# zhongzisha/multi_frame_super_resolution

Measured on AMD Instinct MI355X. Metric: Mpix/s end-to-end (N-frame burst -> x2 SR), higher is better.
Workload: dtype f32

## Files before the change

include/mfsr.h:

```cpp
#ifndef MFSR_H
#define MFSR_H

#include <stddef.h>
#include <stdint.h>

#ifdef __cplusplus
extern "C" {
#endif

#define MFSR_VERSION 100
#define MFSR_MAX_FUSE_GROUP 4

typedef void* mfsr_stream_t;

typedef struct { float x, y; } mfsr_float2;
typedef struct { float x, y, z; } mfsr_float3;
typedef struct { float x, y, z, w; } mfsr_float4;

typedef struct {
    const void* ptr;
    int32_t pitch;
    int32_t width;
    int32_t height;
} mfsr_tex2d;

enum {
    MFSR_OK = 0,
    MFSR_E_INVALID = -1,
    MFSR_E_UNSUPPORTED = -2,
    MFSR_E_NODEVICE = -3,
    MFSR_E_WORKSPACE = -4
};

enum { MFSR_RED = 0, MFSR_GREEN = 1, MFSR_BLUE = 2, MFSR_CYAN = 3, MFSR_MAGENTA = 4, MFSR_YELLOW = 5, MFSR_WHITE = 6 };

const char* mfsr_error_string(int code);
int mfsr_version(void);
int mfsr_device_count(void);

int mfsr_set_cfa_pattern(const int32_t pattern[4]);
int mfsr_get_cfa_pattern(int32_t pattern[4]);

int mfsr_deBayersSubSample3(const uint16_t* dataIn, mfsr_float3* imgOut, float maxVal, int dimX, int dimY, int strideOut,
                            mfsr_stream_t stream);
int mfsr_deBayerGreenKernel(int width, int height, const float* imgIn, int strideIn, mfsr_float3* outImage,
                            int strideOut, mfsr_float3 blackPoint, mfsr_float3 scale, mfsr_stream_t stream);
int mfsr_deBayerRedBlueKernel(int width, int height, const float* imgIn, int strideIn, mfsr_float3* outImage,
                              int strideOut, mfsr_float3 blackPoint, mfsr_float3 scale, mfsr_stream_t stream);
int mfsr_accumulateImages(const uint16_t* dataIn, mfsr_float3* imgOut, mfsr_float3* totalWeights,
                          const mfsr_float4* certaintyMask, const mfsr_float3* kernelParam, const mfsr_float2* shifts,
                          mfsr_float3 whiteLevel, mfsr_float3 blackLevel, int dimX, int dimY, int strideOut,
                          int strideMask, int strideShift, mfsr_stream_t stream);
int mfsr_accumulateImagesSuperRes(const uint16_t* dataIn, mfsr_float3* imgOut, mfsr_float3* totalWeights,
                                  const mfsr_float4* certaintyMask, mfsr_tex2d kernelParam, mfsr_tex2d shifts,
                                  mfsr_float3 whiteLevel, mfsr_float3 blackLevel, int dimX, int dimY, int strideOut,
                                  int strideMask, mfsr_stream_t stream);
int mfsr_accumulateSuperResFull(const uint16_t* dataIn, mfsr_float3* imgOut, mfsr_float3* totalWeights,
                                const mfsr_float4* certaintyMask, mfsr_tex2d kernelParam, mfsr_tex2d shifts,
                                mfsr_float3 whiteLevel, mfsr_float3 blackLevel, int dimX, int dimY, int scale,
                                int strideOut, int strideMask, mfsr_stream_t stream);

int mfsr_accumulateSuperResFull2(const uint16_t* dataIn0, const uint16_t* dataIn1, mfsr_float3* imgOut,
                                 mfsr_float3* totalWeights, const mfsr_float4* certaintyMask0,
                                 const mfsr_float4* certaintyMask1, mfsr_tex2d kernelParam, mfsr_tex2d shifts0,
                                 mfsr_tex2d shifts1, mfsr_float3 whiteLevel, mfsr_float3 blackLevel, int dimX, int dimY,
                                 int scale, int strideOut, int strideMask, mfsr_stream_t stream);

int mfsr_accumulateSuperResFullN(int nFrames, const uint16_t* const* dataIn, mfsr_float3* imgOut, mfsr_float3* totalWeights,
                                 const mfsr_float4* const* certaintyMask, mfsr_tex2d kernelParam, const mfsr_tex2d* shifts,
                                 mfsr_float3 whiteLevel, mfsr_float3 blackLevel, int dimX, int dimY, int scale,
                                 int strideOut, int strideMask, int accumulatorsUndefined, mfsr_stream_t stream);

int mfsr_accumulateSuperResFullRows(int nFrames, const uint16_t* const* dataIn, mfsr_float3* imgOut, mfsr_float3* totalWeights,
                                    const mfsr_float4* const* certaintyMask, mfsr_tex2d kernelParam, const mfsr_tex2d* shifts,
                                    mfsr_float3 whiteLevel, mfsr_float3 blackLevel, int dimX, int dimY, int scale,
                                    int strideOut, int strideMask, int accumulatorsUndefined, int rowBegin, int rowEnd,
                                    mfsr_stream_t stream);

int mfsr_accumulateSuperResFullWindow(int nFrames, const uint16_t* const* dataIn, mfsr_float3* imgOut, mfsr_float3* totalWeights,
                                      const mfsr_float4* const* certaintyMask, mfsr_tex2d kernelParam, const mfsr_tex2d* shifts,
                                      mfsr_float3 whiteLevel, mfsr_float3 blackLevel, int dimX, int dimY, int scale,
                                      int strideOut, int strideMask, int accumulatorsUndefined, int x0, int y0, int w, int h,
                                      mfsr_stream_t stream);

int mfsr_squaredSum(const float* inTiles, float* outValues, int maxShift, int tileSize, int tileCount,
                    mfsr_stream_t stream);
int mfsr_boxFilterWithBorderX(const float* inTiles, float* outTiles, int maxShift, int tileSize, int tileCount,
                              mfsr_stream_t stream);
int mfsr_boxFilterWithBorderY(const float* inTiles, float* outTiles, int maxShift, int tileSize, int tileCount,
                              mfsr_stream_t stream);
int mfsr_normalizedCC(const float* ccImage, const float* squaredTemplate, const float* boxFilteredImage,
                      float* shiftImage, int maxShift, int tileSize, int tileCount, mfsr_stream_t stream);
int mfsr_convertToTilesOverlapBorder(const float* inImg, float* outTiles, int imgWidth, int imgHeight, int imgPitch,
                                     int maxShift, int tileSize, int tileCountX, int tileCountY, mfsr_float2 baseShift,
                                     float baseRotation, mfsr_stream_t stream);
int mfsr_convertToTilesOverlapPreShift(const float* inImg, float* outTiles, const mfsr_float2* preShift,
                                       int preShiftPitch, int imgWidth, int imgHeight, int imgPitch, int maxShift,
                                       int tileSize, int tileCountX, int tileCountY, mfsr_float2 baseShift,
                                       float baseRotation, mfsr_stream_t stream);
int mfsr_GammasRGB(mfsr_float3* inOutImg, int imgWidth, int imgHeight, int imgPitch, mfsr_stream_t stream);
int mfsr_ApplyWeighting(mfsr_float3* inOutImg, const mfsr_float3* finalImg, const mfsr_float3* weight, int imgWidth,
                        int imgHeight, int imgPitch, float threshold, mfsr_stream_t stream);
int mfsr_conjugateComplexMulKernel(const mfsr_float2* aIn, mfsr_float2* bInOut, int maxElem,
                                   mfsr_stream_t stream);
int mfsr_findMinimum(const float* shiftImage, mfsr_float2* coordinates, int coordinatesPitch, int maxShift,
                     int tileCount, int tileCountX, float threshold, mfsr_stream_t stream);
int mfsr_UpSampleShifts(const mfsr_float2* inShift, mfsr_float2* outShift, int inPitch, int outPitch, int oldLevel,
                        int newLevel, int oldCountX, int oldCountY, int newCountX, int newCountY, int oldTileSize,
                        int newTileSize, mfsr_stream_t stream);
int mfsr_ComputeStructureTensor(const float* imgDx, const float* imgDy, mfsr_float3* outImg, int imgWidth,
                                int imgHeight, int imgDxDyPitch, int imgOutPitch, mfsr_stream_t stream);
int mfsr_ComputeKernelParam(mfsr_float3* kernelImg, int imgWidth, int imgHeight, int imgOutPitch, float Dth, float Dtr,
                            float kDetail, float kDenoise, float kStretch, float kShrink,
                            mfsr_stream_t stream);
int mfsr_fourierFilter(mfsr_float2* img, size_t stride, int width, int height, float lp, float hp, float lps,
                       float hps, int clearAxis, mfsr_stream_t stream);
int mfsr_fftshift(mfsr_float2* fft, int width, int height, mfsr_stream_t stream);

int mfsr_copyShiftMatrix(float* matrices, int tileCount, int imageCount, int shiftCount,
                         mfsr_stream_t stream);
int mfsr_setPointers(float** shiftMatrixArray, float** shiftMatrixSafeArray, float** matrixSquareArray,
                     float** matrixInvertedArray, float** solvedMatrixArray, mfsr_float2** shiftOneToOneArray,
                     mfsr_float2** shiftMeasuredArray, mfsr_float2** shiftOptimArray, float* shiftMatrices,
                     float* shiftSafeMatrices, float* matricesSquared, float* matricesInverted, float* solvedMatrices,
                     mfsr_float2* shiftsOneToOne, mfsr_float2* shiftsMeasured, mfsr_float2* shiftsOptim, int tileCount,
                     int imageCount, int shiftCount, mfsr_stream_t stream);
int mfsr_checkForOutliers(mfsr_float2* measuredShifts, const float* optimShiftsT, float* shiftMatrix, int* status,
                          int* inversionInfo, int tileCount, int imageCount, int shiftCount,
                          mfsr_stream_t stream);
int mfsr_transposeShifts(mfsr_float2* measuredShifts, const float* measuredShiftsT, const float* shiftsOneToOneT,
                         mfsr_float2* shiftsOneToOne, int tileCount, int imageCount, int shiftCount,
                         mfsr_stream_t stream);
int mfsr_getOptimalShifts(mfsr_float2* optimalShifts, const mfsr_float2* bestShifts, int imageCount, int tileCountX,
                          int tileCountY, int optimalShiftsPitch, int referenceImage, int imageToTrack,
                          mfsr_stream_t stream);
int mfsr_concatenateShifts(const mfsr_float2* const* shiftIn, int* shiftInPitch, mfsr_float2* shiftOut, int shiftCount,
// ... 189 lines not shown
                           int outPitch, uint16_t* out16, int width, int height, float threshold, int applyGamma, float maxOut,
                           int colOffset, int rowOffset, int fullWidth, int fullHeight, mfsr_stream_t stream);

typedef struct {
    int32_t width, height;
    int32_t frames;
    int32_t reference;
    int32_t scale;
    int32_t mono;
    int32_t cfa[4];
    float black[3], white[3];
    float maxVal;
    int32_t levels;
    int32_t levelFactor[4];
    int32_t tileSize[4];
    int32_t maxShift[4];
    float minimumThreshold;
    float sigmaTracking;
    int32_t lkIterations;
    int32_t lkHalfWindow;
    float lkMinDet;
    float alpha, beta, thresholdM;
    float sigmaTensor;
    float Dth, Dtr, kDetail, kDenoise, kStretch, kShrink;
    float weightThreshold;
    int32_t applyGamma;
    int32_t fused;
    int32_t pairFrames;
    int32_t asyncFuse;
    int32_t preAlign;
    float preAlignMaxAngle;
    int32_t uploadRing;
    int32_t maskErode;
    int32_t rawPacking;
} mfsr_config;

typedef struct mfsr_burst mfsr_burst;

int mfsr_config_default(mfsr_config* cfg, int width, int height, int frames, int scale, int mono);
size_t mfsr_burst_workspace_bytes(const mfsr_config* cfg);
size_t mfsr_burst_accumulator_bytes(const mfsr_config* cfg);
int mfsr_burst_create(mfsr_burst** out, const mfsr_config* cfg, void* workspace, size_t workspaceBytes);
void mfsr_burst_destroy(mfsr_burst* b);

int mfsr_window_check(const mfsr_config* cfg, int x0, int y0, int w, int h);
int mfsr_burst_set_window(mfsr_burst* b, int x0, int y0, int w, int h);
int mfsr_burst_get_window(const mfsr_burst* b, int* x0, int* y0, int* w, int* h);
int mfsr_burst_set_reference(mfsr_burst* b, const uint16_t* rawRef, mfsr_stream_t stream);
int mfsr_burst_set_reference_rows(mfsr_burst* b, const uint16_t* rawRef, int hrRow0, int hrRow1, mfsr_stream_t stream);
int mfsr_burst_add_frame(mfsr_burst* b, const uint16_t* raw, int isReference, mfsr_float3* imgOut,
                         mfsr_float3* totalWeights, mfsr_stream_t stream);
int mfsr_burst_begin(mfsr_burst* b, mfsr_float3* imgOut, mfsr_float3* totalWeights, mfsr_stream_t stream);
int mfsr_burst_flush(mfsr_burst* b, mfsr_stream_t stream);
int mfsr_burst_finish(mfsr_burst* b, const mfsr_float3* imgOut, const mfsr_float3* totalWeights, mfsr_float3* outImg,
                      uint16_t* out16, mfsr_stream_t stream);
int mfsr_burst_finish_rows(mfsr_burst* b, const mfsr_float3* imgOut, const mfsr_float3* totalWeights,
                           mfsr_float3* outImg, uint16_t* out16, int row0, int rows, mfsr_stream_t stream);
int mfsr_burst_set_reference_host(mfsr_burst* b, const uint16_t* hostRaw, mfsr_stream_t stream);
int mfsr_burst_add_frame_host(mfsr_burst* b, const uint16_t* hostRaw, int isReference, mfsr_float3* imgOut,
                              mfsr_float3* totalWeights, mfsr_stream_t stream);
int mfsr_burst_prefetch_host(mfsr_burst* b, const uint16_t* const* hostRaws, int nFrames, mfsr_stream_t stream);
int mfsr_burst_finish_host(mfsr_burst* b, const mfsr_float3* imgOut, const mfsr_float3* totalWeights, uint16_t* out16Dev,
                           uint16_t* out16Host, mfsr_stream_t stream);
int mfsr_burst_host_sync(mfsr_burst* b);
int mfsr_burst_set_host_row_bytes(mfsr_burst* b, int rowBytes);
int mfsr_burst_field_dims(const mfsr_burst* b, int* flowW, int* flowH, int* maskW, int* maskH);
int mfsr_burst_align_frame(mfsr_burst* b, const uint16_t* raw, int isReference, mfsr_float2* flowOut, int flowPitch,
                           mfsr_float4* maskOut, int maskPitch, mfsr_stream_t stream);
int mfsr_burst_align_frames(mfsr_burst* b, int nFrames, const uint16_t* const* raws, const int* isReference,
                            mfsr_float2* const* flowOut, int flowPitch, mfsr_float4* const* maskOut, int maskPitch,
                            mfsr_stream_t stream);
int mfsr_burst_group_size(const mfsr_config* cfg);
int mfsr_burst_fuse_rows(mfsr_burst* b, int nFrames, const uint16_t* const* raws, const mfsr_float2* const* flows, int flowPitch,
                         const mfsr_float4* const* masks, int maskPitch, mfsr_float3* imgOut, mfsr_float3* totalWeights,
                         int accumulatorsUndefined, int rowBegin, int rowEnd, mfsr_stream_t stream);

typedef struct {
    int32_t rowBegin, rowEnd;
    int32_t flowRow0, flowRows;
    int32_t maskRow0, maskRows;
    int32_t rawRow0, rawRows;
    float maxFlowY;
    int32_t reserved[3];
} mfsr_stripe_plan;
int mfsr_dist_stripe_plan(const mfsr_config* cfg, int worldSize, int rank, int rawHalo, mfsr_stripe_plan* out);
int mfsr_checkFlowBound(const mfsr_float2* flow, int pitch, int width, int rows, float bound, int* flag, mfsr_stream_t stream);
int mfsr_maxAbsFlowY(const mfsr_float2* flow, int pitch, int width, int rows, int* maxBits, mfsr_stream_t stream);
int mfsr_exactDivisionOk(float d);

typedef struct mfsr_stream mfsr_stream;
size_t mfsr_stream_workspace_bytes(const mfsr_config* cfg, int radius);
int mfsr_stream_create(mfsr_stream** out, const mfsr_config* cfg, int radius, int framesInHostMemory, void* workspace,
                       size_t workspaceBytes);
void mfsr_stream_destroy(mfsr_stream* s);
int mfsr_stream_push(mfsr_stream* s, const uint16_t* frame, mfsr_float3* outImg, uint16_t* out16, long long* produced,
                     mfsr_stream_t stream);
int mfsr_stream_drain(mfsr_stream* s, mfsr_float3* outImg, uint16_t* out16, long long* produced, mfsr_stream_t stream);
int mfsr_stream_reset(mfsr_stream* s);
int mfsr_stream_set_window(mfsr_stream* s, int x0, int y0, int w, int h);

size_t mfsr_burst_joint_workspace_bytes(const mfsr_config* cfg);
int mfsr_burst_process_joint(mfsr_burst* b, const uint16_t* const* frames, void* jointWorkspace, size_t jointBytes,
                             mfsr_float3* imgOut, mfsr_float3* totalWeights, mfsr_stream_t stream);

typedef struct {
    int (*next_frame)(void* user, uint16_t* dst, mfsr_stream_t stream);
// ... 178 lines not shown
```

multi_frame_super_resolution_amd/csrc/accumulate.hip:

```cpp
#include "accumulate_common.hpp"

__global__ void __launch_bounds__(256)
    k_accumulateImages(const uint16_t* __restrict__ dataIn, pix3* __restrict__ imgOut, pix3* __restrict__ totalWeights,
                       const float4* __restrict__ certaintyMask, const pix3* __restrict__ kernelParam,
                       const float2* __restrict__ shifts, Levels3 lv, int dimX, int dimY, int strideOut, int strideMask,
                       int strideShift, int cfa)
{
    const int x = blockIdx.x * blockDim.x + threadIdx.x;
    const int y = blockIdx.y * blockDim.y + threadIdx.y;
    if (x < 1 || y < 1 || x >= dimX - 1 || y >= dimY - 1) return;
    pix3 pixel = row_ptr(imgOut, strideOut, y)[x];
    pix3 totalWeight = row_ptr(totalWeights, strideOut, y)[x];
    const pix3 kernel = row_ptr(kernelParam, strideOut, y)[x];
    const float2 shift = row_ptr(shifts, strideShift, y)[x];
    const int sx = round2i(shift.x);
    const int sy = round2i(shift.y);
#pragma unroll
    for (int py = -2; py <= 2; py++) {
        const int ppsy = clampi(y + py + sy, 0, dimY - 1);
        const int ppy = clampi(y + py, 0, dimY - 1);
#pragma unroll
        for (int px = -2; px <= 2; px++) {
            const int ppsx = clampi(x + px + sx, 0, dimX - 1);
            const int ppx = clampi(x + px, 0, dimX - 1);
// ... 15 lines not shown
{
    MFSR_REQUIRE(dataIn && imgOut && totalWeights && certaintyMask && kernelParam && shifts);
    MFSR_REQUIRE(dimX > 2 && dimY > 2);
    MFSR_REQUIRE((long long)strideOut >= 12LL * dimX && (strideOut & 3) == 0);
    MFSR_REQUIRE((long long)strideShift >= 8LL * dimX && (strideShift & 7) == 0 && ((uintptr_t)shifts & 7) == 0);
    MFSR_REQUIRE((long long)strideMask >= 16LL * ((dimX + 1) / 2) && (strideMask & 15) == 0 &&
                 ((uintptr_t)certaintyMask & 15) == 0);
    dim3 block(64, 4), grid(mfsr_cdiv(dimX, 64), mfsr_cdiv(dimY, 4));
    hipLaunchKernelGGL(k_accumulateImages, grid, block, 0, mfsr_s(stream), dataIn, (pix3*)imgOut, (pix3*)totalWeights,
                       (const float4*)certaintyMask, (const pix3*)kernelParam, (const float2*)shifts,
                       make_levels(whiteLevel, blackLevel), dimX, dimY, strideOut, strideMask, strideShift,
                       mfsr_cfa_packed());
    return mfsr_launch_status("accumulateImages");
}

template <int GEOM, bool FAST, bool WIN = false>
__global__ void __launch_bounds__(256)
    k_accumulateSuperRes(const uint16_t* __restrict__ dataIn, pix3* __restrict__ imgOut, pix3* __restrict__ totalWeights,
                         const float4* __restrict__ certaintyMask, mfsr_tex2d kernelParam, mfsr_tex2d shifts, Levels3 lv,
                         int dimX, int dimY, int scale, int strideOut, int strideMask, int cfa, int rowBegin, int rowEnd,
                         int colBegin, int colEnd)
{
    const int x = blockIdx.x * blockDim.x + threadIdx.x + (WIN ? colBegin : 0);
    const int y = blockIdx.y * blockDim.y + threadIdx.y + rowBegin;
    const int outW = (GEOM == GEOM_CROP) ? dimX : dimX * scale;
    const int outH = (GEOM == GEOM_CROP) ? dimY : dimY * scale;
    if (x < 1 || y < 1 || x >= outW - 1 || y >= outH - 1 || y >= rowEnd) return;
    if (WIN && x >= colEnd) return;
    accumulate_pixel_generic<GEOM, FAST>(x, y, dataIn, imgOut, totalWeights, certaintyMask, kernelParam, shifts, lv, dimX,
                                         dimY, scale, strideOut, strideMask, cfa, WIN ? colBegin : 0, WIN ? rowBegin : 0);
}

static int g_accumulate_fast = 2;
extern "C" int mfsr_set_accumulate_fast_exp(int enable)
{
    g_accumulate_fast = enable < 0 ? 0 : (enable > 2 ? 2 : enable);
    return MFSR_OK;
}
extern "C" int mfsr_get_accumulate_fast_exp(void) { return g_accumulate_fast; }

int mfsr_try_launch_accumulate2x_strip(int nFrames, const uint16_t* const* dataIn, mfsr_float3* imgOut,
                                       mfsr_float3* totalWeights, const mfsr_float4* const* certaintyMask,
                                       mfsr_tex2d kernelParam, const mfsr_tex2d* shifts, mfsr_float3 whiteLevel,
                                       mfsr_float3 blackLevel, int dimX, int dimY, int strideOut, int strideMask,
                                       int fresh, int rowBegin, int rowEnd, int colBegin, int colEnd, int relative,
                                       mfsr_stream_t stream);

int mfsr_try_launch_accumulate4x_tile(int nFrames, const uint16_t* const* dataIn, mfsr_float3* imgOut,
                                      mfsr_float3* totalWeights, const mfsr_float4* const* certaintyMask,
                                      mfsr_tex2d kernelParam, const mfsr_tex2d* shifts, mfsr_float3 whiteLevel,
                                      mfsr_float3 blackLevel, int dimX, int dimY, int strideOut, int strideMask,
                                      int fresh, int rowBegin, int rowEnd, int colBegin, int colEnd, int relative,
                                      mfsr_stream_t stream);

static int check_superres_args(const uint16_t* dataIn, mfsr_float3* imgOut, mfsr_float3* totalWeights,
                               const mfsr_float4* certaintyMask, const mfsr_tex2d& kernelParam, const mfsr_tex2d& shifts,
                               int dimX, int dimY, int outW, int strideOut, int strideMask)
{
    MFSR_REQUIRE(dataIn && imgOut && totalWeights && certaintyMask);
    MFSR_REQUIRE(dimX >= 8 && dimY >= 8);
    MFSR_REQUIRE(mfsr_tex_ok(kernelParam, 16) && ((uintptr_t)kernelParam.ptr & 15) == 0 && (kernelParam.pitch & 15) == 0);
    MFSR_REQUIRE(mfsr_tex_ok(shifts, 8) && ((uintptr_t)shifts.ptr & 7) == 0 && (shifts.pitch & 7) == 0);
    MFSR_REQUIRE((long long)strideOut >= 12LL * outW && (strideOut & 3) == 0);
    MFSR_REQUIRE((long long)strideMask >= 16LL * ((dimX + 1) / 2) && (strideMask & 15) == 0 &&
                 ((uintptr_t)certaintyMask & 15) == 0);
    return MFSR_OK;
}

extern "C" int mfsr_accumulateImagesSuperRes(const uint16_t* dataIn, mfsr_float3* imgOut, mfsr_float3* totalWeights,
                                             const mfsr_float4* certaintyMask, mfsr_tex2d kernelParam, mfsr_tex2d shifts,
                                             mfsr_float3 whiteLevel, mfsr_float3 blackLevel, int dimX, int dimY,
                                             int strideOut, int strideMask, mfsr_stream_t stream)
{
    int rc = check_superres_args(dataIn, imgOut, totalWeights, certaintyMask, kernelParam, shifts, dimX, dimY, dimX,
                                 strideOut, strideMask);
    if (rc) return rc;
    dim3 block(64, 4), grid(mfsr_cdiv(dimX, 64), mfsr_cdiv(dimY, 4));
    const Levels3 lv = make_levels(whiteLevel, blackLevel);
    if (g_accumulate_fast)
        hipLaunchKernelGGL((k_accumulateSuperRes<GEOM_CROP, true>), grid, block, 0, mfsr_s(stream), dataIn, (pix3*)imgOut,
                           (pix3*)totalWeights, (const float4*)certaintyMask, kernelParam, shifts, lv, dimX, dimY, 2,
                           strideOut, strideMask, mfsr_cfa_packed(), 0, dimY, 0, 0);
    else
        hipLaunchKernelGGL((k_accumulateSuperRes<GEOM_CROP, false>), grid, block, 0, mfsr_s(stream), dataIn,
                           (pix3*)imgOut, (pix3*)totalWeights, (const float4*)certaintyMask, kernelParam, shifts, lv, dimX,
                           dimY, 2, strideOut, strideMask, mfsr_cfa_packed(), 0, dimY, 0, 0);
    return mfsr_launch_status("accumulateImagesSuperRes");
}

static int accumulate_full_win(const uint16_t* dataIn, mfsr_float3* imgOut, mfsr_float3* totalWeights,
                               const mfsr_float4* certaintyMask, mfsr_tex2d kernelParam, mfsr_tex2d shifts,
                               mfsr_float3 whiteLevel, mfsr_float3 blackLevel, int dimX, int dimY, int scale, int strideOut,
                               int strideMask, const HrWindow& w, mfsr_stream_t stream)
{
    MFSR_REQUIRE(scale >= 1 && scale <= 8);
    int rc = check_superres_args(dataIn, imgOut, totalWeights, certaintyMask, kernelParam, shifts, dimX, dimY,
                                 w.rel ? w.x1 - w.x0 : dimX * scale, strideOut, strideMask);
    if (rc) return rc;
    if (g_accumulate_fast == 2 && scale == 2 &&
        mfsr_try_launch_accumulate2x_strip(1, &dataIn, imgOut, totalWeights, &certaintyMask, kernelParam, &shifts, whiteLevel,
                                           blackLevel, dimX, dimY, strideOut, strideMask, 0, w.y0, w.y1, w.x0, w.x1, w.rel,
                                           stream) == 1)
        return mfsr_launch_status("accumulateSuperResFull(strip)");
    if (g_accumulate_fast == 2 && scale == 4 &&
        mfsr_try_launch_accumulate4x_tile(1, &dataIn, imgOut, totalWeights, &certaintyMask, kernelParam, &shifts, whiteLevel,
                                          blackLevel, dimX, dimY, strideOut, strideMask, 0, w.y0, w.y1, w.x0, w.x1, w.rel,
// ... 105 lines not shown
                                           blackLevel, dimX, dimY, scale, strideOut, strideMask, w, stream);
        if (rc) return rc;
    }
    return MFSR_OK;
}

extern "C" int mfsr_accumulateSuperResFullRows(int nFrames, const uint16_t* const* dataIn, mfsr_float3* imgOut,
                                               mfsr_float3* totalWeights, const mfsr_float4* const* certaintyMask,
                                               mfsr_tex2d kernelParam, const mfsr_tex2d* shifts, mfsr_float3 whiteLevel,
                                               mfsr_float3 blackLevel, int dimX, int dimY, int scale, int strideOut,
                                               int strideMask, int accumulatorsUndefined, int rowBegin, int rowEnd,
                                               mfsr_stream_t stream)
{
    MFSR_REQUIRE(nFrames >= 1 && nFrames <= MFSR_MAX_FUSE_GROUP && dataIn && certaintyMask && shifts);
    MFSR_REQUIRE(scale >= 1 && scale <= 8);
    const int hrH = scale * dimY;
    MFSR_REQUIRE(rowBegin >= 0 && rowBegin < rowEnd && rowEnd <= hrH && (rowBegin % 16) == 0 && ((rowEnd % 16) == 0 || rowEnd == hrH));
    return accumulate_group_win(nFrames, dataIn, imgOut, totalWeights, certaintyMask, kernelParam, shifts, whiteLevel, blackLevel, dimX,
                                dimY, scale, strideOut, strideMask, accumulatorsUndefined,
                                HrWindow{0, rowBegin, scale * dimX, rowEnd, 0}, stream);
}

extern "C" int mfsr_accumulateSuperResFullWindow(int nFrames, const uint16_t* const* dataIn, mfsr_float3* imgOut,
                                                 mfsr_float3* totalWeights, const mfsr_float4* const* certaintyMask,
                                                 mfsr_tex2d kernelParam, const mfsr_tex2d* shifts, mfsr_float3 whiteLevel,
                                                 mfsr_float3 blackLevel, int dimX, int dimY, int scale, int strideOut,
                                                 int strideMask, int accumulatorsUndefined, int x0, int y0, int w, int h,
                                                 mfsr_stream_t stream)
{
    MFSR_REQUIRE(nFrames >= 1 && nFrames <= MFSR_MAX_FUSE_GROUP && dataIn && certaintyMask && shifts);
    MFSR_REQUIRE(scale >= 1 && scale <= 8 && dimX > 0 && dimY > 0);
    const int hrW = scale * dimX, hrH = scale * dimY;
    if (w == 0 && h == 0 && x0 == 0 && y0 == 0) {
        w = hrW;
        h = hrH;
    }
    MFSR_REQUIRE(mfsr_window_ok(hrW, hrH, x0, y0, w, h));
    MFSR_REQUIRE((strideOut & 15) == 0 && ((uintptr_t)imgOut & 15) == 0 && ((uintptr_t)totalWeights & 15) == 0);
    return accumulate_group_win(nFrames, dataIn, imgOut, totalWeights, certaintyMask, kernelParam, shifts, whiteLevel, blackLevel, dimX,
                                dimY, scale, strideOut, strideMask, accumulatorsUndefined, HrWindow{x0, y0, x0 + w, y0 + h, 1}, stream);
}

extern "C" int mfsr_accumulateSuperResFullN(int nFrames, const uint16_t* const* dataIn, mfsr_float3* imgOut,
                                            mfsr_float3* totalWeights, const mfsr_float4* const* certaintyMask,
                                            mfsr_tex2d kernelParam, const mfsr_tex2d* shifts, mfsr_float3 whiteLevel,
                                            mfsr_float3 blackLevel, int dimX, int dimY, int scale, int strideOut,
                                            int strideMask, int accumulatorsUndefined, mfsr_stream_t stream)
{
    MFSR_REQUIRE(scale >= 1 && scale <= 8 && dimY > 0);
    return mfsr_accumulateSuperResFullRows(nFrames, dataIn, imgOut, totalWeights, certaintyMask, kernelParam, shifts, whiteLevel,
                                           blackLevel, dimX, dimY, scale, strideOut, strideMask, accumulatorsUndefined, 0,
                                           scale * dimY, stream);
}
```

multi_frame_super_resolution_amd/csrc/accumulate_fast.hip:

```cpp
#include <cstdlib>

#include "accumulate_common.hpp"
#include <type_traits>

namespace {

template <int CFA>
struct Cfa {
    static constexpr int col(int yp, int xp) { return (CFA >> (2 * ((yp << 1) | xp))) & 3; }
    static constexpr int pos_of(int c)
    {
        int n = 0, p = -1;
        for (int a = 0; a < 4; a++)
            if (((CFA >> (2 * a)) & 3) == c) {
                n++;
                p = a;
            }
        return n == 1 ? p : -1;
    }
    static constexpr int count(int c)
    {
        int n = 0;
        for (int a = 0; a < 4; a++)
            if (((CFA >> (2 * a)) & 3) == c) n++;
// ... 968 lines not shown
#pragma unroll 1
        for (int n = 0; n < NF; n++) {
            if (!((safeBits >> n) & 1u) && stripLive) {
                TileFrame F = fr.f[0];
#pragma unroll
                for (int m = 1; m < NF; m++)
                    if (n == m) F = fr.f[m];
#pragma unroll 1
                for (int k = 0; k < 4; k++) {
                    const int X = X0 + k;
                    if (X >= 1 && X < hrW - 1) {
                        pix3 px = {0.0f, 0.0f, 0.0f}, tw = {0.0f, 0.0f, 0.0f};
                        if (DO_P) px = {myP[3 * k], myP[3 * k + 1], myP[3 * k + 2]};
                        if (DO_W) tw = {myW[3 * k], myW[3 * k + 1], myW[3 * k + 2]};
                        accumulate_pixel_core<GEOM_FULL, true>(X, Y, F.raw, F.mask, kernelParam, F.shifts, glv, dimX, dimY, 2,
                                                               strideMask, cfaPacked, px, tw);
                        if (DO_P) { myP[3 * k] = px.x; myP[3 * k + 1] = px.y; myP[3 * k + 2] = px.z; }
                        if (DO_W) { myW[3 * k] = tw.x; myW[3 * k + 1] = tw.y; myW[3 * k + 2] = tw.z; }
                    }
                }
            }
        }
    };
    auto store_plane = [&](int pl, char* g) {
        asm volatile("s_waitcnt lgkmcnt(0)" ::: "memory");
#pragma unroll
        for (int j = 0; j < 3; j++) {
            const size_t off = (size_t)(j * 64 + lx) * 16;
            const size_t gb = segByte + off;
            const bool sideMargin = gb < (size_t)STRIP_MARGIN * 12 || gb + 16 > rowBytes - (size_t)STRIP_MARGIN * 12;
            if (gb + 16 <= rowBytes && (fresh || !sideMargin) && inWin(gb)) *(float4*)chunk(g, off) = sAcc[pl][ly][j * 64 + lx];
        }
    };
    using Yes = std::true_type;
    using No = std::false_type;
    asm volatile("s_waitcnt vmcnt(0)" ::: "memory");
    constexpr bool valueSumsStaged = TILE_PIXEL_MAJOR && (NF > 1 || FR != 4);
    if constexpr (PL == 2) {
        if (!valueSumsStaged) add_plane(0, accP);
        add_plane(1, accW);
        if (safeBits != (1u << NF) - 1u) slow_frames(Yes{}, Yes{}, 0, 1);
        store_plane(0, gP);
        store_plane(1, gW);
    } else {
        if (!valueSumsStaged) add_plane(0, accP);
        if (safeBits != (1u << NF) - 1u) slow_frames(Yes{}, No{}, 0, 0);
        store_plane(0, gP);
        asm volatile("s_waitcnt lgkmcnt(0)" ::: "memory");
        stage_plane(gW, 0);
        asm volatile("s_waitcnt vmcnt(0)" ::: "memory");
        add_plane(0, accW);
        if (safeBits != (1u << NF) - 1u) slow_frames(No{}, Yes{}, 0, 0);
        store_plane(0, gW);
    }
}

template <int K8, int CFA, bool PARITY = false, typename RawF, typename MaskF>
__device__ __forceinline__ void strip_pixel4_w(int X, int Y, int sx, int sy, const float (&w)[13], RawF rawf, MaskF mval,
                                                const StripLevels& lv, float* accP, float* accW)
{
    const int qx = X + sx - 2, qy = Y + sy - 2;
    const int x0 = qx >> 2, y0 = qy >> 2;
    const uint32_t bx0 = 0u - (uint32_t)(qx & 1), bx1 = 0u - (uint32_t)((qx >> 1) & 1);
    const uint32_t by0 = 0u - (uint32_t)(qy & 1), by1 = 0u - (uint32_t)((qy >> 1) & 1);
    const uint32_t mx[5] = {0u, bx0 & bx1, bx1, bx0 | bx1, ~0u};
    const uint32_t my[5] = {0u, by0 & by1, by1, by0 | by1, ~0u};
    const uint32_t mP = 0u - (uint32_t)(x0 & 1), mQ = 0u - (uint32_t)(y0 & 1);
    auto andm = [](uint32_t m, float a) { return __uint_as_float(m & __float_as_uint(a)); };

    float s[2][2];
    rawf(x0, y0, s);
    auto W_ = [&](int jt, int it) { const int n = jt * 5 + it; return w[n <= 12 ? n : 24 - n]; };

    auto cellOf = [](int it) { return (K8 + it - 2 + 8) >> 3; };
    constexpr int cellLo = (K8 - 2 + 8) >> 3;
    constexpr bool twoCells = ((K8 + 4 - 2 + 8) >> 3) != cellLo;

    float C[5][2];
#pragma unroll
    for (int jt = 0; jt < 5; jt++) {
        const uint32_t mya = mQ ^ my[jt];
        float Ee[2], Eo[2];
        if constexpr (PARITY) {
            const int ph = qy & 3;
            const int flip = jt == 0 ? 0 : (jt == 4 ? 1 : (jt == 1 ? (ph == 3) : (jt == 2 ? (ph >> 1) : (ph != 0))));
            const int e = (((y0 & 1) ^ flip) << 1) | (x0 & 1);
#pragma unroll
            for (int c = 0; c < (twoCells ? 2 : 1); c++) {
                Ee[c] = mval(jt, cellLo + c, e);
                Eo[c] = mval(jt, cellLo + c, e ^ 1);
            }
        } else {
#pragma unroll
            for (int c = 0; c < (twoCells ? 2 : 1); c++) {
                float m[3];
#pragma unroll
                for (int ch = 0; ch < 3; ch++) m[ch] = mval(jt, cellLo + c, ch);
                resolve_certainty<CFA>(mya, mP, m, Ee[c], Eo[c]);
            }
        }
        float lo[2] = {0.0f, 0.0f}, hi[2] = {0.0f, 0.0f};
        bool loUsed[2] = {false, false}, hiUsed[2] = {false, false};
#pragma unroll
        for (int it = 0; it < 5; it++) {
            const int c = cellOf(it) - cellLo;
            const float wt = W_(jt, it);
// ... 627 lines not shown
            if (msx) {
                (void)hipEventRecord(msx->join, msx->stream);
                (void)hipStreamWaitEvent(st, msx->join, 0);
            }
        };
        if (nFrames == 1) launch_mono(std::integral_constant<int, 1>{});
        if (nFrames == 2) launch_mono(std::integral_constant<int, 2>{});
        return 1;
    }
#define STRIP_CASE(a, b, c, d)                                                                                         \
    case pack_cfa(a, b, c, d):                                                                                         \
        if (pair) {                                                                                                    \
            using CfaTag = std::integral_constant<int, pack_cfa(a, b, c, d)>;                                          \
            if (nFrames == 2) launch_group(CfaTag{}, std::integral_constant<int, 2>{});                                \
            if (nFrames == 3) launch_group(CfaTag{}, std::integral_constant<int, 3>{});                                \
            if (nFrames == 4) launch_group(CfaTag{}, std::integral_constant<int, 4>{});                                \
        } else if (nFrames == 2) {                                                                                     \
            TileFrames<2> fr;                                                                                          \
            for (int n = 0; n < 2; n++) {                                                                              \
                fr.f[n].raw = dataIn[n];                                                                               \
                fr.f[n].mask = (const float4*)certaintyMask[n];                                                        \
                fr.f[n].shifts = shifts[n];                                                                            \
            }                                                                                                          \
            launch_strip_regs<pack_cfa(a, b, c, d), 2>(grid, block, st, fr, pI, pT, kernelParam, glv, lv, dimX, dimY,  \
                                                       strideOut, strideMask, cp, rowBlock0, wlc);                                \
            launch_margin(0);                                                                                          \
            launch_margin(1);                                                                                          \
        } else {                                                                                                       \
            TileFrames<1> fr;                                                                                          \
            fr.f[0].raw = dataIn[0];                                                                                   \
            fr.f[0].mask = (const float4*)certaintyMask[0];                                                            \
            fr.f[0].shifts = shifts[0];                                                                                \
            if (tile_kernel_ok(kernelParam, shifts[0], dimX, dimY))                                                    \
                launch_tile<pack_cfa(a, b, c, d), 1>(grid, block, st, fr, pI, pT, kernelParam, glv, lv, dimX, dimY,    \
                                                     strideOut, strideMask, cp, tileFresh, rowBlock0, wlc);                       \
            else                                                                                                       \
                launch_strip_regs<pack_cfa(a, b, c, d), 1>(grid, block, st, fr, pI, pT, kernelParam, glv, lv, dimX,    \
                                                           dimY, strideOut, strideMask, cp, rowBlock0, wlc);                       \
            launch_margin(0);                                                                                          \
        }                                                                                                              \
        return 1;
    switch (packed2) {
        STRIP_CASE(MFSR_RED, MFSR_GREEN, MFSR_GREEN, MFSR_BLUE)
        STRIP_CASE(MFSR_BLUE, MFSR_GREEN, MFSR_GREEN, MFSR_RED)
        STRIP_CASE(MFSR_GREEN, MFSR_RED, MFSR_BLUE, MFSR_GREEN)
        STRIP_CASE(MFSR_GREEN, MFSR_BLUE, MFSR_RED, MFSR_GREEN)
        STRIP_CASE(MFSR_GREEN, MFSR_GREEN, MFSR_GREEN, MFSR_GREEN)
        default: break;
    }
#undef STRIP_CASE
    return 0;
}

int mfsr_try_launch_accumulate4x_tile(int nFrames, const uint16_t* const* dataIn, mfsr_float3* imgOut,
                                      mfsr_float3* totalWeights, const mfsr_float4* const* certaintyMask,
                                      mfsr_tex2d kernelParam, const mfsr_tex2d* shifts, mfsr_float3 whiteLevel,
                                      mfsr_float3 blackLevel, int dimX, int dimY, int strideOut, int strideMask,
                                      int fresh, int rowBegin, int rowEnd, int colBegin, int colEnd, int relative,
                                      mfsr_stream_t stream)
{
    read_env_once();
    if (nFrames < 1 || nFrames > 4 || !g_strip_use_tile) return 0;
    int cfa[4];
    mfsr_get_cfa_pattern(cfa);
    for (int i = 0; i < 4; i++)
        if (cfa[i] > MFSR_BLUE) return 0;
    const int packed2 = pack_cfa(cfa[0], cfa[1], cfa[2], cfa[3]);
    const int hrW = 4 * dimX, hrH = 4 * dimY;
    if ((dimX & 1) || (dimY & 1) || ((uintptr_t)imgOut & 15) || ((uintptr_t)totalWeights & 15) || (strideOut & 15)) return 0;
    if (hrW < 4 * STRIP_MARGIN || hrH < 4 * STRIP_MARGIN) return 0;
    for (int n = 0; n < nFrames; n++)
        if (!(kernelParam.width == shifts[n].width && kernelParam.height == shifts[n].height && kernelParam.width * 8 == hrW &&
              kernelParam.height * 8 == hrH && kernelParam.width >= 4))
            return 0;
    Levels3 glv;
    StripLevels lv;
    const float wl[3] = {whiteLevel.x, whiteLevel.y, whiteLevel.z}, bl[3] = {blackLevel.x, blackLevel.y, blackLevel.z};
    for (int c = 0; c < 3; c++) {
        glv.white[c] = wl[c];
        glv.black[c] = bl[c];
        lv.black[c] = bl[c];
        lv.invWhite[c] = 1.0f / wl[c];
    }
    hipStream_t st = mfsr_s(stream);
    pix3* pI = (pix3*)imgOut;
    pix3* pT = (pix3*)totalWeights;
    const int cp = mfsr_cfa_packed();
    const int tileY0 = rowBegin / 2;
    const WinLaunch wlc = win_launch(HrWindow{colBegin, rowBegin, colEnd, rowEnd, relative}, hrW, 512);
    const MarginRects mr = margin_rects(hrW, hrH, STRIP_MARGIN, HrWindow{colBegin, rowBegin, colEnd, rowEnd, relative});
    const int tilesX = wlc.tilesX, tilesY = mfsr_cdiv(rowEnd, 2) - tileY0;
    const dim3 block(64, 4), grid(tilesX * tilesY);
    if (fresh) {
        if (zero_margin_bands(imgOut, totalWeights, hrH, strideOut, rowBegin, rowEnd, wlc, st) != 0) return -1;
    }
    MarginStream* msx = (g_margin_overlap && !fresh) ? margin_stream() : nullptr;
    if (msx && (hipEventRecord(msx->fork, st) != hipSuccess || hipStreamWaitEvent(msx->stream, msx->fork, 0) != hipSuccess)) msx = nullptr;
    const hipStream_t mst = msx ? msx->stream : st;
    auto launch_margin = [&](int n) {
        const int M = STRIP_MARGIN;
        const long long cnt = 2LL * (M - 1) * (hrW - 2) + (long long)(hrH - 2 * M) * 2 * (M - 1);
        if (!wlc.on)
            hipLaunchKernelGGL(k_accumulateMargin<4>, dim3(mfsr_cdiv(cnt, 256)), dim3(256), 0, mst, dataIn[n], pI, pT,
                               (const float4*)certaintyMask[n], kernelParam, shifts[n], glv, dimX, dimY, strideOut, strideMask, cp,
                               rowBegin, rowEnd, mr);
        else if (mr.start[4] > 0)
// ... 53 lines not shown
```

multi_frame_super_resolution_amd/csrc/pipeline.cpp:

```cpp
#include <hip/hip_runtime.h>

#include <cmath>
#include <cstdio>
#include <cstring>
#include <new>
#include <vector>

#include "common.hpp"
#include "raw_stage.hpp"

namespace {

constexpr int kMaxLevels = 4;
constexpr int kMaxTimedLaunches = 4096;
constexpr int kRing = 2 * MFSR_MAX_FUSE_GROUP;
constexpr int kMaxUploadRing = 32;

inline size_t align_up(size_t v, size_t a) { return (v + a - 1) / a * a; }

struct Img {
    void* ptr = nullptr;
    int pitch = 0;
    int w = 0, h = 0;
};

struct FrameProducts {
    uint16_t* raw;
    Img half;
    Img pyr[8];
    void* prePyr;
};

struct AlignScratch {
    Img shifts[kMaxLevels];
    Img lkSum[2], lkDiff[2];
    mfsr_prealign* preResult;
};

struct Layout {
    int W, H, hw, hh, tw, th, hrW, hrH;
    int flowScale;
    int lw[kMaxLevels], lh[kMaxLevels];
    int tcx[kMaxLevels], tcy[kMaxLevels];
    int maxFactor;
    FrameProducts ref, mov[MFSR_MAX_FUSE_GROUP];
    AlignScratch work[MFSR_MAX_FUSE_GROUP];
    int nAlign;
    Img kparam4;
    Img tensor, tensorTmp, tensorSm;
    Img fallback;
    Img tmpA, tmpB;
    Img flowBuf[2 * kRing];
    Img maskBuf[kRing];
    Img maskRaw[MFSR_MAX_FUSE_GROUP];
    Img pre[kMaxLevels];
    Img warped, Ix, Iy, It, rawf;
    float *refTiles, *movTiles, *cc, *boxX, *boxY, *sqsum, *dist;
    float* refSq[kMaxLevels];
    void* preWork;
    uint16_t* rawRing[kMaxUploadRing];
    uint16_t* refRaw[2];
    uint8_t* stage[kMaxUploadRing + 2];
    size_t total;
};

struct Bump {
    char* base;
    size_t off;
    void* take(size_t bytes)
    {
        off = align_up(off, 256);
        void* p = base ? base + off : nullptr;
        off += bytes;
        return p;
    }
    Img image(int w, int h, int elemBytes)
    {
        Img im;
        im.w = w;
        im.h = h;
        im.pitch = (int)align_up((size_t)w * elemBytes, 64);
        im.ptr = take((size_t)im.pitch * h);
        return im;
    }
};

int ilog2(int v)
{
    int l = 0;
    while ((1 << l) < v) l++;
    return l;
}

int validate(const mfsr_config* c)
{
    MFSR_REQUIRE(c != nullptr);
    MFSR_REQUIRE(c->width >= 64 && c->height >= 64 && (c->width % 4) == 0 && (c->height % 4) == 0);
    MFSR_REQUIRE(c->frames >= 1 && c->reference >= 0 && c->reference < c->frames);
    MFSR_REQUIRE(c->scale >= 1 && c->scale <= 8);
    MFSR_REQUIRE(c->levels >= 1 && c->levels <= kMaxLevels);
    MFSR_REQUIRE(c->levelFactor[c->levels - 1] == 1);
    for (int l = 0; l < c->levels; l++) {
        const int f = c->levelFactor[l];
        MFSR_REQUIRE(f >= 1 && f <= 128 && (f & (f - 1)) == 0);
        if (l > 0) MFSR_REQUIRE(c->levelFactor[l] < c->levelFactor[l - 1]);
        MFSR_REQUIRE(c->tileSize[l] >= 4 && c->tileSize[l] <= 128 && c->maxShift[l] >= 1 && c->maxShift[l] <= 15);
// ... 69 lines not shown
    for (int l = 0; l < kMaxLevels; l++) L->refSq[l] = nullptr;
    if (c->fused) {
        for (int l = 0; l < c->levels; l++) L->refSq[l] = (float*)b.take((size_t)L->tcx[l] * L->tcy[l] * 4);
        for (int i = 0; i < 2; i++) {
            L->work[0].lkSum[i] = b.image(L->tw, L->th, 4);
            L->work[0].lkDiff[i] = b.image(L->tw, L->th, 4);
        }
    }
    L->Ix = b.image(L->tw, L->th, 4);
    L->Iy = b.image(L->tw, L->th, 4);
    if (!c->fused) {
        L->warped = b.image(L->tw, L->th, 4);
        L->It = b.image(L->tw, L->th, 4);
        L->rawf = b.image(L->W, L->H, 4);
        L->refTiles = (float*)b.take(maxTileFloats * 4);
        L->movTiles = (float*)b.take(maxTileFloats * 4);
        L->cc = (float*)b.take(maxTileFloats * 4);
        L->boxX = (float*)b.take(maxTileFloats * 4);
        L->boxY = (float*)b.take(maxTileFloats * 4);
        L->sqsum = (float*)b.take(maxTiles * 4);
        L->dist = (float*)b.take(maxDist * 4);
    }
    if (c->preAlign) {
        const size_t pb = mfsr_preAlign_pyramid_bytes(L->tw, L->th);
        L->ref.prePyr = b.take(pb);
        L->mov[0].prePyr = b.take(pb);
        L->preWork = b.take(mfsr_preAlign_workspace_bytes(c->preAlignMaxAngle));
        L->work[0].preResult = (mfsr_prealign*)b.take(sizeof(mfsr_prealign));
    }
    L->nAlign = c->fused ? mfsr_burst_group_size(c) : 1;
    for (int q = 1; q < L->nAlign; q++) {
        FrameProducts& M = L->mov[q];
        AlignScratch& S = L->work[q];
        M.half = b.image(L->hw, L->hh, 12);
        for (int i = 0; i < nl; i++) M.pyr[i] = b.image(L->tw >> i, L->th >> i, 4);
        for (int l = 0; l < c->levels; l++) S.shifts[l] = b.image(L->tcx[l], L->tcy[l], 8);
        for (int i = 0; i < 2; i++) {
            S.lkSum[i] = b.image(L->tw, L->th, 4);
            S.lkDiff[i] = b.image(L->tw, L->th, 4);
        }
        if (c->preAlign) {
            M.prePyr = b.take(mfsr_preAlign_pyramid_bytes(L->tw, L->th));
            S.preResult = (mfsr_prealign*)b.take(sizeof(mfsr_prealign));
        }
    }
    for (int i = 0; i < c->uploadRing; i++) L->rawRing[i] = (uint16_t*)b.take((size_t)L->W * L->H * 2);
    if (c->uploadRing > 0)
        for (int i = 0; i < 2; i++) L->refRaw[i] = (uint16_t*)b.take((size_t)L->W * L->H * 2);
    if (c->maskErode > 0)
        for (int i = 0; i < mfsr_burst_group_size(c); i++) L->maskRaw[i] = b.image(L->hw, L->hh, 16);
    if (c->rawPacking != MFSR_PACK_NONE)
        for (int i = 0; i < c->uploadRing + 2; i++)
            L->stage[i] = (uint8_t*)b.take((size_t)mfsr_packed_row_bytes(c->rawPacking, L->W) * L->H);
    L->total = align_up(b.off, 256);
    return layout;
}

mfsr_tex2d as_tex(const Img& im)
{
    mfsr_tex2d t;
    t.ptr = im.ptr;
    t.pitch = im.pitch;
    t.width = im.w;
    t.height = im.h;
    return t;
}

}

struct mfsr_burst {
    mfsr_burst(const mfsr_config& c, char* workspace) : cfg(c), L(make_layout(&c, workspace)) {}
    mfsr_config cfg;
    const Layout L;
    FrameProducts ref;
    float taps[99];
    int ntaps;
    float tensorTaps[99];
    int ntensorTaps;
    const Img* flowCur;
    const Img* maskCur;
    mfsr_prealign* preCur;
    bool haveRef;
    bool refStale;
    struct Pending {
        int n;
        int slot[MFSR_MAX_FUSE_GROUP];
        const uint16_t* raw[MFSR_MAX_FUSE_GROUP];
        const Img* flow[MFSR_MAX_FUSE_GROUP];
        const Img* mask[MFSR_MAX_FUSE_GROUP];
        bool deferred[MFSR_MAX_FUSE_GROUP];
        int isRef[MFSR_MAX_FUSE_GROUP];
        mfsr_float3 *imgOut, *totalWeights;
    } pend;
    Pending held;
    bool heldHas;
    int group;
    int nFramesTimed;
    struct Fresh {
        bool has;
        mfsr_float3 *imgOut, *totalWeights;
    } fresh;
    int frameCounter;
    hipStream_t fuseStream;
    hipEvent_t evAligned[kRing];
    hipEvent_t evFused[kRing];
    hipEvent_t evRefStart, evRefDone;
    bool refOnFuse;
    bool fusedOutstanding[kRing];
    const Img* slotFlow[kRing];
    hipStream_t copyStream;
    hipStream_t downStream;
    hipEvent_t evFinished, evDown;
    bool downRecorded;
    hipEvent_t evBand[16];
    int framesSinceRef;
    bool holdLastGroup;
    hipEvent_t evUp[kMaxUploadRing + 2];
    hipEvent_t evFree[kMaxUploadRing + 2];
    bool freeRecorded[kMaxUploadRing + 2];
    hipStream_t freeOn[kMaxUploadRing + 2];
    int hostRowBytes;
    bool renderOn;
    mfsr_render render;
    bool sharpenOn;
    mfsr_sharpen sharpen;
    int sharpenedFinishes;
    unsigned long long hostEpoch;
    hipEvent_t evEpoch;
    hipEvent_t evUnp[kMaxUploadRing + 2];
    hipEvent_t unpDone[kMaxUploadRing + 2];
    int unpQ[kMaxUploadRing + 2], nUnp;
    struct Prefetched {
        const uint16_t* host;
        int slot;
    } prefetched[kMaxUploadRing];
    int nPrefetched, prefetchHead;
    bool upPending;
    int upPendingSlot;
    int refSlot;
    bool hostBusy;
    int upCounter, refCounter;
    const uint16_t* refHost;
    const uint16_t* refDev;
    std::vector<float> jointHost;
    struct Window {
        bool on = false;
        int x0 = 0, y0 = 0, w = 0, h = 0;
    } win, winNext;
    bool timing;
    int nEvents;
    hipEvent_t evStart[kMaxTimedLaunches], evStop[kMaxTimedLaunches];
    int32_t paths[MFSR_PATH_COUNT];
};

#define TRY(expr)                  \
    do {                           \
        int rc_ = (expr);          \
        if (rc_ != MFSR_OK) return rc_; \
    } while (0)

static int flush_pending(mfsr_burst* b, mfsr_stream_t stream, bool materializeFresh = true);

static int out_w(const mfsr_burst* b) { return b->win.on ? b->win.w : b->L.hrW; }
static int out_h(const mfsr_burst* b) { return b->win.on ? b->win.h : b->L.hrH; }
static size_t acc_bytes(const mfsr_burst* b) { return (size_t)12 * out_w(b) * out_h(b); }

static int fuse_group(mfsr_burst* b, int n, const uint16_t* const* raws, mfsr_float3* imgOut, mfsr_float3* totalWeights,
                      const mfsr_float4* const* masks, const mfsr_tex2d* flows, int maskPitch, int fresh, int r0, int r1,
                      mfsr_stream_t stream)
{
    const mfsr_config& c = b->cfg;
    const Layout& L = b->L;
    const mfsr_float3 white = {c.white[0], c.white[1], c.white[2]};
    const mfsr_float3 black = {c.black[0], c.black[1], c.black[2]};
    if (!b->win.on)
        return mfsr_accumulateSuperResFullRows(n, raws, imgOut, totalWeights, masks, as_tex(L.kparam4), flows, white, black, L.W, L.H,
                                               c.scale, 12 * L.hrW, maskPitch, fresh, r0, r1, stream);
    const int pitch = 12 * b->win.w;
    const size_t off = (size_t)r0 * pitch;
    return mfsr_accumulateSuperResFullWindow(n, raws, (mfsr_float3*)((char*)imgOut + off), (mfsr_float3*)((char*)totalWeights + off),
                                             masks, as_tex(L.kparam4), flows, white, black, L.W, L.H, c.scale, pitch, maskPitch, fresh,
                                             b->win.x0, b->win.y0 + r0, b->win.w, r1 - r0, stream);
}


extern "C" int mfsr_config_default(mfsr_config* cfg, int width, int height, int frames, int scale, int mono)
{
    MFSR_REQUIRE(cfg != nullptr);
    memset(cfg, 0, sizeof(*cfg));
    cfg->width = width;
    cfg->height = height;
    cfg->frames = frames;
    cfg->reference = 0;
    cfg->scale = scale;
    cfg->mono = mono;
    if (mono) {
        cfg->cfa[0] = cfg->cfa[1] = cfg->cfa[2] = cfg->cfa[3] = MFSR_GREEN;
    } else {
        cfg->cfa[0] = MFSR_RED;
        cfg->cfa[1] = MFSR_GREEN;
        cfg->cfa[2] = MFSR_GREEN;
        cfg->cfa[3] = MFSR_BLUE;
    }
    for (int i = 0; i < 3; i++) {
// ... 19 lines not shown
    cfg->sigmaTensor = 1.0f;
    cfg->Dth = 0.005f;
    cfg->Dtr = 0.05f;
    cfg->kDetail = 0.3f;
    cfg->kDenoise = 2.0f;
    cfg->kStretch = 2.0f;
    cfg->kShrink = 2.0f;
    cfg->weightThreshold = 1e-3f;
    cfg->applyGamma = 0;
    cfg->fused = 1;
    cfg->pairFrames = 1;
    cfg->preAlign = 0;
    cfg->preAlignMaxAngle = 20.0f;
    cfg->asyncFuse = 0;
    return MFSR_OK;
}

extern "C" size_t mfsr_burst_workspace_bytes(const mfsr_config* cfg)
{
    if (validate(cfg) != MFSR_OK) return 0;
    return make_layout(cfg, nullptr).total;
}

extern "C" size_t mfsr_burst_accumulator_bytes(const mfsr_config* cfg)
{
    if (!cfg || cfg->width <= 0 || cfg->height <= 0 || cfg->scale <= 0) return 0;
    return (size_t)12 * cfg->scale * cfg->width * (size_t)cfg->scale * cfg->height;
}

extern "C" int mfsr_burst_create(mfsr_burst** out, const mfsr_config* cfg, void* workspace, size_t workspaceBytes)
{
    MFSR_REQUIRE(out != nullptr && workspace != nullptr);
    TRY(validate(cfg));
    if (mfsr_device_count() <= 0) {
        fprintf(stderr, "mfsr: no HIP device available (there is no CPU fallback)\n");
        return MFSR_E_NODEVICE;
    }
    MFSR_REQUIRE(((uintptr_t)workspace & 255) == 0);
    mfsr_burst* b = new (std::nothrow) mfsr_burst(*cfg, (char*)workspace);
    MFSR_REQUIRE(b != nullptr);
    if (b->L.total > workspaceBytes) {
        fprintf(stderr, "mfsr: workspace too small: need %zu bytes, got %zu\n", b->L.total, workspaceBytes);
        delete b;
        return MFSR_E_WORKSPACE;
    }
    b->ntaps = mfsr_gaussin_filter_1D(cfg->sigmaTracking, b->taps);
    b->ntensorTaps = mfsr_gaussin_filter_1D(cfg->sigmaTensor, b->tensorTaps);
    b->flowCur = &b->L.flowBuf[0];
    b->maskCur = &b->L.maskBuf[0];
    b->preCur = b->L.work[0].preResult;
    b->ref = b->L.ref;
    b->pend.n = 0;
    b->group = mfsr_burst_group_size(&b->cfg);
    b->fresh.has = false;
    b->nFramesTimed = 0;
    b->timing = false;
    b->nEvents = 0;
    memset(b->evStart, 0, sizeof(b->evStart));
    memset(b->evStop, 0, sizeof(b->evStop));
    b->frameCounter = 0;
    b->fuseStream = nullptr;
    b->evRefStart = b->evRefDone = nullptr;
    b->refOnFuse = false;
    for (int i = 0; i < kRing; i++) {
        b->evAligned[i] = b->evFused[i] = nullptr;
        b->fusedOutstanding[i] = false;
        b->slotFlow[i] = nullptr;
    }
    if (cfg->asyncFuse) {
        int lo = 0, hi = 0;
        hipError_t e = hipDeviceGetStreamPriorityRange(&lo, &hi);
        static const int prioMode = [] {
            const char* v = getenv("MFSR_FUSE_PRIO");
            return !v ? 0 : (v[0] == 'l' ? 1 : (v[0] == 'n' ? 2 : 0));
        }();
        const int prio = prioMode == 1 ? lo : (prioMode == 2 ? (lo + hi) / 2 : hi);
        if (e == hipSuccess) e = hipStreamCreateWithPriority(&b->fuseStream, hipStreamNonBlocking, prio);
        if (e == hipSuccess) e = hipEventCreateWithFlags(&b->evRefStart, hipEventDisableTiming);
        if (e == hipSuccess) e = hipEventCreateWithFlags(&b->evRefDone, hipEventDisableTiming);
        for (int i = 0; i < kRing && e == hipSuccess; i++) {
            e = hipEventCreateWithFlags(&b->evAligned[i], hipEventDisableTiming);
            if (e == hipSuccess) e = hipEventCreateWithFlags(&b->evFused[i], hipEventDisableTiming);
        }
        if (e != hipSuccess) {
            mfsr_burst_destroy(b);
            return MFSR_E_NODEVICE;
        }
    }
    b->copyStream = nullptr;
    b->downStream = nullptr;
    b->evFinished = b->evDown = nullptr;
    b->downRecorded = false;
    b->upCounter = b->refCounter = 0;
    for (int i = 0; i < 16; i++) b->evBand[i] = nullptr;
    b->framesSinceRef = 0;
    b->holdLastGroup = false;
    b->heldHas = false;
    b->held.n = 0;
    b->refHost = b->refDev = nullptr;
    b->refSlot = -1;
    b->hostBusy = false;
    b->upPending = false;
    b->upPendingSlot = -1;
    b->nPrefetched = b->prefetchHead = 0;
    for (int i = 0; i < kMaxUploadRing + 2; i++) {
        b->evUp[i] = b->evFree[i] = b->evUnp[i] = b->unpDone[i] = nullptr;
        b->freeRecorded[i] = false;
        b->freeOn[i] = nullptr;
    }
    b->hostRowBytes = 0;
    b->renderOn = false;
    b->sharpenOn = false;
    b->sharpenedFinishes = 0;
    b->nUnp = 0;
    b->hostEpoch = 0;
    b->evEpoch = nullptr;
    if (cfg->uploadRing > 0) {
        hipError_t e = hipStreamCreateWithFlags(&b->copyStream, hipStreamNonBlocking);
        if (e == hipSuccess) e = hipStreamCreateWithFlags(&b->downStream, hipStreamNonBlocking);
        if (e == hipSuccess) e = hipEventCreateWithFlags(&b->evFinished, hipEventDisableTiming);
        if (e == hipSuccess) e = hipEventCreateWithFlags(&b->evDown, hipEventDisableTiming);
        if (e == hipSuccess) e = hipEventCreateWithFlags(&b->evEpoch, hipEventDisableTiming);
        for (int i = 0; i < cfg->uploadRing + 2 && e == hipSuccess; i++) {
            e = hipEventCreateWithFlags(&b->evUp[i], hipEventDisableTiming);
            if (e == hipSuccess) e = hipEventCreateWithFlags(&b->evFree[i], hipEventDisableTiming);
            if (e == hipSuccess && cfg->rawPacking != MFSR_PACK_NONE) e = hipEventCreateWithFlags(&b->evUnp[i], hipEventDisableTiming);
        }
        if (e != hipSuccess) {
            mfsr_burst_destroy(b);
            return MFSR_E_NODEVICE;
        }
    }
    b->haveRef = false;
    b->refStale = false;
    memset(b->paths, 0, sizeof(b->paths));
    *out = b;
    return MFSR_OK;
}

extern "C" void mfsr_burst_destroy(mfsr_burst* b)
{
    if (!b) return;
    for (int i = 0; i < kMaxTimedLaunches; i++) {
        if (b->evStart[i]) (void)hipEventDestroy(b->evStart[i]);
        if (b->evStop[i]) (void)hipEventDestroy(b->evStop[i]);
    }
    if (b->fuseStream) (void)hipStreamSynchronize(b->fuseStream);
    for (int i = 0; i < kRing; i++) {
        if (b->evAligned[i]) (void)hipEventDestroy(b->evAligned[i]);
        if (b->evFused[i]) (void)hipEventDestroy(b->evFused[i]);
    }
    if (b->evRefStart) (void)hipEventDestroy(b->evRefStart);
    if (b->evRefDone) (void)hipEventDestroy(b->evRefDone);
    if (b->fuseStream) (void)hipStreamDestroy(b->fuseStream);
    if (b->copyStream) (void)hipStreamSynchronize(b->copyStream);
    if (b->downStream) (void)hipStreamSynchronize(b->downStream);
    if (b->evFinished) (void)hipEventDestroy(b->evFinished);
    if (b->evDown) (void)hipEventDestroy(b->evDown);
    if (b->evEpoch) (void)hipEventDestroy(b->evEpoch);
    for (int i = 0; i < 16; i++)
        if (b->evBand[i]) (void)hipEventDestroy(b->evBand[i]);
    if (b->downStream) (void)hipStreamDestroy(b->downStream);
    for (int i = 0; i < kMaxUploadRing + 2; i++) {
        if (b->evUp[i]) (void)hipEventDestroy(b->evUp[i]);
        if (b->evFree[i]) (void)hipEventDestroy(b->evFree[i]);
        if (b->evUnp[i]) (void)hipEventDestroy(b->evUnp[i]);
    }
    if (b->copyStream) (void)hipStreamDestroy(b->copyStream);
    delete b;
}

extern "C" int mfsr_burst_timing(mfsr_burst* b, int enable)
{
    MFSR_REQUIRE(b != nullptr);
    b->timing = enable != 0;
    b->nEvents = 0;
    b->nFramesTimed = 0;
    return MFSR_OK;
}

extern "C" int mfsr_burst_timing_read(mfsr_burst* b, double* totalMs, int* launches, int* frames)
{
    MFSR_REQUIRE(b && totalMs && launches && frames);
    double total = 0;
    for (int i = 0; i < b->nEvents; i++) {
        MFSR_HIP_TRY(hipEventSynchronize(b->evStop[i]));
        float ms = 0;
        MFSR_HIP_TRY(hipEventElapsedTime(&ms, b->evStart[i], b->evStop[i]));
        total += ms;
    }
    *totalMs = total;
    *launches = b->nEvents;
    *frames = b->nFramesTimed;
    b->nEvents = 0;
    b->nFramesTimed = 0;
    return MFSR_OK;
}

static int unpack_uploaded(mfsr_burst* b, int lastSlot, mfsr_stream_t stream);
static int wait_uploads(mfsr_burst* b, mfsr_stream_t stream)
{
    if (b->upPending) {
        MFSR_HIP_TRY(hipStreamWaitEvent(mfsr_s(stream), b->evUp[b->upPendingSlot], 0));
        b->upPending = false;
        if (b->nUnp > 0) TRY(unpack_uploaded(b, b->upPendingSlot, stream));
    }
    return MFSR_OK;
}

static int record_free(mfsr_burst* b, int us, mfsr_stream_t stream)
{
    MFSR_HIP_TRY(hipEventRecord(b->evFree[us], mfsr_s(stream)));
    b->freeRecorded[us] = true;
    b->freeOn[us] = mfsr_s(stream);
    return MFSR_OK;
}

static int unpack_uploaded(mfsr_burst* b, int lastSlot, mfsr_stream_t stream)
{
    const Layout& L = b->L;
    int n = 0;
    while (n < b->nUnp && b->unpQ[n] != lastSlot) n++;
    if (n == b->nUnp) return MFSR_OK;
    n++;
    const uint8_t* packed[kMaxUploadRing + 2];
    uint16_t* frames[kMaxUploadRing + 2];
    for (int i = 0; i < n; i++) {
        const int us = b->unpQ[i];
        packed[i] = L.stage[us];
        frames[i] = us < b->cfg.uploadRing ? L.rawRing[us] : L.refRaw[us - b->cfg.uploadRing];
        if (b->freeRecorded[us]) {
            if (b->freeOn[us] != mfsr_s(stream)) MFSR_HIP_TRY(hipStreamWaitEvent(mfsr_s(stream), b->evFree[us], 0));
            b->freeRecorded[us] = false;
        }
    }
    static_assert(kMaxUploadRing + 2 <= kRawMaxFrames, "one launch takes every upload slot");
    TRY(mfsr_unpackRaw(n, packed, mfsr_packed_row_bytes(b->cfg.rawPacking, L.W), b->cfg.rawPacking, frames, 2 * L.W, L.W, L.H, stream));
    hipEvent_t done = b->evUnp[b->unpQ[0]];
    MFSR_HIP_TRY(hipEventRecord(done, mfsr_s(stream)));
    for (int i = 0; i < n; i++) b->unpDone[b->unpQ[i]] = done;
    for (int i = n; i < b->nUnp; i++) b->unpQ[i - n] = b->unpQ[i];
    b->nUnp -= n;
    return MFSR_OK;
}

// ... 130 lines not shown
    if (!fusedRing) MFSR_HIP_TRY(hipMemsetAsync(fb, 0, (size_t)L.fallback.pitch * (r1 - r0), mfsr_s(es)));
    if (c.fused) {
        if (fusedRing) {
            const mfsr_tex2d fbt = {fb, L.fallback.pitch, L.W, r1 - r0};
            TRY(mfsr_deBayerFusedRing(rawRef + (size_t)r0 * L.W, fbt, bp, sc, es));
        } else
            TRY(mfsr_deBayerFused(rawRef + (size_t)r0 * L.W, (mfsr_float3*)fb, L.fallback.pitch, L.W, r1 - r0, bp, sc, es));
        if (es != stream) {
            MFSR_HIP_TRY(hipEventRecord(b->evRefDone, b->fuseStream));
            b->refOnFuse = true;
        }
    } else {
        TRY(mfsr_u16ToFloat(rawRef, (float*)L.rawf.ptr, L.rawf.pitch, L.W, L.H, 1.0f, stream));
        TRY(mfsr_deBayerGreenKernel(L.W, L.H, (const float*)L.rawf.ptr, L.rawf.pitch, (mfsr_float3*)L.fallback.ptr,
                                    L.fallback.pitch, bp, sc, stream));
        TRY(mfsr_deBayerRedBlueKernel(L.W, L.H, (const float*)L.rawf.ptr, L.rawf.pitch, (mfsr_float3*)L.fallback.ptr,
                                      L.fallback.pitch, bp, sc, stream));
    }
    b->haveRef = true;
    b->refStale = false;
    b->framesSinceRef = 0;
    b->holdLastGroup = false;
    return MFSR_OK;
}

extern "C" int mfsr_burst_set_reference(mfsr_burst* b, const uint16_t* rawRef, mfsr_stream_t stream)
{
    MFSR_REQUIRE(b != nullptr);
    return set_reference_impl(b, rawRef, 0, b->L.hrH, stream);
}

extern "C" int mfsr_burst_set_reference_rows(mfsr_burst* b, const uint16_t* rawRef, int hrRow0, int hrRow1, mfsr_stream_t stream)
{
    MFSR_REQUIRE(b != nullptr);
    return set_reference_impl(b, rawRef, hrRow0, hrRow1, stream);
}

extern "C" int mfsr_window_check(const mfsr_config* cfg, int x0, int y0, int w, int h)
{
    MFSR_REQUIRE(cfg != nullptr);
    TRY(validate(cfg));
    const int hrW = cfg->width * cfg->scale, hrH = cfg->height * cfg->scale;
    if (x0 == 0 && y0 == 0 && ((w == 0 && h == 0) || (w == hrW && h == hrH))) return MFSR_OK;
    if (!mfsr_window_ok(hrW, hrH, x0, y0, w, h)) return MFSR_E_INVALID;
    if (!cfg->fused) return MFSR_E_UNSUPPORTED;
    return MFSR_OK;
}

extern "C" int mfsr_burst_set_window(mfsr_burst* b, int x0, int y0, int w, int h)
{
    MFSR_REQUIRE(b != nullptr);
    const int rc = mfsr_window_check(&b->cfg, x0, y0, w, h);
    if (rc != MFSR_OK) return rc;
    if (b->pend.n > 0 || b->heldHas) {
        fprintf(stderr, "mfsr: mfsr_burst_set_window with frames pending (flush or finish the burst first)\n");
        return MFSR_E_INVALID;
    }
    const Layout& L = b->L;
    const bool whole = (x0 == 0 && y0 == 0 && w == 0 && h == 0) || (x0 == 0 && y0 == 0 && w == L.hrW && h == L.hrH);
    b->winNext.on = !whole;
    b->winNext.x0 = whole ? 0 : x0;
    b->winNext.y0 = whole ? 0 : y0;
    b->winNext.w = whole ? 0 : w;
    b->winNext.h = whole ? 0 : h;
    return MFSR_OK;
}

extern "C" int mfsr_burst_get_window(const mfsr_burst* b, int* x0, int* y0, int* w, int* h)
{
    MFSR_REQUIRE(b && x0 && y0 && w && h);
    const mfsr_burst::Window& v = b->winNext;
    *x0 = v.on ? v.x0 : 0;
    *y0 = v.on ? v.y0 : 0;
    *w = v.on ? v.w : b->L.hrW;
    *h = v.on ? v.h : b->L.hrH;
    return MFSR_OK;
}

static int track_tiles(mfsr_burst* b, const FrameProducts& refF, float* const* refSq, const FrameProducts& movF,
                       const AlignScratch& work, const mfsr_prealign* hostBase, mfsr_stream_t stream)
{
    const mfsr_config& c = b->cfg;
    const Layout& L = b->L;
    const mfsr_float2 zero2 = {0.0f, 0.0f};
    for (int l = 0; l < c.levels; l++) {
        const int pi = ilog2(c.levelFactor[l]);
        const Img& ref = refF.pyr[pi];
        const Img& mov = movF.pyr[pi];
        const int T = c.tileSize[l], S = c.maxShift[l];
        const int tiles = L.tcx[l] * L.tcy[l];
        const mfsr_float2* pre = nullptr;
        b->paths[mfsr_trackTilesFastSupported(T, S) ? MFSR_PATH_TRACK_FAST_PAIR : MFSR_PATH_TRACK_GENERIC_PAIR]++;
        if (c.fused && l > 0) {
            TRY(mfsr_trackTilesFusedUp((const float*)ref.ptr, (const float*)mov.ptr, (const mfsr_float2*)work.shifts[l - 1].ptr,
                                       work.shifts[l - 1].pitch, c.levelFactor[l - 1], c.levelFactor[l], L.tcx[l - 1], L.tcy[l - 1],
                                       c.tileSize[l - 1], (mfsr_float2*)work.shifts[l].ptr, work.shifts[l].pitch, ref.w, ref.h, ref.pitch, S,
                                       T, L.tcx[l], L.tcy[l], c.minimumThreshold, refSq[l], c.preAlign ? work.preResult : nullptr,
                                       1.0f / (float)c.levelFactor[l], stream));
            b->paths[MFSR_PATH_TRACK_FUSED_UP]++;
            continue;
        }
        if (l > 0) {
            TRY(mfsr_UpSampleShifts((const mfsr_float2*)work.shifts[l - 1].ptr, (mfsr_float2*)L.pre[l].ptr,
                                    work.shifts[l - 1].pitch, L.pre[l].pitch, c.levelFactor[l - 1], c.levelFactor[l],
                                    L.tcx[l - 1], L.tcy[l - 1], L.tcx[l], L.tcy[l], c.tileSize[l - 1], T, stream));
            pre = (const mfsr_float2*)L.pre[l].ptr;
        }
        if (c.fused) {
            TRY(mfsr_trackTilesFusedBase((const float*)ref.ptr, (const float*)mov.ptr, pre, L.pre[l].pitch,
                                         (mfsr_float2*)work.shifts[l].ptr, work.shifts[l].pitch, ref.w, ref.h, ref.pitch, S, T,
                                         L.tcx[l], L.tcy[l], c.minimumThreshold, refSq[l],
                                         c.preAlign ? work.preResult : nullptr, 1.0f / (float)c.levelFactor[l], stream));
            b->paths[MFSR_PATH_TRACK_FUSED_BASE]++;
        } else {
            b->paths[MFSR_PATH_TRACK_CHAIN]++;
            if (!pre) {
                MFSR_HIP_TRY(hipMemsetAsync(L.pre[l].ptr, 0, (size_t)L.pre[l].pitch * L.pre[l].h, mfsr_s(stream)));
                pre = (const mfsr_float2*)L.pre[l].ptr;
            }
            TRY(mfsr_convertToTilesOverlapBorder((const float*)ref.ptr, L.refTiles, ref.w, ref.h, ref.pitch, S, T, L.tcx[l],
                                                 L.tcy[l], zero2, 0.0f, stream));
            mfsr_float2 base = zero2;
            float rot = 0.0f;
            if (hostBase) {
                const float inv = 1.0f / (float)c.levelFactor[l];
                base.x = hostBase->shiftX * inv;
                base.y = hostBase->shiftY * inv;
                rot = hostBase->rotation;
            }
            TRY(mfsr_convertToTilesOverlapPreShift((const float*)mov.ptr, L.movTiles, pre, L.pre[l].pitch, mov.w, mov.h,
                                                   mov.pitch, S, T, L.tcx[l], L.tcy[l], base, rot, stream));
            TRY(mfsr_crossCorrelateTiles(L.refTiles, L.movTiles, L.cc, S, T, tiles, stream));
            TRY(mfsr_squaredSum(L.refTiles, L.sqsum, S, T, tiles, stream));
            TRY(mfsr_boxFilterWithBorderX(L.movTiles, L.boxX, S, T, tiles, stream));
            TRY(mfsr_boxFilterWithBorderY(L.boxX, L.boxY, S, T, tiles, stream));
            TRY(mfsr_normalizedCC(L.cc, L.sqsum, L.boxY, L.dist, S, T, tiles, stream));
            TRY(mfsr_findMinimum(L.dist, (mfsr_float2*)work.shifts[l].ptr, work.shifts[l].pitch, S, tiles, L.tcx[l],
                                 c.minimumThreshold, stream));
            TRY(mfsr_addRoundedPreShift(pre, L.pre[l].pitch, (mfsr_float2*)work.shifts[l].ptr, work.shifts[l].pitch, L.tcx[l],
                                        L.tcy[l], stream));
        }
    }
    return MFSR_OK;
}

static int upload_slot_of(const mfsr_burst* b, const uint16_t* raw)
{
    if (!raw) return -1;
    for (int i = 0; i < b->cfg.uploadRing; i++)
        if (b->L.rawRing[i] == raw) return i;
    for (int i = 0; i < 2; i++)
        if (b->cfg.uploadRing > 0 && b->L.refRaw[i] == raw) return b->cfg.uploadRing + i;
    return -1;
}

static int align_deferred(mfsr_burst* b, mfsr_stream_t stream);

static int accumulate_pending(mfsr_burst* b, mfsr_stream_t callerStream);

static int fuse_held(mfsr_burst* b, mfsr_stream_t callerStream)
{
    if (!b->heldHas) return MFSR_OK;
    const mfsr_burst::Pending later = b->pend;
    b->pend = b->held;
    b->heldHas = false;
    b->held.n = 0;
    const int rc = accumulate_pending(b, callerStream);
    b->pend = later;
    return rc;
}

static int accumulate_pending(mfsr_burst* b, mfsr_stream_t callerStream)
{
    TRY(fuse_held(b, callerStream));
    TRY(align_deferred(b, callerStream));
    TRY(wait_uploads(b, callerStream));
    const mfsr_config& c = b->cfg;
    const mfsr_burst::Pending p = b->pend;
    b->pend.n = 0;
    const int n = p.n;
    if (n == 0) return MFSR_OK;
    mfsr_float3* imgOut = p.imgOut;
    mfsr_float3* totalWeights = p.totalWeights;
    mfsr_stream_t stream = callerStream;
    if (b->fuseStream) {
        stream = (mfsr_stream_t)b->fuseStream;
        for (int i = 0; i < n; i++) MFSR_HIP_TRY(hipStreamWaitEvent(b->fuseStream, b->evAligned[p.slot[i]], 0));
    }
    TRY(mfsr_set_cfa_pattern(c.cfa));
    const bool timed = b->timing && b->nEvents < kMaxTimedLaunches;
    if (timed) {
        const int i = b->nEvents;
        if (!b->evStart[i]) MFSR_HIP_TRY(hipEventCreate(&b->evStart[i]));
        if (!b->evStop[i]) MFSR_HIP_TRY(hipEventCreate(&b->evStop[i]));
        MFSR_HIP_TRY(hipEventRecord(b->evStart[i], mfsr_s(stream)));
    }
    {
        const mfsr_float4* masks[MFSR_MAX_FUSE_GROUP];
        mfsr_tex2d flows[MFSR_MAX_FUSE_GROUP];
        for (int i = 0; i < n; i++) {
            masks[i] = (const mfsr_float4*)p.mask[i]->ptr;
            flows[i] = as_tex(*p.flow[i]);
        }
        const int freshNow = b->fresh.has && b->fresh.imgOut == imgOut && b->fresh.totalWeights == totalWeights;
        if (b->fresh.has && !freshNow) {
            const size_t bytes = acc_bytes(b);
            MFSR_HIP_TRY(hipMemsetAsync(b->fresh.imgOut, 0, bytes, mfsr_s(stream)));
            MFSR_HIP_TRY(hipMemsetAsync(b->fresh.totalWeights, 0, bytes, mfsr_s(stream)));
        }
        b->fresh.has = false;
        TRY(fuse_group(b, n, p.raw, imgOut, totalWeights, masks, flows, p.mask[0]->pitch, freshNow, 0, out_h(b), stream));
    }
    if (timed) {
        MFSR_HIP_TRY(hipEventRecord(b->evStop[b->nEvents], mfsr_s(stream)));
        b->nEvents++;
        b->nFramesTimed += n;
    }
    if (b->copyStream) {
        for (int j = 0; j < n; j++) {
            const int us = upload_slot_of(b, p.raw[j]);
            if (us >= 0) TRY(record_free(b, us, stream));
        }
    }
    if (b->fuseStream) {
        for (int i = 0; i < n; i++) {
            MFSR_HIP_TRY(hipEventRecord(b->evFused[p.slot[i]], b->fuseStream));
            b->fusedOutstanding[p.slot[i]] = true;
        }
    }
    return MFSR_OK;
}

static int wait_ref_products(mfsr_burst* b, mfsr_stream_t stream)
{
    if (b->refOnFuse && mfsr_s(stream) != b->fuseStream) MFSR_HIP_TRY(hipStreamWaitEvent(mfsr_s(stream), b->evRefDone, 0));
    return MFSR_OK;
}

static int join_fuse(mfsr_burst* b, mfsr_stream_t stream)
{
    if (!b->fuseStream) return MFSR_OK;
    TRY(wait_ref_products(b, stream));
    for (int i = 0; i < kRing; i++)
        if (b->fusedOutstanding[i]) {
            MFSR_HIP_TRY(hipStreamWaitEvent(mfsr_s(stream), b->evFused[i], 0));
            b->fusedOutstanding[i] = false;
        }
    return MFSR_OK;
}

static int flush_pending(mfsr_burst* b, mfsr_stream_t stream, bool materializeFresh)
{
    if (materializeFresh && b->fresh.has && b->pend.n == 0 && !b->heldHas) {
        const size_t bytes = acc_bytes(b);
        MFSR_HIP_TRY(hipMemsetAsync(b->fresh.imgOut, 0, bytes, mfsr_s(stream)));
        MFSR_HIP_TRY(hipMemsetAsync(b->fresh.totalWeights, 0, bytes, mfsr_s(stream)));
        b->fresh.has = false;
    }
    TRY(accumulate_pending(b, stream));
    return join_fuse(b, stream);
}

static bool lk_warped_path(const mfsr_burst* b)
{
    static const bool lkWarped = [] {
        const char* e = getenv("MFSR_LK_WARPED");
        return !(e && e[0] == '0');
    }();
    const mfsr_config& c = b->cfg;
    return c.fused && lkWarped && c.lkIterations > 0 && b->L.tw >= 64 && b->L.th >= 32;
}

static const Img* final_flow(const mfsr_burst* b, int slot, int isReference)
{
    const mfsr_config& c = b->cfg;
    return &b->L.flowBuf[2 * slot + (!isReference && c.fused ? (c.lkIterations & 1) : 0)];
}

static int align_pre(mfsr_burst* b, const uint16_t* raw, int isReference, int slot, const FrameProducts& mov, bool prepared,
                     const AlignScratch& work, const Img* suppliedShifts, mfsr_stream_t stream)
{
    const mfsr_config& c = b->cfg;
    const Layout& L = b->L;
    const FrameProducts& ref = b->ref;
    TRY(wait_uploads(b, stream));
    if (b->fuseStream && b->fusedOutstanding[slot]) {
        MFSR_HIP_TRY(hipStreamWaitEvent(mfsr_s(stream), b->evFused[slot], 0));
        b->fusedOutstanding[slot] = false;
    }
    const Img* flow = &L.flowBuf[2 * slot];
    if (isReference) {
        const Img* mask = &L.maskBuf[slot];
        MFSR_HIP_TRY(hipMemsetAsync(flow->ptr, 0, (size_t)flow->pitch * flow->h, mfsr_s(stream)));
        return mfsr_fill_f32((float*)mask->ptr, (size_t)mask->pitch / 4 * mask->h, 1.0f, stream);
    }
    if (!prepared) TRY(prepare_frame(b, raw, mov, stream));
    mfsr_prealign hostBase;
    const mfsr_prealign* hb = nullptr;
    if (c.preAlign) {
        if (!prepared) TRY(mfsr_preAlignPyramid((const float*)mov.pyr[0].ptr, L.tw, L.th, mov.pyr[0].pitch, mov.prePyr, stream));
        TRY(mfsr_preAlign(ref.prePyr, mov.prePyr, L.tw, L.th, c.preAlignMaxAngle, L.preWork, work.preResult, stream));
        b->preCur = work.preResult;
        if (!c.fused) {
            MFSR_HIP_TRY(hipMemcpyAsync(&hostBase, work.preResult, sizeof(hostBase), hipMemcpyDeviceToHost, mfsr_s(stream)));
            MFSR_HIP_TRY(hipStreamSynchronize(mfsr_s(stream)));
            hb = &hostBase;
// ... 275 lines not shown
    bool maskBatch = stageBatch && batched && m > 0;
    if (maskBatch) {
        mfsr_robustness_frame rf[MFSR_MAX_FUSE_GROUP];
        for (int k = 0; k < m; k++) {
            const int slot = b->pend.slot[idx[mq[k]]];
            rf[k].movedHalf = (const mfsr_float3*)L.mov[mq[k]].half.ptr;
            rf[k].mask = (mfsr_float4*)(c.maskErode > 0 ? L.maskRaw[k].ptr : L.maskBuf[slot].ptr);
            rf[k].flow = (const mfsr_float2*)final_flow(b, slot, 0)->ptr;
        }
        const int rc = mfsr_robustnessMaskFusedBatch(m, rf, (const mfsr_float3*)ref.half.ptr, L.flowBuf[0].pitch, L.tw, L.th, L.hw, L.hh,
                                                     ref.half.pitch, L.maskBuf[0].pitch, c.alpha, c.beta, c.thresholdM, stream);
        if (rc == MFSR_E_UNSUPPORTED)
            maskBatch = false;
        else if (rc)
            return rc;
        else
            b->paths[MFSR_PATH_ROBUST_BATCH]++;
        if (maskBatch && c.maskErode > 0) {
            const mfsr_float4* ein[MFSR_MAX_FUSE_GROUP];
            mfsr_float4* eout[MFSR_MAX_FUSE_GROUP];
            for (int k = 0; k < m; k++) {
                ein[k] = (const mfsr_float4*)L.maskRaw[k].ptr;
                eout[k] = (mfsr_float4*)L.maskBuf[b->pend.slot[idx[mq[k]]]].ptr;
            }
            TRY(mfsr_erodeMaskBatch(m, ein, eout, L.hw, L.hh, L.maskRaw[0].pitch, L.maskBuf[0].pitch, c.maskErode, stream));
        }
    }
    for (int q = 0; q < n; q++) {
        const int i = idx[q], slot = b->pend.slot[i];
        if (!b->pend.isRef[i]) {
            if (!batched) TRY(align_lk(b, slot, L.mov[q], L.work[q], stream));
            if (!maskBatch) TRY(align_post(b, slot, L.mov[q], stream));
        }
        aligned_outputs(b, slot, b->pend.isRef[i], &b->pend.flow[i], &b->pend.mask[i]);
        b->pend.deferred[i] = false;
        b->flowCur = b->pend.flow[i];
        b->maskCur = b->pend.mask[i];
        if (b->fuseStream) MFSR_HIP_TRY(hipEventRecord(b->evAligned[b->pend.slot[i]], mfsr_s(stream)));
    }
    return MFSR_OK;
}

static int add_frame_impl(mfsr_burst* b, const uint16_t* raw, int isReference, mfsr_float3* imgOut, mfsr_float3* totalWeights,
                          bool hostBurst, mfsr_stream_t stream, const FrameProducts* prepared = nullptr,
                          const Img* suppliedShifts = nullptr)
{
    MFSR_REQUIRE(b && raw && imgOut && totalWeights);
    MFSR_REQUIRE(b->haveRef);
    MFSR_REQUIRE(!b->refStale);
    const mfsr_config& c = b->cfg;
    TRY(mfsr_set_cfa_pattern(c.cfa));
    b->holdLastGroup = hostBurst;
    if (b->pend.n && (b->pend.imgOut != imgOut || b->pend.totalWeights != totalWeights)) TRY(flush_pending(b, stream));
    if (b->pend.n >= b->group) TRY(accumulate_pending(b, stream));
    MFSR_REQUIRE(b->pend.n < MFSR_MAX_FUSE_GROUP);
    const int slot = b->frameCounter++ % kRing;
    const Img *flow = nullptr, *mask = nullptr;
    const bool defer = can_defer_alignment(b, prepared || suppliedShifts);
    b->paths[defer ? MFSR_PATH_FRAMES_DEFERRED : MFSR_PATH_FRAMES_IMMEDIATE]++;
    if (!defer) {
        TRY(align_deferred(b, stream));
        TRY(align_frame(b, raw, isReference, slot, prepared, suppliedShifts, &flow, &mask, stream));
        b->flowCur = flow;
        b->maskCur = mask;
        if (b->fuseStream) MFSR_HIP_TRY(hipEventRecord(b->evAligned[slot], mfsr_s(stream)));
    }
    if (defer) b->slotFlow[slot] = nullptr;
    const int i = b->pend.n++;
    b->pend.slot[i] = slot;
    b->pend.raw[i] = raw;
    b->pend.flow[i] = flow;
    b->pend.mask[i] = mask;
    b->pend.deferred[i] = defer;
    b->pend.isRef[i] = isReference;
    b->pend.imgOut = imgOut;
    b->pend.totalWeights = totalWeights;
    b->framesSinceRef++;
    if (b->pend.n < b->group) return MFSR_OK;
    if (b->holdLastGroup && b->framesSinceRef == c.frames) return MFSR_OK;
    static const int holdGroups = [] {
        const char* e = getenv("MFSR_HOST_HOLD");
        return e ? atoi(e) : 2;
    }();
    if (b->holdLastGroup && holdGroups >= 2 && !b->heldHas && c.frames - b->framesSinceRef <= b->group &&
        c.frames - b->framesSinceRef > 0 && !b->pend.deferred[0]) {
        bool aligned = true;
        for (int j = 0; j < b->pend.n; j++) aligned = aligned && !b->pend.deferred[j];
        if (aligned) {
            b->held = b->pend;
            b->heldHas = true;
            b->pend.n = 0;
            return MFSR_OK;
        }
    }
    return accumulate_pending(b, stream);
}

extern "C" int mfsr_burst_add_frame(mfsr_burst* b, const uint16_t* raw, int isReference, mfsr_float3* imgOut,
                                    mfsr_float3* totalWeights, mfsr_stream_t stream)
{
    return add_frame_impl(b, raw, isReference, imgOut, totalWeights, false, stream);
}

extern "C" int mfsr_burst_group_size(const mfsr_config* cfg)
{
    if (!cfg || cfg->pairFrames <= 0) return 1;
    if (cfg->pairFrames >= 2) return cfg->pairFrames < MFSR_MAX_FUSE_GROUP ? cfg->pairFrames : MFSR_MAX_FUSE_GROUP;
    return ((cfg->scale == 2 || cfg->scale == 4) && !cfg->mono) ? MFSR_MAX_FUSE_GROUP : 2;
}

extern "C" int mfsr_burst_field_dims(const mfsr_burst* b, int* flowW, int* flowH, int* maskW, int* maskH)
{
    MFSR_REQUIRE(b != nullptr);
    if (flowW) *flowW = b->L.tw;
    if (flowH) *flowH = b->L.th;
    if (maskW) *maskW = b->L.hw;
    if (maskH) *maskH = b->L.hh;
    return MFSR_OK;
}

extern "C" int mfsr_burst_align_frame(mfsr_burst* b, const uint16_t* raw, int isReference, mfsr_float2* flowOut, int flowPitch,
                                      mfsr_float4* maskOut, int maskPitch, mfsr_stream_t stream)
{
    MFSR_REQUIRE(b && raw && flowOut && maskOut);
    MFSR_REQUIRE(b->haveRef);
    MFSR_REQUIRE(!b->refStale);
    const Layout& L = b->L;
    MFSR_REQUIRE((long long)flowPitch >= 8LL * L.tw && (flowPitch & 7) == 0 && ((uintptr_t)flowOut & 7) == 0);
    MFSR_REQUIRE((long long)maskPitch >= 16LL * L.hw && (maskPitch & 15) == 0 && ((uintptr_t)maskOut & 15) == 0);
    TRY(mfsr_set_cfa_pattern(b->cfg.cfa));
    const int slot = b->frameCounter++ % kRing;
    const Img *flow = nullptr, *mask = nullptr;
    TRY(align_frame(b, raw, isReference, slot, nullptr, nullptr, &flow, &mask, stream));
    b->flowCur = flow;
    b->maskCur = mask;
    MFSR_HIP_TRY(hipMemcpy2DAsync(flowOut, flowPitch, flow->ptr, flow->pitch, (size_t)L.tw * 8, L.th, hipMemcpyDeviceToDevice,
                                  mfsr_s(stream)));
    MFSR_HIP_TRY(hipMemcpy2DAsync(maskOut, maskPitch, mask->ptr, mask->pitch, (size_t)L.hw * 16, L.hh, hipMemcpyDeviceToDevice,
                                  mfsr_s(stream)));
    return MFSR_OK;
}

extern "C" int mfsr_burst_align_frames(mfsr_burst* b, int nFrames, const uint16_t* const* raws, const int* isReference,
                                       mfsr_float2* const* flowOut, int flowPitch, mfsr_float4* const* maskOut, int maskPitch,
                                       mfsr_stream_t stream)
{
    MFSR_REQUIRE(b && raws && flowOut && maskOut && nFrames >= 0);
    MFSR_REQUIRE(b->haveRef && !b->refStale);
    MFSR_REQUIRE(b->pend.n == 0);
    const Layout& L = b->L;
    MFSR_REQUIRE((long long)flowPitch >= 8LL * L.tw && (flowPitch & 7) == 0);
    MFSR_REQUIRE((long long)maskPitch >= 16LL * L.hw && (maskPitch & 15) == 0);
    for (int k = 0; k < nFrames; k++)
        MFSR_REQUIRE(raws[k] && flowOut[k] && maskOut[k] && ((uintptr_t)flowOut[k] & 7) == 0 && ((uintptr_t)maskOut[k] & 15) == 0);
    TRY(mfsr_set_cfa_pattern(b->cfg.cfa));
    const bool batch = can_defer_alignment(b, false);
    const int per = batch ? b->group : 1;
    for (int k0 = 0; k0 < nFrames; k0 += per) {
        const int n = nFrames - k0 < per ? nFrames - k0 : per;
        for (int j = 0; j < n; j++) {
            const int isRef = isReference ? isReference[k0 + j] : 0;
            const int slot = b->frameCounter++ % kRing;
            b->pend.slot[j] = slot;
            b->pend.raw[j] = raws[k0 + j];
            b->pend.isRef[j] = isRef;
            b->pend.deferred[j] = batch;
            b->pend.flow[j] = nullptr;
            b->pend.mask[j] = nullptr;
            if (!batch) {
                const int rc = align_frame(b, raws[k0 + j], isRef, slot, nullptr, nullptr, &b->pend.flow[j], &b->pend.mask[j], stream);
                if (rc) {
                    b->pend.n = 0;
                    return rc;
                }
            }
        }
        b->pend.n = n;
        const int rc = align_deferred(b, stream);
        const mfsr_burst::Pending p = b->pend;
        b->pend.n = 0;
        if (rc) return rc;
        for (int j = 0; j < n; j++) {
            b->flowCur = p.flow[j];
            b->maskCur = p.mask[j];
            MFSR_HIP_TRY(hipMemcpy2DAsync(flowOut[k0 + j], flowPitch, p.flow[j]->ptr, p.flow[j]->pitch, (size_t)L.tw * 8, L.th,
                                          hipMemcpyDeviceToDevice, mfsr_s(stream)));
            MFSR_HIP_TRY(hipMemcpy2DAsync(maskOut[k0 + j], maskPitch, p.mask[j]->ptr, p.mask[j]->pitch, (size_t)L.hw * 16, L.hh,
                                          hipMemcpyDeviceToDevice, mfsr_s(stream)));
        }
    }
    return MFSR_OK;
}

extern "C" int mfsr_burst_fuse_rows(mfsr_burst* b, int nFrames, const uint16_t* const* raws, const mfsr_float2* const* flows,
                                    int flowPitch, const mfsr_float4* const* masks, int maskPitch, mfsr_float3* imgOut,
                                    mfsr_float3* totalWeights, int accumulatorsUndefined, int rowBegin, int rowEnd,
                                    mfsr_stream_t stream)
{
    MFSR_REQUIRE(b && raws && flows && masks && imgOut && totalWeights && nFrames >= 1 && nFrames <= MFSR_MAX_FUSE_GROUP);
    MFSR_REQUIRE(b->haveRef && !b->win.on);
    TRY(wait_ref_products(b, stream));
    const mfsr_config& c = b->cfg;
    const Layout& L = b->L;
    const mfsr_float3 white = {c.white[0], c.white[1], c.white[2]};
    const mfsr_float3 black = {c.black[0], c.black[1], c.black[2]};
    TRY(mfsr_set_cfa_pattern(c.cfa));
    mfsr_tex2d sh[MFSR_MAX_FUSE_GROUP];
    for (int n = 0; n < nFrames; n++) {
        sh[n].ptr = flows[n];
        sh[n].pitch = flowPitch;
        sh[n].width = L.tw;
        sh[n].height = L.th;
    }
    const bool timed = b->timing && b->nEvents < kMaxTimedLaunches;
    if (timed) {
        const int i = b->nEvents;
        if (!b->evStart[i]) MFSR_HIP_TRY(hipEventCreate(&b->evStart[i]));
        if (!b->evStop[i]) MFSR_HIP_TRY(hipEventCreate(&b->evStop[i]));
        MFSR_HIP_TRY(hipEventRecord(b->evStart[i], mfsr_s(stream)));
    }
    TRY(mfsr_accumulateSuperResFullRows(nFrames, raws, imgOut, totalWeights, masks, as_tex(L.kparam4), sh, white, black, L.W, L.H,
                                        c.scale, 12 * L.hrW, maskPitch, accumulatorsUndefined, rowBegin, rowEnd, stream));
    if (timed) {
        MFSR_HIP_TRY(hipEventRecord(b->evStop[b->nEvents], mfsr_s(stream)));
        b->nEvents++;
        b->nFramesTimed += nFrames;
    }
    return MFSR_OK;
}

extern "C" int mfsr_dist_stripe_plan(const mfsr_config* cfg, int worldSize, int rank, int rawHalo, mfsr_stripe_plan* out)
{
    MFSR_REQUIRE(out != nullptr && worldSize >= 1 && rank >= 0 && rank < worldSize && rawHalo >= 4);
    TRY(validate(cfg));
    const int s = cfg->scale, W = cfg->width, H = cfg->height;
    const int hrH = s * H;
    const int th = cfg->mono ? H : H / 2, hh = H / 2;
    (void)W;
    auto cut = [&](int g) { return g >= worldSize ? hrH : (int)((long long)hrH * g / worldSize / 16 * 16); };
    const int r0 = cut(rank), r1 = cut(rank + 1);
    memset(out, 0, sizeof(*out));
    out->rowBegin = r0;
    out->rowEnd = r1;
    if (r1 <= r0) return MFSR_OK;
    auto rows_of = [&](int fh, int pad, int* first, int* count) {
        const int per = hrH / fh;
        int a = r0 / per - 1 - pad, b = (r1 + per - 1) / per + 1 + pad;
        if (a < 0) a = 0;
        if (b > fh) b = fh;
        *first = a;
        *count = b - a;
    };
    rows_of(th, 0, &out->flowRow0, &out->flowRows);
    rows_of(hh, 1, &out->maskRow0, &out->maskRows);
    {
        int a = r0 / s - rawHalo, b = (r1 + s - 1) / s + rawHalo;
        if (a < 0) a = 0;
        if (b > H) b = H;
        out->rawRow0 = a;
        out->rawRows = b - a;
    }
    out->maxFlowY = (float)(rawHalo - 3);
    return MFSR_OK;
}

extern "C" int mfsr_burst_begin(mfsr_burst* b, mfsr_float3* imgOut, mfsr_float3* totalWeights, mfsr_stream_t stream)
{
    MFSR_REQUIRE(b && imgOut && totalWeights);
    TRY(flush_pending(b, stream));
    memset(b->paths, 0, sizeof(b->paths));
    b->sharpenedFinishes = 0;
    b->fresh.has = true;
    b->fresh.imgOut = imgOut;
    b->fresh.totalWeights = totalWeights;
    return MFSR_OK;
}

extern "C" int mfsr_burst_flush(mfsr_burst* b, mfsr_stream_t stream)
{
    MFSR_REQUIRE(b != nullptr);
    return flush_pending(b, stream);
}

static size_t out_row_bytes(const mfsr_burst* b)
{
    return b->renderOn ? (size_t)mfsr_render_row_bytes(b->render.format, out_w(b)) : (size_t)out_w(b) * 6;
}

static bool yuv_format(int format) { return format == MFSR_OUT_NV12 || format == MFSR_OUT_P010; }
static bool yuv_on(const mfsr_burst* b) { return b->renderOn && yuv_format(b->render.format); }

static size_t out_image_bytes(const mfsr_burst* b)
{
    return b->renderOn ? (size_t)mfsr_render_image_bytes(b->render.format, out_w(b), out_h(b)) : (size_t)out_w(b) * 6 * out_h(b);
}

static int finish_rendered_rows(mfsr_burst* b, const mfsr_float3* imgOut, const mfsr_float3* totalWeights, mfsr_float3* outImg,
                                void* out, int r0, int rows, mfsr_stream_t stream)
{
    const mfsr_config& c = b->cfg;
    const Layout& L = b->L;
    const int oW = out_w(b), pitch = 12 * oW;
    const int rowBytes = (int)out_row_bytes(b);
    const size_t off = (size_t)r0 * pitch;
    const int x0 = b->win.on ? b->win.x0 : 0, y0 = b->win.on ? b->win.y0 : 0;
    if (yuv_on(b)) {
        MFSR_REQUIRE((oW & 1) == 0 && (out_h(b) & 1) == 0 && (r0 & 1) == 0 && (rows & 1) == 0);
        char* y = out ? (char*)out + (size_t)r0 * rowBytes : nullptr;
        char* uv = out ? (char*)out + ((size_t)out_h(b) + (size_t)(r0 / 2)) * rowBytes : nullptr;
        return mfsr_finishRenderedYuv((const mfsr_float3*)((const char*)imgOut + off),
                                      (const mfsr_float3*)((const char*)totalWeights + off), pitch, (const mfsr_float3*)L.fallback.ptr,
                                      L.fallback.pitch, L.W, L.H, 0.0f, 1.0f, 0.0f, 1.0f,
                                      outImg ? (mfsr_float3*)((char*)outImg + off) : nullptr, pitch, y, rowBytes, uv, rowBytes,
                                      &b->render, oW, rows, c.weightThreshold, c.applyGamma, x0, y0 + r0, L.hrW, L.hrH, stream);
    }
    return mfsr_finishRendered((const mfsr_float3*)((const char*)imgOut + off), (const mfsr_float3*)((const char*)totalWeights + off),
                               pitch, (const mfsr_float3*)L.fallback.ptr, L.fallback.pitch, L.W, L.H, 0.0f, 1.0f, 0.0f, 1.0f,
                               outImg ? (mfsr_float3*)((char*)outImg + off) : nullptr, pitch,
                               out ? (char*)out + (size_t)r0 * rowBytes : nullptr, rowBytes, &b->render, oW, rows,
                               c.weightThreshold, c.applyGamma, x0, y0 + r0, L.hrW, L.hrH, stream);
}

static int finish_sharpened_rows(mfsr_burst* b, const mfsr_float3* imgOut, const mfsr_float3* totalWeights, mfsr_float3* outImg,
                                 void* out, int r0, int rows, int rowsAbove, int rowsBelow, mfsr_stream_t stream)
{
    const mfsr_config& c = b->cfg;
    const Layout& L = b->L;
    const int oW = out_w(b), pitch = 12 * oW;
    const int rowBytes = (int)out_row_bytes(b);
    const size_t off = (size_t)r0 * pitch;
    const int x0 = b->win.on ? b->win.x0 : 0, y0 = b->win.on ? b->win.y0 : 0;
    b->sharpenedFinishes++;
    return mfsr_finishSharpened((const mfsr_float3*)((const char*)imgOut + off), (const mfsr_float3*)((const char*)totalWeights + off),
                                pitch, (const mfsr_float3*)L.fallback.ptr, L.fallback.pitch, L.W, L.H, 0.0f, 1.0f, 0.0f, 1.0f,
                                outImg ? (mfsr_float3*)((char*)outImg + off) : nullptr, pitch,
                                out ? (char*)out + (size_t)r0 * rowBytes : nullptr, rowBytes, b->renderOn ? &b->render : nullptr, oW,
                                rows, c.weightThreshold, c.applyGamma, x0, y0 + r0, L.hrW, L.hrH, &b->sharpen, rowsAbove, rowsBelow,
                                stream);
}

static void sharpen_reach(const mfsr_burst* b, int r0, int rows, int* above, int* below)
{
    const int R = b->sharpen.radius, rest = out_h(b) - r0 - rows;
    *above = R < r0 ? R : r0;
    *below = R < rest ? R : rest;
}

extern "C" int mfsr_burst_set_sharpen(mfsr_burst* b, const mfsr_sharpen* sharpen)
{
    MFSR_REQUIRE(b != nullptr);
    MFSR_REQUIRE(b->pend.n == 0 && !b->heldHas && b->nUnp == 0);
    if (!sharpen) {
        b->sharpenOn = false;
        return MFSR_OK;
    }
    TRY(mfsr_sharpen_validate(sharpen));
    const bool on = sharpen->radius != 0 && sharpen->amount != 0.0f;
    MFSR_REQUIRE(!(on && yuv_on(b)));
    b->sharpen = *sharpen;
    b->sharpenOn = on;
    return MFSR_OK;
}

extern "C" int mfsr_burst_debug_sharpened(const mfsr_burst* b, int* finishes)
{
    MFSR_REQUIRE(b && finishes);
    *finishes = b->sharpenedFinishes;
    return MFSR_OK;
}

extern "C" int mfsr_burst_set_render(mfsr_burst* b, const mfsr_render* render)
{
    MFSR_REQUIRE(b != nullptr);
    MFSR_REQUIRE(b->pend.n == 0 && !b->heldHas && b->nUnp == 0);
    if (!render) {
        b->renderOn = false;
        return MFSR_OK;
    }
    TRY(mfsr_render_validate(render));
    MFSR_REQUIRE(!(b->sharpenOn && yuv_format(render->format)));
    b->render = *render;
    b->renderOn = true;
    return MFSR_OK;
}

extern "C" int mfsr_burst_finish(mfsr_burst* b, const mfsr_float3* imgOut, const mfsr_float3* totalWeights,
                                 mfsr_float3* outImg, uint16_t* out16, mfsr_stream_t stream)
{
    MFSR_REQUIRE(b && imgOut && totalWeights && (outImg || out16));
    MFSR_REQUIRE(b->haveRef);
    TRY(flush_pending(b, stream));
    const mfsr_config& c = b->cfg;
    const Layout& L = b->L;
    const int pitch = 12 * out_w(b);
    if (b->sharpenOn) return finish_sharpened_rows(b, imgOut, totalWeights, outImg, out16, 0, out_h(b), 0, 0, stream);
    if (b->renderOn && c.fused) return finish_rendered_rows(b, imgOut, totalWeights, outImg, out16, 0, out_h(b), stream);
    if (b->renderOn) {
        MFSR_REQUIRE(outImg != nullptr);
        TRY(mfsr_resampleFloat3((const mfsr_float3*)L.fallback.ptr, L.fallback.pitch, L.W, L.H, outImg, pitch, L.hrW, L.hrH,
                                0.0f, 1.0f, 0.0f, 1.0f, stream));
        TRY(mfsr_ApplyWeighting(outImg, imgOut, totalWeights, L.hrW, L.hrH, pitch, c.weightThreshold, stream));
        if (yuv_on(b)) {
            const int rowBytes = (int)out_row_bytes(b);
            return mfsr_renderImageYuv(outImg, pitch, outImg, pitch, out16, rowBytes,
                                       out16 ? (char*)out16 + (size_t)L.hrH * rowBytes : nullptr, rowBytes, L.hrW, L.hrH, &b->render,
                                       c.applyGamma, stream);
        }
        return mfsr_renderImage(outImg, pitch, outImg, pitch, out16, (int)out_row_bytes(b), L.hrW, L.hrH, &b->render, c.applyGamma,
                                stream);
    }
    if (c.fused && b->win.on) {
        return mfsr_finishFusedWindow(imgOut, totalWeights, pitch, (const mfsr_float3*)L.fallback.ptr, L.fallback.pitch, L.W, L.H,
                                      0.0f, 1.0f, 0.0f, 1.0f, outImg, pitch, out16, b->win.w, b->win.h, c.weightThreshold,
                                      c.applyGamma, 65535.0f, b->win.x0, b->win.y0, L.hrW, L.hrH, stream);
    }
    if (c.fused) {
        return mfsr_finishFused(imgOut, totalWeights, pitch, (const mfsr_float3*)L.fallback.ptr, L.fallback.pitch, L.W, L.H,
                                0.0f, 1.0f, 0.0f, 1.0f, outImg, pitch, out16, L.hrW, L.hrH, c.weightThreshold,
                                c.applyGamma, 65535.0f, stream);
    }
    MFSR_REQUIRE(outImg != nullptr);
    TRY(mfsr_resampleFloat3((const mfsr_float3*)L.fallback.ptr, L.fallback.pitch, L.W, L.H, outImg, pitch, L.hrW, L.hrH,
                            0.0f, 1.0f, 0.0f, 1.0f, stream));
    TRY(mfsr_ApplyWeighting(outImg, imgOut, totalWeights, L.hrW, L.hrH, pitch, c.weightThreshold, stream));
    if (c.applyGamma) TRY(mfsr_GammasRGB(outImg, L.hrW, L.hrH, pitch, stream));
    if (out16) TRY(mfsr_quantize(outImg, pitch, out16, nullptr, L.hrW, L.hrH, 65535.0f, stream));
    return MFSR_OK;
// ... 147 lines not shown
            return add_frame_impl(b, b->L.rawRing[ps], isReference, imgOut, totalWeights, banded, stream);
        }
        b->nPrefetched = b->prefetchHead = 0;
    }
    const int us = b->upCounter++ % b->cfg.uploadRing;
    bool waiting = false, waitingHeld = false;
    for (int i = 0; i < b->pend.n; i++) waiting = waiting || b->pend.raw[i] == b->L.rawRing[us];
    for (int i = 0; b->heldHas && i < b->held.n; i++) waitingHeld = waitingHeld || b->held.raw[i] == b->L.rawRing[us];
    if (waiting)
        TRY(accumulate_pending(b, stream));
    else if (waitingHeld)
        TRY(fuse_held(b, stream));
    TRY(upload_into(b, us, b->L.rawRing[us], hostRaw, stream));
    return add_frame_impl(b, b->L.rawRing[us], isReference, imgOut, totalWeights, banded, stream);
}

extern "C" int mfsr_burst_prefetch_host(mfsr_burst* b, const uint16_t* const* hostRaws, int nFrames, mfsr_stream_t stream)
{
    MFSR_REQUIRE(b && hostRaws && nFrames >= 0);
    MFSR_REQUIRE(b->copyStream != nullptr);
    TRY(host_epoch(b, stream));
    b->nPrefetched = b->prefetchHead = 0;
    if (b->pend.n > 0 || b->heldHas) return MFSR_OK;
    for (int k = 0; k < nFrames && b->nPrefetched < b->cfg.uploadRing; k++) {
        MFSR_REQUIRE(hostRaws[k] != nullptr);
        if (hostRaws[k] == b->refHost && b->refDev) continue;
        const int us = b->upCounter++ % b->cfg.uploadRing;
        TRY(upload_into(b, us, b->L.rawRing[us], hostRaws[k], stream));
        b->prefetched[b->nPrefetched].host = hostRaws[k];
        b->prefetched[b->nPrefetched].slot = us;
        b->nPrefetched++;
    }
    b->upPending = false;
    return MFSR_OK;
}

static int release_ref_slot(mfsr_burst* b, mfsr_stream_t stream)
{
    if (b->refSlot >= 0) {
        TRY(record_free(b, b->refSlot, stream));
        b->refSlot = -1;
    }
    return MFSR_OK;
}

extern "C" int mfsr_burst_finish_host(mfsr_burst* b, const mfsr_float3* imgOut, const mfsr_float3* totalWeights,
                                      uint16_t* out16Dev, uint16_t* out16Host, mfsr_stream_t stream)
{
    MFSR_REQUIRE(b && imgOut && totalWeights && out16Dev && out16Host);
    MFSR_REQUIRE(b->downStream != nullptr);
    MFSR_REQUIRE(b->haveRef);
    bool capturing = false;
    TRY(host_epoch(b, stream, &capturing));
    const mfsr_config& c = b->cfg;
    const Layout& L = b->L;
    if (b->downRecorded) MFSR_HIP_TRY(hipStreamWaitEvent(mfsr_s(stream), b->evDown, 0));
    static const int nBandsEnv = [] {
        const char* e = getenv("MFSR_HOST_BANDS");
        return e ? atoi(e) : 8;
    }();
    int nBands = nBandsEnv < 1 ? 1 : (nBandsEnv > 16 ? 16 : nBandsEnv);
    static const int nBandsBusy = [] {
        const char* e = getenv("MFSR_HOST_BANDS_BUSY");
        return e ? atoi(e) : 2;
    }();
    const int oW = out_w(b), oH = out_h(b);
    const size_t rowBytes = out_row_bytes(b);
    const double outBytes = (double)out_image_bytes(b), inBytes = (double)L.W * L.H * 2.0 * c.frames;
    if (b->hostBusy && nBandsBusy >= 1 && nBandsBusy < nBands && outBytes <= 1.5 * inBytes) nBands = nBandsBusy;
    bool heldGroup = b->pend.n > 0 && b->pend.imgOut == imgOut && b->pend.totalWeights == totalWeights && c.fused;
    if (b->heldHas && !(heldGroup && b->held.imgOut == imgOut && b->held.totalWeights == totalWeights)) {
        TRY(flush_pending(b, stream));
        heldGroup = false;
    }
    if (!heldGroup) TRY(flush_pending(b, stream));
    if (nBands == 1 && !heldGroup) {
        TRY(mfsr_burst_finish(b, imgOut, totalWeights, nullptr, out16Dev, stream));
        MFSR_HIP_TRY(hipEventRecord(b->evFinished, mfsr_s(stream)));
        MFSR_HIP_TRY(hipStreamWaitEvent(b->downStream, b->evFinished, 0));
        MFSR_HIP_TRY(hipMemcpy2DAsync(out16Host, rowBytes, out16Dev, rowBytes, rowBytes, yuv_on(b) ? (size_t)oH * 3 / 2 : (size_t)oH,
                                      hipMemcpyDeviceToHost, b->downStream));
        MFSR_HIP_TRY(hipEventRecord(b->evDown, b->downStream));
        b->downRecorded = true;
        b->nUnp = 0;
        if (capturing) TRY(join_captured(b, stream));
        return release_ref_slot(b, stream);
    }
    mfsr_burst::Pending p = b->pend, p0;
    p0.n = 0;
    int freshNow = 0;
    if (heldGroup) {
        TRY(align_deferred(b, stream));
        p = b->pend;
        b->pend.n = 0;
        if (b->heldHas) {
            p0 = b->held;
            b->heldHas = false;
            b->held.n = 0;
        }
        TRY(join_fuse(b, stream));
        freshNow = b->fresh.has && b->fresh.imgOut == imgOut && b->fresh.totalWeights == totalWeights;
        if (b->fresh.has && !freshNow) {
            const size_t bytes = acc_bytes(b);
            MFSR_HIP_TRY(hipMemsetAsync(b->fresh.imgOut, 0, bytes, mfsr_s(stream)));
            MFSR_HIP_TRY(hipMemsetAsync(b->fresh.totalWeights, 0, bytes, mfsr_s(stream)));
        }
// ... 33 lines not shown
                TRY(fuse_group(b, q.n, q.raw, const_cast<mfsr_float3*>(imgOut), const_cast<mfsr_float3*>(totalWeights), masks, flows,
                               q.mask[0]->pitch, fresh, r0, r1, stream));
                fresh = 0;
            }
        }
        if (b->sharpenOn) {
            if (lagR0 >= 0) TRY(finish_lagged());
            lagI = i;
            lagR0 = r0;
            lagR1 = r1;
            continue;
        }
        const size_t off = (size_t)r0 * 12 * oW;
        const int x0 = b->win.on ? b->win.x0 : 0, y0 = b->win.on ? b->win.y0 : 0;
        if (b->renderOn) {
            TRY(finish_rendered_rows(b, imgOut, totalWeights, nullptr, out16Dev, r0, r1 - r0, stream));
        } else {
            TRY(mfsr_finishFusedWindow((const mfsr_float3*)((const char*)imgOut + off), (const mfsr_float3*)((const char*)totalWeights + off),
                                       12 * oW, (const mfsr_float3*)L.fallback.ptr, L.fallback.pitch, L.W, L.H, 0.0f, 1.0f, 0.0f, 1.0f,
                                       nullptr, 12 * oW, out16Dev + (size_t)r0 * oW * 3, oW, r1 - r0, c.weightThreshold,
                                       c.applyGamma, 65535.0f, x0, y0 + r0, L.hrW, L.hrH, stream));
        }
        if (!b->evBand[i]) MFSR_HIP_TRY(hipEventCreateWithFlags(&b->evBand[i], hipEventDisableTiming));
        MFSR_HIP_TRY(hipEventRecord(b->evBand[i], mfsr_s(stream)));
        MFSR_HIP_TRY(hipStreamWaitEvent(b->downStream, b->evBand[i], 0));
        MFSR_HIP_TRY(hipMemcpy2DAsync((char*)out16Host + (size_t)r0 * rowBytes, rowBytes, (const char*)out16Dev + (size_t)r0 * rowBytes,
                                      rowBytes, rowBytes, (size_t)(r1 - r0), hipMemcpyDeviceToHost, b->downStream));
        if (yuv_on(b)) {
            const size_t c0 = ((size_t)oH + (size_t)(r0 / 2)) * rowBytes;
            MFSR_HIP_TRY(hipMemcpy2DAsync((char*)out16Host + c0, rowBytes, (const char*)out16Dev + c0, rowBytes, rowBytes,
                                          (size_t)((r1 - r0) / 2), hipMemcpyDeviceToHost, b->downStream));
        }
    }
    if (lagR0 >= 0) TRY(finish_lagged());
    if (heldGroup && b->copyStream) {
        for (int gi = 0; gi < 2; gi++) {
            const mfsr_burst::Pending& q = gi ? p : p0;
            for (int j = 0; j < q.n; j++) {
                const int us = upload_slot_of(b, q.raw[j]);
                if (us >= 0) TRY(record_free(b, us, stream));
            }
        }
    }
    MFSR_HIP_TRY(hipEventRecord(b->evDown, b->downStream));
    b->downRecorded = true;
    b->nUnp = 0;
    if (capturing) TRY(join_captured(b, stream));
    return release_ref_slot(b, stream);
}

extern "C" int mfsr_burst_set_host_row_bytes(mfsr_burst* b, int rowBytes)
{
    MFSR_REQUIRE(b != nullptr && b->cfg.uploadRing > 0);
    MFSR_REQUIRE(b->pend.n == 0 && !b->heldHas && b->nUnp == 0);
    const bool isPacked = b->cfg.rawPacking != MFSR_PACK_NONE;
    const int dense = isPacked ? mfsr_packed_row_bytes(b->cfg.rawPacking, b->L.W) : 2 * b->L.W;
    MFSR_REQUIRE(rowBytes == 0 || rowBytes >= dense);
    MFSR_REQUIRE(isPacked || (rowBytes % 2) == 0);
    MFSR_REQUIRE(rowBytes == 0 || rowBytes == dense || !upload_1d());
    b->hostRowBytes = rowBytes;
    return MFSR_OK;
}

extern "C" int mfsr_burst_host_sync(mfsr_burst* b)
{
    MFSR_REQUIRE(b != nullptr);
    if (b->downRecorded) MFSR_HIP_TRY(hipEventSynchronize(b->evDown));
    return MFSR_OK;
}

extern "C" int mfsr_burst_process_source(mfsr_burst* b, const mfsr_frame_source* src, mfsr_float3* imgOut, mfsr_float3* totalWeights,
                                         mfsr_float3* outImg, uint16_t* out16, int* framesUsed, mfsr_stream_t stream)
{
    MFSR_REQUIRE(b && src && src->next_frame && imgOut && totalWeights && (outImg || out16));
    MFSR_REQUIRE(b->copyStream != nullptr);
    MFSR_REQUIRE(b->cfg.rawPacking == MFSR_PACK_NONE);
    MFSR_REQUIRE(b->cfg.reference == 0);
    if (framesUsed) *framesUsed = 0;
    if (src->reset) src->reset(src->user);
    TRY(mfsr_burst_begin(b, imgOut, totalWeights, stream));
    int n = 0;
    for (; n < b->cfg.frames; n++) {
        int us;
        uint16_t* dst;
        if (n == 0) {
            const int i = b->refCounter++ & 1;
            us = b->cfg.uploadRing + i;
            dst = b->L.refRaw[i];
            TRY(flush_pending(b, stream, false));
        } else {
            us = b->upCounter++ % b->cfg.uploadRing;
            dst = b->L.rawRing[us];
            for (int i = 0; i < b->pend.n; i++)
                if (b->pend.raw[i] == dst) {
                    TRY(accumulate_pending(b, stream));
                    break;
                }
        }
        if (b->freeRecorded[us]) {
            MFSR_HIP_TRY(hipStreamWaitEvent(mfsr_s(stream), b->evFree[us], 0));
            b->freeRecorded[us] = false;
        }
        const int got = src->next_frame(src->user, dst, stream);
        if (got < 0) return got;
        if (got == 0) break;
        if (n == 0) {
            b->refHost = nullptr;
// ... 207 lines not shown
    long long* sumDev = (long long*)((char*)scratchDev + sizeof(uint32_t) * MFSR_NOISE_HIST_ENTRIES);
    long long* countDev = sumDev + MFSR_NOISE_LEVEL_ENTRIES;
    TRY(mfsr_noiseStats(nFrames, frames, 2 * c.width, c.width, c.height, black, sat, r, histDev, sumDev, countDev, stream));
    std::vector<unsigned char> host(MFSR_NOISE_SCRATCH_BYTES);
    TRY(download(host.data(), scratchDev, host.size(), stream));
    const uint32_t* hist = (const uint32_t*)host.data();
    const long long* sum = (const long long*)(host.data() + sizeof(uint32_t) * MFSR_NOISE_HIST_ENTRIES);
    double a = 0, bt = 0;
    TRY(mfsr_noise_fit(hist, sum, sum + MFSR_NOISE_LEVEL_ENTRIES, black, white, minBlocks, &a, &bt, status, nullptr));
    *alpha = (float)a;
    *beta = (float)bt;
    return MFSR_OK;
}

namespace {
struct TemporalScratch {
    size_t flow0, flowBytes, mask, total;
    int tw, th, hw, hh;
};
size_t up256(size_t v) { return (v + 255) / 256 * 256; }
bool temporal_scratch(const mfsr_config* cfg, int nFrames, TemporalScratch* s)
{
    if (cfg == nullptr || nFrames < 2 || nFrames > 64 || validate(cfg) != MFSR_OK) return false;
    s->hw = cfg->width / 2;
    s->hh = cfg->height / 2;
    s->tw = cfg->mono ? cfg->width : s->hw;
    s->th = cfg->mono ? cfg->height : s->hh;
    s->flow0 = up256(MFSR_NOISE_SCRATCH_BYTES);
    s->flowBytes = up256((size_t)8 * s->tw * s->th);
    s->mask = s->flow0 + (size_t)(nFrames - 1) * s->flowBytes;
    s->total = s->mask + up256((size_t)16 * s->hw * s->hh);
    return true;
}
}

extern "C" size_t mfsr_noise_temporal_scratch_bytes(const mfsr_config* cfg, int nFrames)
{
    TemporalScratch s;
    return temporal_scratch(cfg, nFrames, &s) ? s.total : 0;
}

extern "C" int mfsr_burst_calibrate_noise_temporal(mfsr_burst* b, int nFrames, const uint16_t* const* frames, int reference, float tol,
                                                   int minBlocks, void* scratchDev, size_t scratchBytes, double* alpha, double* beta,
                                                   int32_t* status, int32_t* points, long long* blocks, mfsr_stream_t stream)
{
    MFSR_REQUIRE(b && frames && scratchDev && alpha && beta && status);
    MFSR_REQUIRE(nFrames >= 2 && nFrames <= 64 && reference >= 0 && reference < nFrames);
    MFSR_REQUIRE(!(tol > 0.25f) && tol == tol);
    for (int k = 0; k < nFrames; k++) MFSR_REQUIRE(frames[k] != nullptr && ((uintptr_t)frames[k] & 1) == 0);
    const mfsr_config& c = b->cfg;
    TemporalScratch s;
    MFSR_REQUIRE(temporal_scratch(&c, nFrames, &s));
    MFSR_REQUIRE(((uintptr_t)scratchDev & 255) == 0 && scratchBytes >= s.total);
    if (b->pend.n > 0 || b->heldHas || b->nUnp != 0) {
        fprintf(stderr, "mfsr: mfsr_burst_calibrate_noise_temporal with frames pending (flush or finish the burst first)\n");
        return MFSR_E_INVALID;
    }
    int32_t black[4], sat = 0, defBlocks = 0, r[4];
    float white[4];
    TRY(mfsr_noise_defaults(&c, black, white, &sat, &defBlocks, r));
    const float useTol = tol > 0.0f ? tol : 0.0625f;
    const int useBlocks = minBlocks > 0 ? minBlocks : defBlocks;

    TRY(flush_pending(b, stream));
    memset(b->paths, 0, sizeof(b->paths));
    b->sharpenedFinishes = 0;
    TRY(mfsr_burst_set_reference(b, frames[reference], stream));

    char* base = (char*)scratchDev;
    const uint16_t* moved[64];
    const mfsr_float2* flows[64];
    mfsr_float2* flowOut[64];
    mfsr_float4* maskOut[64];
    int m = 0;
    for (int k = 0; k < nFrames; k++) {
        if (k == reference) {
            flows[k] = nullptr;
            continue;
        }
        moved[m] = frames[k];
        flowOut[m] = (mfsr_float2*)(base + s.flow0 + (size_t)m * s.flowBytes);
        maskOut[m] = (mfsr_float4*)(base + s.mask);
        flows[k] = flowOut[m];
        m++;
    }
    TRY(mfsr_burst_align_frames(b, m, moved, nullptr, flowOut, 8 * s.tw, maskOut, 16 * s.hw, stream));
    uint32_t* histDev = (uint32_t*)base;
    long long* sumDev = (long long*)(base + sizeof(uint32_t) * MFSR_NOISE_HIST_ENTRIES);
    long long* countDev = sumDev + MFSR_NOISE_LEVEL_ENTRIES;
    TRY(mfsr_noiseStatsTemporal(nFrames, frames, 2 * c.width, c.width, c.height, flows, 8 * s.tw, s.tw, s.th, black, sat, r, useTol,
                                histDev, sumDev, countDev, stream));
    std::vector<unsigned char> host(MFSR_NOISE_SCRATCH_BYTES);
    TRY(download(host.data(), scratchDev, host.size(), stream));
    const uint32_t* hist = (const uint32_t*)host.data();
    const long long* sum = (const long long*)(host.data() + sizeof(uint32_t) * MFSR_NOISE_HIST_ENTRIES);
    const long long* count = sum + MFSR_NOISE_LEVEL_ENTRIES;
    TRY(mfsr_noise_fit_temporal(hist, sum, count, black, white, useBlocks, alpha, beta, status, points));
    if (blocks) {
        long long n = 0;
        for (int l = 0; l < 64; l++) n += count[l];
        *blocks = n;
    }
    return MFSR_OK;
}

extern "C" int mfsr_burst_debug_views(mfsr_burst* b, mfsr_tex2d* flow, mfsr_tex2d* mask, mfsr_tex2d* kernelParam,
                                      mfsr_tex2d* tracking)
{
    MFSR_REQUIRE(b != nullptr);
    if ((flow || mask) && b->pend.n > 0 && b->pend.deferred[b->pend.n - 1]) return MFSR_E_INVALID;
    if (flow) *flow = as_tex(*b->flowCur);
    if (mask) *mask = as_tex(*b->maskCur);
    if (kernelParam) *kernelParam = as_tex(b->L.kparam4);
    if (tracking) *tracking = as_tex(b->ref.pyr[0]);
    return MFSR_OK;
}

extern "C" int mfsr_burst_debug_paths(const mfsr_burst* b, int32_t* counts, int capacity, int* count)
{
    MFSR_REQUIRE(b && counts && count && capacity >= 0);
    const int n = capacity < (int)MFSR_PATH_COUNT ? capacity : (int)MFSR_PATH_COUNT;
    for (int i = 0; i < n; i++) counts[i] = b->paths[i];
    *count = (int)MFSR_PATH_COUNT;
    return MFSR_OK;
}

extern "C" int mfsr_burst_debug_frame_views(mfsr_burst* b, int framesBack, mfsr_tex2d* flow, mfsr_tex2d* mask)
{
    MFSR_REQUIRE(b != nullptr && framesBack >= 0 && framesBack < kRing && framesBack < b->frameCounter);
    const int slot = (int)((b->frameCounter - 1 - framesBack) % kRing);
    MFSR_REQUIRE(b->slotFlow[slot] != nullptr);
    if (flow) *flow = as_tex(*b->slotFlow[slot]);
    if (mask) *mask = as_tex(b->L.maskBuf[slot]);
    return MFSR_OK;
}

extern "C" int mfsr_burst_prealign_result(mfsr_burst* b, mfsr_prealign* hostOut, mfsr_stream_t stream)
{
    MFSR_REQUIRE(b && hostOut);
    MFSR_REQUIRE(b->cfg.preAlign && b->preCur);
    TRY(align_deferred(b, stream));
    MFSR_HIP_TRY(hipMemcpyAsync(hostOut, b->preCur, sizeof(*hostOut), hipMemcpyDeviceToHost, mfsr_s(stream)));
    MFSR_HIP_TRY(hipStreamSynchronize(mfsr_s(stream)));
    return MFSR_OK;
}

namespace {
struct StreamLayout {
    size_t burstWs, accBytes, entryBytes;
    size_t offBurst, offImg, offTw, offEntries, total;
};
size_t stream_entry(const mfsr_config* c, char* base, FrameProducts* fp)
{
    const Layout L = make_layout(c, nullptr);
    Bump b{base, 0};
    const int nl = ilog2(L.maxFactor) + 1;
    FrameProducts tmp;
    memset((void*)&tmp, 0, sizeof(tmp));
    tmp.raw = (uint16_t*)b.take((size_t)L.W * L.H * 2);
    tmp.half = b.image(L.hw, L.hh, 12);
    for (int i = 0; i < nl; i++) tmp.pyr[i] = b.image(L.tw >> i, L.th >> i, 4);
    tmp.prePyr = c->preAlign ? b.take(mfsr_preAlign_pyramid_bytes(L.tw, L.th)) : nullptr;
    if (fp) *fp = tmp;
    return align_up(b.off, 256);
}
int stream_layout(const mfsr_config* c, int radius, StreamLayout* S)
{
    memset(S, 0, sizeof(*S));
    const Layout L = make_layout(c, nullptr);
    S->burstWs = L.total;
    S->accBytes = (size_t)12 * L.hrW * L.hrH;
    S->entryBytes = stream_entry(c, nullptr, nullptr);
    size_t off = 0;
    S->offBurst = off;
    off = align_up(off + S->burstWs, 256);
    S->offImg = off;
    off = align_up(off + S->accBytes, 256);
    S->offTw = off;
    off = align_up(off + S->accBytes, 256);
    S->offEntries = off;
    off += S->entryBytes * (size_t)(2 * radius + 1);
    S->total = align_up(off, 256);
    return MFSR_OK;
// ... 398 lines not shown
```

multi_frame_super_resolution_amd/pipeline.py:

```python
from __future__ import annotations

import ctypes
from collections import namedtuple
from typing import Iterable, Optional, Sequence, Tuple

import torch

from . import capi


def default_config(width: int, height: int, frames: int, scale: int = 2, mono: bool = False) -> capi.Config:
    cfg = capi.Config()
    capi.lib().config_default(ctypes.byref(cfg), width, height, frames, scale, 1 if mono else 0)
    return cfg


WINDOW_GRID = 16


def align_window(cfg: capi.Config, x: int, y: int, w: int, h: int) -> Tuple[int, int, int, int]:
    hr_w, hr_h = cfg.width * cfg.scale, cfg.height * cfg.scale
    if w <= 0 or h <= 0:
        raise ValueError("window must not be empty")
    x1, y1 = min(x + w, hr_w), min(y + h, hr_h)
# ... 581 lines not shown

def sharpen_image(img: torch.Tensor, amount: float = 1.0, sigma: float = 1.0, radius: int = 0, threshold: float = 0.0, taps=None,
                  format: Optional[int] = None, matrix=None, tone_lut=None, apply_gamma: bool = False, want_float: bool = True):
    if not (img.is_cuda and img.dtype == torch.float32 and img.dim() == 3 and img.shape[2] == 3 and img.stride(2) == 1
            and img.stride(1) == 3):
        raise ValueError("img: a float32 device tensor [h, w, 3] with dense pixels")
    s = _sharpen_struct(amount, sigma, radius, threshold, taps)
    if s is None or s.radius == 0 or s.amount == 0:
        raise ValueError("sharpen_image: amount and radius must not be 0")
    h, w = int(img.shape[0]), int(img.shape[1])
    with torch.cuda.device(img.device):
        r, lut, out = None, None, None
        if format is not None:
            r, lut = _render_struct(format, matrix, tone_lut, img.device)
            out = _render_buffer(format, h, w, img.device)
        fl = torch.empty(h, w, 3, dtype=torch.float32, device=img.device) if (want_float or out is None) else None
        capi.lib().sharpenImage(img.data_ptr(), img.stride(0) * 4, None if fl is None else fl.data_ptr(), 12 * w,
                                None if out is None else out.data_ptr(), 0 if out is None else render_row_bytes(format, w), w, h,
                                ctypes.byref(s), None if r is None else ctypes.byref(r), 1 if apply_gamma else 0,
                                torch.cuda.current_stream().cuda_stream)
        del lut
    if out is None:
        return fl
    return (out, fl) if want_float else out


class BurstPipeline:

    def __init__(self, cfg: capi.Config, device: Optional[torch.device] = None, window: Optional[Sequence[int]] = None):
        if not torch.cuda.is_available():
            raise RuntimeError("multi_frame_super_resolution_amd needs a HIP device (MI355X); there is no CPU fallback")
        self.L = capi.lib()
        self.cfg = cfg
        self.window = _Window(cfg, window)
        self.device = torch.device("cuda", torch.cuda.current_device()) if device is None else torch.device(device)
        nbytes = self.L.burst_workspace_bytes(ctypes.byref(cfg))
        if nbytes == 0:
            raise ValueError("invalid mfsr_config")
        with torch.cuda.device(self.device):
            self.workspace = torch.empty(nbytes + 256, dtype=torch.uint8, device=self.device)
            base = self.workspace.data_ptr()
            self._ws_ptr = (base + 255) // 256 * 256
            self.hr_w, self.hr_h = cfg.width * cfg.scale, cfg.height * cfg.scale
            out_h, out_w = self.window.aligned[3], self.window.aligned[2]
            self._img_out = torch.zeros(out_h, out_w, 3, dtype=torch.float32, device=self.device)
            self._total_weights = torch.zeros_like(self._img_out)
            self.out_img = torch.empty_like(self._img_out)
            self.out16 = torch.empty(out_h, out_w, 3, dtype=torch.int16, device=self.device)
            self._fmt = capi.OUT_RGB16
            handle = ctypes.c_void_p()
            self.L.burst_create(ctypes.byref(handle), ctypes.byref(cfg), self._ws_ptr, nbytes)
            self._h = handle
            self.window.apply(self.L.burst_set_window, self._h)

    def close(self):
        if getattr(self, "_h", None):
            self.L.burst_destroy(self._h)
            self._h = None

    def __del__(self):
        try:
            self.close()
        except Exception:
            pass

    @staticmethod
    def _stream() -> int:
        return torch.cuda.current_stream().cuda_stream

    def set_render(self, format: Optional[int] = capi.OUT_RGB16, matrix=None, tone_lut=None, yuv: int = 0):
        if format is not None:
            self.window.check_yuv(int(format))
        out_h, out_w = self.window.aligned[3], self.window.aligned[2]
        with torch.cuda.device(self.device):
            if format is None:
                self.L.burst_set_render(self._h, None)
                self._render_lut, fmt = None, capi.OUT_RGB16
            else:
                r, lut = _render_struct(format, matrix, tone_lut, self.device, yuv)
                self.L.burst_set_render(self._h, ctypes.byref(r))
                self._render_lut, fmt = lut, int(format)
            self.out16 = _render_buffer(fmt, out_h, out_w, self.device)
            self._out16_host = None
            self._fmt = fmt

    def set_sharpen(self, amount: Optional[float] = None, sigma: float = 1.0, radius: int = 0, threshold: float = 0.0, taps=None):
        s = _sharpen_struct(amount, sigma, radius, threshold, taps)
        on = s is not None and s.radius != 0 and s.amount != 0
        with torch.cuda.device(self.device):
            self.L.burst_set_sharpen(self._h, None if s is None else ctypes.byref(s))
            if self.window.grow(WINDOW_GRID if on else 0):
                self.L.burst_set_window(self._h, *self.window.aligned)
                out_h, out_w = self.window.aligned[3], self.window.aligned[2]
                self._img_out = torch.zeros(out_h, out_w, 3, dtype=torch.float32, device=self.device)
                self._total_weights = torch.zeros_like(self._img_out)
                self.out_img = torch.empty_like(self._img_out)
                self.out16 = _render_buffer(self._fmt, out_h, out_w, self.device)
                self._out16_host = None

    def sharpened_finishes(self) -> int:
        n = ctypes.c_int(-1)
        self.L.burst_debug_sharpened(self._h, ctypes.byref(n))
        return n.value

    def flush(self):
        self.L.burst_flush(self._h, self._stream())

    @property
    def img_out(self) -> torch.Tensor:
        self.flush()
        return self._img_out

    @property
    def total_weights(self) -> torch.Tensor:
        self.flush()
        return self._total_weights

    def reset_accumulators(self):
        self.flush()
        self._img_out.zero_()
        self._total_weights.zero_()

    def begin_burst(self):
        self.L.burst_begin(self._h, self._img_out.data_ptr(), self._total_weights.data_ptr(), self._stream())

    def set_reference(self, raw: torch.Tensor):
        self._check_raw(raw)
        self.L.burst_set_reference(self._h, raw.data_ptr(), self._stream())

    def add_frame(self, raw: torch.Tensor, is_reference: bool = False):
        self._check_raw(raw)
        self.L.burst_add_frame(self._h, raw.data_ptr(), 1 if is_reference else 0, self._img_out.data_ptr(),
                               self._total_weights.data_ptr(), self._stream())

    def finish(self, want_float: bool = True, want_u16: bool = True):
        self.L.burst_finish(self._h, self._img_out.data_ptr(), self._total_weights.data_ptr(),
                            self.out_img.data_ptr() if want_float else None,
                            self.out16.data_ptr() if want_u16 else None, self._stream())
        return self.window(self.out_img if want_float else None), self.window.output(self.out16 if want_u16 else None, self._fmt)

    def finish_rows(self, row0: int, rows: int) -> torch.Tensor:
        self.L.burst_finish_rows(self._h, self._img_out.data_ptr(), self._total_weights.data_ptr(), None,
                                 self.out16.data_ptr(), row0, rows, self._stream())
        return self.out16

    def _checked(self, frames: Sequence[torch.Tensor], clone: bool):
        for f in frames:
            self._check_raw(f)
        return [f.clone() for f in frames] if clone else list(frames)

    def _repair(self, work, threshold: Optional[int], spread: int, min_votes: Optional[int]):
        n = len(work)
        t0, _, v0 = defect_defaults(self.cfg, n)
        self.defect_map = torch.empty(self.cfg.height, self.cfg.width, dtype=torch.uint8, device=self.device)
        counts_dev = torch.empty(2, dtype=torch.int32, device=self.device)
        counts = (ctypes.c_uint32 * 2)()
        self.L.burst_repair_defects(self._h, n, _ptr_table(work), t0 if threshold is None else int(threshold), int(spread),
                                    v0 if min_votes is None else int(min_votes), self.defect_map.data_ptr(),
                                    counts_dev.data_ptr(), counts, self._stream())
        self.defects = (int(counts[0]), int(counts[1]))

    def _shade(self, work, gain_map: torch.Tensor, cell: Optional[int]):
        cell = _shading_map(gain_map, self.cfg, cell, self.device)
        self.L.burst_correct_shading(self._h, len(work), _ptr_table(work), gain_map.data_ptr(), cell, self._stream())

    def _select(self, work, candidates: int, keep_ratio: float):
        n = len(work)
        sums_dev = torch.empty(n, dtype=torch.int64, device=self.device)
        ref, keep = ctypes.c_int(-1), (ctypes.c_int32 * n)()
        sums, rect = (ctypes.c_longlong * n)(), (ctypes.c_int32 * 4)()
        self.L.burst_select_frames(self._h, n, _ptr_table(work), int(candidates), float(keep_ratio), sums_dev.data_ptr(),
                                   ctypes.byref(ref), keep, sums, rect, self._stream())
        r = ref.value
        kept = [k for k in range(n) if keep[k]]
        self.selection = Selection(r, kept, list(sums), tuple(rect))
        return r, kept

    def _match(self, work, r: int, per_colour: bool, deadband: Optional[int], min_gain: Optional[int], max_gain: Optional[int]):
        n = len(work)
        d = exposure_defaults(self.cfg)
        levels_dev = torch.empty(n, 5, dtype=torch.int64, device=self.device)
        gains, status, levels = (ctypes.c_int32 * (3 * n))(), (ctypes.c_int32 * n)(), (ctypes.c_longlong * (5 * n))()
        self.L.burst_match_exposure(self._h, n, _ptr_table(work), r, 1 if per_colour else 0,
                                    d.deadband if deadband is None else int(deadband),
                                    d.min_gain if min_gain is None else int(min_gain),
                                    d.max_gain if max_gain is None else int(max_gain), levels_dev.data_ptr(), gains, status, levels,
                                    self._stream())
        q16 = [[int(gains[3 * k + c]) for c in range(3)] for k in range(n)]
        self.exposure = Exposure(r, [[g / 65536.0 for g in row] for row in q16], [int(s) for s in status],
                                 [[int(levels[5 * k + i]) for i in range(5)] for k in range(n)], q16)

    def calibrate_noise(self, frames: Sequence[torch.Tensor], reference: int = 0, tol: Optional[float] = None,
                        min_blocks: Optional[int] = None):
        frames = self._checked(frames, clone=False)
        n = len(frames)
        nbytes = self.L.noise_temporal_scratch_bytes(ctypes.byref(self.cfg), n)
# ... 252 lines not shown
```

Measured before the change: 23420.

## Fuse multiple 4-frame accumulate groups into one burst tile kernel launch

Adds a burst accumulation kernel that loops over up to four 4-frame groups per tile, keeping the HR accumulator tile resident in LDS across groups instead of reloading and storing it for each group launch. The burst object now holds aligned groups and fuses them at flush, finish, or when the ring fills, and the Python wrapper enables holding by default while keeping raw frames alive. This is meant to cut accumulator global memory traffic and launch count, at the cost of extra frame-slot ring capacity, more complex hold and flush state, and an extra barrier plus field restaging per group.

```diff
diff --git a/include/mfsr.h b/include/mfsr.h
--- a/include/mfsr.h
+++ b/include/mfsr.h
@@ -10,6 +10,7 @@
 
 #define MFSR_VERSION 100
 #define MFSR_MAX_FUSE_GROUP 4
+#define MFSR_MAX_BURST_FUSE 16
 
 typedef void* mfsr_stream_t;
 
@@ -82,6 +83,11 @@
                                       mfsr_float3 whiteLevel, mfsr_float3 blackLevel, int dimX, int dimY, int scale,
                                       int strideOut, int strideMask, int accumulatorsUndefined, int x0, int y0, int w, int h,
                                       mfsr_stream_t stream);
+
+int mfsr_accumulateSuperResBurst(int nFrames, const uint16_t* const* dataIn, mfsr_tex2d imgOut, mfsr_tex2d totalWeights,
+                                 const mfsr_tex2d* certaintyMasks, mfsr_tex2d kernelParam, const mfsr_tex2d* shifts,
+                                 mfsr_float3 whiteLevel, mfsr_float3 blackLevel, int scale, int accumulatorsUndefined,
+                                 mfsr_stream_t stream);
 
 int mfsr_squaredSum(const float* inTiles, float* outValues, int maxShift, int tileSize, int tileCount,
                     mfsr_stream_t stream);
@@ -377,6 +383,9 @@
                          mfsr_float3* totalWeights, mfsr_stream_t stream);
 int mfsr_burst_begin(mfsr_burst* b, mfsr_float3* imgOut, mfsr_float3* totalWeights, mfsr_stream_t stream);
 int mfsr_burst_flush(mfsr_burst* b, mfsr_stream_t stream);
+int mfsr_burst_hold_fuse(mfsr_burst* b, int enable);
+int mfsr_burst_fuse_stats(const mfsr_burst* b, int* burstLaunches, int* groupsFused);
+int mfsr_set_burst_fuse(int enable);
 int mfsr_burst_finish(mfsr_burst* b, const mfsr_float3* imgOut, const mfsr_float3* totalWeights, mfsr_float3* outImg,
                       uint16_t* out16, mfsr_stream_t stream);
 int mfsr_burst_finish_rows(mfsr_burst* b, const mfsr_float3* imgOut, const mfsr_float3* totalWeights,
diff --git a/multi_frame_super_resolution_amd/csrc/accumulate.hip b/multi_frame_super_resolution_amd/csrc/accumulate.hip
--- a/multi_frame_super_resolution_amd/csrc/accumulate.hip
+++ b/multi_frame_super_resolution_amd/csrc/accumulate.hip
@@ -91,6 +91,12 @@
                                       mfsr_float3 blackLevel, int dimX, int dimY, int strideOut, int strideMask,
                                       int fresh, int rowBegin, int rowEnd, int colBegin, int colEnd, int relative,
                                       mfsr_stream_t stream);
+
+int mfsr_try_launch_accumulate2x_burst(int nFrames, const uint16_t* const* dataIn, mfsr_float3* imgOut,
+                                       mfsr_float3* totalWeights, const mfsr_float4* const* certaintyMask,
+                                       mfsr_tex2d kernelParam, const mfsr_tex2d* shifts, mfsr_float3 whiteLevel,
+                                       mfsr_float3 blackLevel, int dimX, int dimY, int strideOut, int strideMask, int fresh,
+                                       mfsr_stream_t stream);
 
 static int check_superres_args(const uint16_t* dataIn, mfsr_float3* imgOut, mfsr_float3* totalWeights,
                                const mfsr_float4* certaintyMask, const mfsr_tex2d& kernelParam, const mfsr_tex2d& shifts,
@@ -302,3 +308,31 @@
                                            blackLevel, dimX, dimY, scale, strideOut, strideMask, accumulatorsUndefined, 0,
                                            scale * dimY, stream);
 }
+
+extern "C" int mfsr_accumulateSuperResBurst(int nFrames, const uint16_t* const* dataIn, mfsr_tex2d imgOut, mfsr_tex2d totalWeights,
+                                            const mfsr_tex2d* certaintyMasks, mfsr_tex2d kernelParam, const mfsr_tex2d* shifts,
+                                            mfsr_float3 whiteLevel, mfsr_float3 blackLevel, int scale, int accumulatorsUndefined,
+                                            mfsr_stream_t stream)
+{
+    MFSR_REQUIRE(dataIn && certaintyMasks && shifts);
+    MFSR_REQUIRE(nFrames >= 2 * MFSR_MAX_FUSE_GROUP && nFrames <= MFSR_MAX_BURST_FUSE && (nFrames % MFSR_MAX_FUSE_GROUP) == 0);
+    MFSR_REQUIRE(scale >= 1 && scale <= 8);
+    MFSR_REQUIRE(imgOut.width > 0 && imgOut.height > 0 && (imgOut.width % scale) == 0 && (imgOut.height % scale) == 0);
+    MFSR_REQUIRE(totalWeights.width == imgOut.width && totalWeights.height == imgOut.height && totalWeights.pitch == imgOut.pitch);
+    const int dimX = imgOut.width / scale, dimY = imgOut.height / scale;
+    const mfsr_float4* masks[MFSR_MAX_BURST_FUSE];
+    for (int n = 0; n < nFrames; n++) {
+        MFSR_REQUIRE(certaintyMasks[n].width == (dimX + 1) / 2 && certaintyMasks[n].height == (dimY + 1) / 2 &&
+                     certaintyMasks[n].pitch == certaintyMasks[0].pitch);
+        masks[n] = (const mfsr_float4*)certaintyMasks[n].ptr;
+        const int rc = check_superres_args(dataIn[n], (mfsr_float3*)imgOut.ptr, (mfsr_float3*)totalWeights.ptr, masks[n], kernelParam,
+                                           shifts[n], dimX, dimY, dimX * scale, imgOut.pitch, certaintyMasks[0].pitch);
+        if (rc) return rc;
+    }
+    if (g_accumulate_fast != 2 || scale != 2) return MFSR_E_UNSUPPORTED;
+    const int r = mfsr_try_launch_accumulate2x_burst(nFrames, dataIn, (mfsr_float3*)imgOut.ptr, (mfsr_float3*)totalWeights.ptr, masks,
+                                                     kernelParam, shifts, whiteLevel, blackLevel, dimX, dimY, imgOut.pitch,
+                                                     certaintyMasks[0].pitch, accumulatorsUndefined ? 1 : 0, stream);
+    if (r == 1) return mfsr_launch_status("accumulateSuperResBurst");
+    return r < 0 ? MFSR_E_INVALID : MFSR_E_UNSUPPORTED;
+}
diff --git a/multi_frame_super_resolution_amd/csrc/accumulate_fast.hip b/multi_frame_super_resolution_amd/csrc/accumulate_fast.hip
--- a/multi_frame_super_resolution_amd/csrc/accumulate_fast.hip
+++ b/multi_frame_super_resolution_amd/csrc/accumulate_fast.hip
@@ -1044,6 +1044,386 @@
         add_plane(0, accW);
         if (safeBits != (1u << NF) - 1u) slow_frames(No{}, Yes{}, 0, 0);
         store_plane(0, gW);
+    }
+}
+
+#define TILE_BURST_GROUPS 4
+struct BurstFrames {
+    TileFrame f[4 * TILE_BURST_GROUPS];
+};
+
+template <int CFA>
+__global__ void __launch_bounds__(256, 3)
+    k_accumulate2xTileBurst(BurstFrames fr, int nGroups, pix3* __restrict__ imgOut, pix3* __restrict__ totalWeights, mfsr_tex2d kernelParam,
+                            Levels3 glv, StripLevels lv, int dimX, int dimY, int strideOut, int strideMask, int cfaPacked, int tilesX,
+                            int tilesY, int tilesPerXcd, int fresh)
+{
+    constexpr int NF = 4, FC = TILE_COLS, FROWS = 3;
+    const int pid = (int)blockIdx.x;
+    const int tile = tilesPerXcd > 0 ? (pid & 7) * tilesPerXcd + (pid >> 3) : pid;
+    if (tile >= tilesX * tilesY) return;
+    const int bIdY = tile / tilesX, bIdX = tile - bIdY * tilesX;
+    __shared__ __attribute__((aligned(16))) float4 sAcc[2][4][192];
+    __shared__ float4 sK[FROWS][FC];
+    __shared__ float2 sF[NF][FROWS][FC];
+    __shared__ __attribute__((aligned(16))) float sMp[4][3][NF][TILE_COLS];
+    constexpr int EP = 3 * NF * TILE_COLS * 4;
+    __shared__ uint32_t sUnsat[3][TILE_COLS];
+    __shared__ __attribute__((aligned(16))) float sColA[256];
+    __shared__ float sRowB[4];
+    const int lx = threadIdx.x, ly = threadIdx.y;
+    const int t = ly * 64 + lx;
+    const int tx = bIdX * 64 + lx;
+    const int Y = bIdY * 4 + ly;
+    const int hrW = 2 * dimX, hrH = 2 * dimY;
+    const int X0 = 4 * tx;
+    const int fw = kernelParam.width, fh = kernelParam.height;
+    const int mw = dimX / 2, mh = dimY / 2;
+    auto stage_fields = [&](int g) {
+        if (t < 3 * TILE_COLS) {
+            const int r = t / TILE_COLS, c = t - r * TILE_COLS;
+            const int gy = bIdY - 1 + r, gx = bIdX * 64 - 1 + c;
+            const int fy = clampi(gy, 0, fh - 1), fx = clampi(gx, 0, fw - 1);
+            uint32_t unsat = 0;
+#pragma unroll
+            for (int n = 0; n < NF; n++) {
+                const TileFrame& F = fr.f[4 * g + n];
+                sF[n][r][c] = row_ptr((const float2*)F.shifts.ptr, F.shifts.pitch, fy)[fx];
+                const float4 m = row_ptr(F.mask, strideMask, clampi(gy, 0, mh - 1))[clampi(gx, 0, mw - 1)];
+                const float mc[3] = {sane(m.x), sane(m.y), sane(m.z)};
+                sMp[0][r][n][c] = mc[Cfa<CFA>::col(0, 0)];
+                sMp[1][r][n][c] = mc[Cfa<CFA>::col(0, 1)];
+                sMp[2][r][n][c] = mc[Cfa<CFA>::col(1, 0)];
+                sMp[3][r][n][c] = mc[Cfa<CFA>::col(1, 1)];
+                if (!(mc[0] == 1.0f && mc[1] == 1.0f && mc[2] == 1.0f)) unsat |= 1u << n;
+            }
+            sUnsat[r][c] = unsat;
+        }
+    };
+    if (t < 3 * TILE_COLS) {
+        const int r = t / TILE_COLS, c = t - r * TILE_COLS;
+        const int fy = clampi(bIdY - 1 + r, 0, fh - 1), fx = clampi(bIdX * 64 - 1 + c, 0, fw - 1);
+        float4 k = row_ptr((const float4*)kernelParam.ptr, kernelParam.pitch, fy)[fx];
+        k.w = psd_ok(k.x, k.y, k.z) ? 1.0f : 0.0f;
+        sK[r][c] = k;
+    }
+    stage_fields(0);
+    {
+        const int X = bIdX * 256 + t;
+        const float posX = ((float)X + 0.5f) / (float)hrW;
+        float xB = posX * (float)fw - 0.5f;
+        if (!finitef(xB)) xB = 0.0f;
+        const float fxf = floorf(xB);
+        const int txc = X >> 2, ci = (t & 3) < 2 ? 0 : 1;
+        const bool ok = (f2i(fxf) == txc - 1 + ci) && (txc + ci <= fw - 1);
+        sColA[t] = ok ? xB - fxf : -1.0f;
+    }
+    if (t < 4) {
+        const int Yr = bIdY * 4 + t;
+        const float posY = ((float)Yr + 0.5f) / (float)hrH;
+        float yB = posY * (float)fh - 0.5f;
+        if (!finitef(yB)) yB = 0.0f;
+        const float fyf = floorf(yB);
+        const int frr = t < 2 ? 0 : 1;
+        const bool ok = (f2i(fyf) == bIdY - 1 + frr) && f2i(fyf) >= 0 && f2i(fyf) + 1 <= fh - 1;
+        sRowB[t] = ok ? yB - fyf : -1.0f;
+    }
+    const bool rowLive = Y >= STRIP_MARGIN && Y < hrH - STRIP_MARGIN;
+    const size_t rowBytes = (size_t)hrW * 12;
+    const size_t segByte = (size_t)bIdX * 3072;
+    char* gP = (char*)imgOut + (size_t)Y * strideOut + segByte;
+    char* gW = (char*)totalWeights + (size_t)Y * strideOut + segByte;
+    auto stage_plane = [&](char* g, int pl) {
+#pragma unroll
+        for (int j = 0; j < 3; j++) {
+            if (fresh) {
+                sAcc[pl][ly][j * 64 + lx] = make_float4(0.0f, 0.0f, 0.0f, 0.0f);
+            } else {
+                const size_t off = (size_t)(j * 64 + lx) * 16;
+                if (segByte + off + 16 <= rowBytes)
+                    __builtin_amdgcn_global_load_lds((const __attribute__((address_space(1))) void*)(g + off),
+                                                     (__attribute__((address_space(3))) void*)&sAcc[pl][ly][j * 64], 16, 0, 0);
+            }
+        }
+    };
+    if (rowLive) {
+        stage_plane(gP, 0);
+        stage_plane(gW, 1);
+    }
+    __syncthreads();
+    if (!rowLive) return;
+    const bool stripLive = X0 >= STRIP_MARGIN && X0 < hrW - STRIP_MARGIN;
+
+    const int fr_ = ly < 2 ? 0 : 1;
+    auto ciOf = [](int k) { return k < 2 ? 0 : 1; };
+    const float b0 = sRowB[ly];
+    const float4 av4 = ((const float4*)sColA)[lx];
+    const bool geomOk = stripLive && b0 >= 0.0f && fminf(fminf(av4.x, av4.y), fminf(av4.z, av4.w)) >= 0.0f;
+
+    float kxa[4], kya[4], kza[4];
+    bool kOk;
+    {
+        const float av[4] = {av4.x, av4.y, av4.z, av4.w}, b = b0;
+        float4 Kt[2][3];
+#pragma unroll
+        for (int r = 0; r < 2; r++)
+#pragma unroll
+            for (int c = 0; c < 3; c++) Kt[r][c] = sK[fr_ + r][lx + c];
+        const float kAll = ((Kt[0][0].w * Kt[0][1].w) * (Kt[0][2].w * Kt[1][0].w)) * (Kt[1][1].w * Kt[1][2].w);
+        kOk = kAll > 0.0f;
+#pragma unroll
+        for (int k = 0; k < 4; k++) {
+            const int ci = ciOf(k);
+            const float w00 = (1.0f - av[k]) * (1.0f - b), w10 = av[k] * (1.0f - b), w01 = (1.0f - av[k]) * b, w11 = av[k] * b;
+            auto mix = [&](float t00, float t10, float t01, float t11) {
+                return __builtin_fmaf(w11, t11, __builtin_fmaf(w01, t01, __builtin_fmaf(w10, t10, w00 * t00)));
+            };
+            kxa[k] = mix(Kt[0][ci].x, Kt[0][ci + 1].x, Kt[1][ci].x, Kt[1][ci + 1].x);
+            kya[k] = mix(Kt[0][ci].y, Kt[0][ci + 1].y, Kt[1][ci].y, Kt[1][ci + 1].y);
+            kza[k] = mix(Kt[0][ci].z, Kt[0][ci + 1].z, Kt[1][ci].z, Kt[1][ci + 1].z);
+        }
+    }
+    const uint32_t xmax = (uint32_t)(2 * dimX - 5), ymax = (uint32_t)(2 * dimY - 5);
+    typedef const __attribute__((address_space(3))) char* lds_cptr;
+    typedef const __attribute__((address_space(1))) char* glb_cptr;
+    uint32_t mrowA[5];
+#pragma unroll
+    for (int jt = 0; jt < 5; jt++) {
+        mrowA[jt] = (uint32_t)(uintptr_t)(lds_cptr)&sMp[0][((ly + jt - 2) >> 2) + 1][0][lx];
+        asm volatile("" : "+v"(mrowA[jt]));
+    }
+    const uint32_t rawPitch = (uint32_t)dimX * 2u;
+    float* const myP = (float*)&sAcc[0][ly][0] + lx * 12;
+    float* const myW = (float*)&sAcc[1][ly][0] + lx * 12;
+
+#pragma unroll 1
+    for (int g = 0; g < nGroups; g++) {
+        if (g > 0) {
+            __syncthreads();
+            stage_fields(g);
+            __syncthreads();
+        }
+#pragma unroll
+        for (int k = 0; k < 4; k++) asm volatile("" : "+v"(kxa[k]), "+v"(kya[k]), "+v"(kza[k]));
+        float av[4] = {av4.x, av4.y, av4.z, av4.w};
+        float b = b0;
+#pragma unroll
+        for (int k = 0; k < 4; k++) asm volatile("" : "+v"(av[k]));
+        asm volatile("" : "+v"(b));
+        uint32_t safeBits = 0;
+        uint32_t sxy[NF][2];
+        int bsx[NF], bsy[NF];
+#pragma unroll
+        for (int n = 0; n < NF; n++) {
+            sxy[n][0] = sxy[n][1] = 0u;
+            const float2 cf = sF[n][1][FC / 2];
+            bsx[n] = __builtin_amdgcn_readfirstlane(min(max(round2i(cf.x * 2.0f), -32000), 32000));
+            bsy[n] = __builtin_amdgcn_readfirstlane(min(max(round2i(cf.y * 2.0f), -32000), 32000));
+            float2 Ft[2][3];
+#pragma unroll
+            for (int r = 0; r < 2; r++)
+#pragma unroll
+                for (int c = 0; c < 3; c++) Ft[r][c] = sF[n][fr_ + r][lx + c];
+            bool safe = geomOk && kOk;
+#pragma unroll
+            for (int k = 0; k < 4; k++) {
+                const int ci = ciOf(k);
+                const float ux = lerp4(Ft[0][ci].x, Ft[0][ci + 1].x, Ft[1][ci].x, Ft[1][ci + 1].x, av[k], b);
+                const float uy = lerp4(Ft[0][ci].y, Ft[0][ci + 1].y, Ft[1][ci].y, Ft[1][ci + 1].y, av[k], b);
+                const int sx = round2i(ux * 2.0f), sy = round2i(uy * 2.0f);
+                const int qx = X0 + k + sx - 2, qy = Y + sy - 2;
+                safe = safe && (uint32_t)qx <= xmax && (uint32_t)qy <= ymax;
+                const uint32_t dx = (uint32_t)sx - (uint32_t)bsx[n], dy = (uint32_t)sy - (uint32_t)bsy[n];
+                safe = safe && dx + 128u < 256u && dy + 128u < 256u;
+                sxy[n][0] |= (dx & 0xffu) << (8 * k);
+                sxy[n][1] |= (dy & 0xffu) << (8 * k);
+            }
+            if (safe) safeBits |= 1u << n;
+        }
+        glb_cptr rawBase[NF];
+#pragma unroll
+        for (int n = 0; n < NF; n++) {
+            rawBase[n] = (glb_cptr)fr.f[4 * g + n].raw;
+            asm volatile("" : "+s"(rawBase[n]));
+        }
+        uint32_t satW = 0;
+        {
+            const int r0 = ((ly - 2) >> 2) + 1;
+            uint32_t u = sUnsat[r0][lx] | sUnsat[r0 + 1][lx];
+            if (lx < 2) u |= sUnsat[r0][64 + lx] | sUnsat[r0 + 1][64 + lx];
+#pragma unroll
+            for (int n = 0; n < NF; n++)
+                if (__builtin_amdgcn_ballot_w64((u >> n) & 1u) == 0) satW |= 1u << n;
+            satW = (uint32_t)__builtin_amdgcn_readfirstlane((int)satW);
+        }
+        float accW[12];
+#pragma unroll
+        for (int i = 0; i < 12; i++) accW[i] = 0.0f;
+        auto pixel = [&](auto kc) {
+            constexpr int k = decltype(kc)::value;
+            if (safeBits == 0) return;
+            float aP[12];
+            aP[3 * k] = aP[3 * k + 1] = aP[3 * k + 2] = 0.0f;
+            float w[13];
+            tap_weights13(kxa[k], kya[k], kza[k], w);
+            float P[3][4];
+            if (satW) tap_pair_sums(w, P);
+#pragma unroll
+            for (int n = 0; n < NF; n++) {
+                if ((safeBits >> n) & 1u) {
+                    auto rawf = [&](int x0, int y0, float (&sv)[3][3]) {
+                        const uint32_t boff = (uint32_t)(y0 * dimX + x0) * 2u;
+#pragma unroll
+                        for (int j = 0; j < 3; j++) {
+                            uint32_t off = boff + (uint32_t)j * rawPitch;
+                            asm volatile("" : "+v"(off));
+                            glb_cptr rb = rawBase[n] + off;
+#pragma unroll
+                            for (int i = 0; i < 3; i++) sv[j][i] = (float)*(const __attribute__((address_space(1))) uint16_t*)(rb + 2 * i);
+                        }
+                    };
+                    auto mval = [&](int jt, int cell, auto... e) {
+                        return *(const __attribute__((address_space(3))) float*)(uintptr_t)((mrowA[jt] + ... + e) +
+                                                                                             (uint32_t)(n * TILE_COLS + cell) * 4u);
+                    };
+                    const int sx = bsx[n] + (int)(int8_t)(sxy[n][0] >> (8 * k));
+                    const int sy = bsy[n] + (int)(int8_t)(sxy[n][1] >> (8 * k));
+                    if ((satW >> n) & 1u)
+                        strip_pixel_sat<k, CFA>(X0 + k, Y, sx, sy, w, P, rawf, lv, aP, accW);
+                    else
+                        strip_pixel_w<k, CFA, EP>(X0 + k, Y, sx, sy, w, rawf, mval, lv, aP, accW);
+                }
+            }
+            if (k == 0) asm volatile("s_waitcnt vmcnt(0)" ::: "memory");
+            myP[3 * k] += aP[3 * k];
+            myP[3 * k + 1] += aP[3 * k + 1];
+            myP[3 * k + 2] += aP[3 * k + 2];
+        };
+        pixel(std::integral_constant<int, 0>{});
+        pixel(std::integral_constant<int, 1>{});
+        pixel(std::integral_constant<int, 2>{});
+        pixel(std::integral_constant<int, 3>{});
+        asm volatile("s_waitcnt vmcnt(0)" ::: "memory");
+        {
+            float4* my = (float4*)myW;
+#pragma unroll
+            for (int j = 0; j < 3; j++) {
+                float4 a = my[j];
+                a.x += accW[4 * j + 0]; a.y += accW[4 * j + 1]; a.z += accW[4 * j + 2]; a.w += accW[4 * j + 3];
+                my[j] = a;
+            }
+        }
+        if (safeBits != (1u << NF) - 1u && stripLive) {
+#pragma unroll 1
+            for (int n = 0; n < NF; n++) {
+                if ((safeBits >> n) & 1u) continue;
+                const TileFrame F = fr.f[4 * g + n];
+#pragma unroll 1
+                for (int k = 0; k < 4; k++) {
+                    const int X = X0 + k;
+                    if (X >= 1 && X < hrW - 1) {
+                        pix3 px = {myP[3 * k], myP[3 * k + 1], myP[3 * k + 2]};
+                        pix3 tw = {myW[3 * k], myW[3 * k + 1], myW[3 * k + 2]};
+                        accumulate_pixel_core<GEOM_FULL, true>(X, Y, F.raw, F.mask, kernelParam, F.shifts, glv, dimX, dimY, 2, strideMask,
+                                                               cfaPacked, px, tw);
+                        myP[3 * k] = px.x; myP[3 * k + 1] = px.y; myP[3 * k + 2] = px.z;
+                        myW[3 * k] = tw.x; myW[3 * k + 1] = tw.y; myW[3 * k + 2] = tw.z;
+                    }
+                }
+            }
+        }
+    }
+    int Yw = Y;
+    asm volatile("" : "+v"(Yw));
+    auto store_plane = [&](int pl, pix3* base) {
+        char* g = (char*)base + (size_t)Yw * strideOut + segByte;
+        asm volatile("s_waitcnt lgkmcnt(0)" ::: "memory");
+#pragma unroll
+        for (int j = 0; j < 3; j++) {
+            const size_t off = (size_t)(j * 64 + lx) * 16;
+            const size_t gb = segByte + off;
+            const bool sideMargin = gb < (size_t)STRIP_MARGIN * 12 || gb + 16 > rowBytes - (size_t)STRIP_MARGIN * 12;
+            if (gb + 16 <= rowBytes && (fresh || !sideMargin)) *(float4*)(g + off) = sAcc[pl][ly][j * 64 + lx];
+        }
+    };
+    store_plane(0, imgOut);
+    store_plane(1, totalWeights);
+}
+
+#ifndef MARGIN_BURST_LOOP
+#define MARGIN_BURST_LOOP 1
+#endif
+template <int SCALE>
+__global__ void __launch_bounds__(256, 4)
+    k_accumulateMarginBurst(BurstFrames fr, int nGroups, pix3* __restrict__ imgOut, pix3* __restrict__ totalWeights, mfsr_tex2d kernelParam,
+                            Levels3 glv, int dimX, int dimY, int strideOut, int strideMask, int cfaPacked)
+{
+    constexpr int scale = SCALE, NF = 4;
+    __shared__ float sSum[NF][6][64];
+    const int hrW = scale * dimX, hrH = scale * dimY, M = STRIP_MARGIN;
+    const int rowLen = hrW - 2;
+    const int nTop = (M - 1) * rowLen, nBot = (M - 1) * rowLen;
+    const int sideLen = 2 * (M - 1);
+    const int nSide = (hrH - 2 * M) * sideLen;
+    const int lane = threadIdx.x, n = threadIdx.y;
+    const int idx = blockIdx.x * 64 + lane;
+    int x = 0, y = -1;
+    if (idx < nTop) {
+        y = 1 + idx / rowLen;
+        x = 1 + idx % rowLen;
+    } else if (idx < nTop + nBot) {
+        const int r = idx - nTop;
+        y = hrH - M + r / rowLen;
+        x = 1 + r % rowLen;
+    } else if (idx < nTop + nBot + nSide) {
+        const int r = idx - nTop - nBot;
+        y = M + r / sideLen;
+        const int c = r % sideLen;
+        x = c < M - 1 ? 1 + c : hrW - M + (c - (M - 1));
+    }
+    const bool live = y >= 0;
+    const bool first = n == 0 && live;
+    pix3 a = {0.0f, 0.0f, 0.0f}, w = {0.0f, 0.0f, 0.0f};
+    if (first) {
+        a = row_ptr(imgOut, strideOut, y)[x];
+        w = row_ptr(totalWeights, strideOut, y)[x];
+    }
+#pragma unroll 1
+    for (int g = 0; g < nGroups; g++) {
+        pix3 pixel = {0.0f, 0.0f, 0.0f}, totalWeight = {0.0f, 0.0f, 0.0f};
+        int xg = x, yg = y;
+        asm volatile("" : "+v"(xg), "+v"(yg));
+        if (live) {
+            TileFrame F = fr.f[4 * g];
+#pragma unroll
+            for (int m = 1; m < NF; m++)
+                if (n == m) F = fr.f[4 * g + m];
+            accumulate_pixel_core<GEOM_FULL, true, MARGIN_TAP_SUMS>(xg, yg, F.raw, F.mask, kernelParam, F.shifts, glv, dimX, dimY, scale,
+                                                                    strideMask, cfaPacked, pixel, totalWeight);
+        }
+        sSum[n][0][lane] = pixel.x;
+        sSum[n][1][lane] = pixel.y;
+        sSum[n][2][lane] = pixel.z;
+        sSum[n][3][lane] = totalWeight.x;
+        sSum[n][4][lane] = totalWeight.y;
+        sSum[n][5][lane] = totalWeight.z;
+        __syncthreads();
+        if (first) {
+#pragma unroll
+            for (int m = 0; m < NF; m++) {
+                a.x += sSum[m][0][lane];
+                a.y += sSum[m][1][lane];
+                a.z += sSum[m][2][lane];
+                w.x += sSum[m][3][lane];
+                w.y += sSum[m][4][lane];
+                w.z += sSum[m][5][lane];
+            }
+        }
+        __syncthreads();
+    }
+    if (first) {
+        row_ptr(imgOut, strideOut, y)[x] = a;
+        row_ptr(totalWeights, strideOut, y)[x] = w;
     }
 }
 
@@ -1777,6 +2157,87 @@
     return 0;
 }
 
+int mfsr_try_launch_accumulate2x_burst(int nFrames, const uint16_t* const* dataIn, mfsr_float3* imgOut,
+                                       mfsr_float3* totalWeights, const mfsr_float4* const* certaintyMask,
+                                       mfsr_tex2d kernelParam, const mfsr_tex2d* shifts, mfsr_float3 whiteLevel,
+                                       mfsr_float3 blackLevel, int dimX, int dimY, int strideOut, int strideMask, int fresh,
+                                       mfsr_stream_t stream)
+{
+    read_env_once();
+    if (nFrames < 8 || nFrames > 4 * TILE_BURST_GROUPS || (nFrames & 3)) return 0;
+    int cfa[4];
+    mfsr_get_cfa_pattern(cfa);
+    const int packed2 = pack_cfa(cfa[0], cfa[1], cfa[2], cfa[3]);
+    if ((dimX & 1) || ((uintptr_t)imgOut & 15) || ((uintptr_t)totalWeights & 15) || (strideOut & 15)) return 0;
+    if (dimX < 2 * STRIP_MARGIN || dimY < 2 * STRIP_MARGIN) return 0;
+    for (int n = 0; n < nFrames; n++)
+        if (!tile_kernel_ok(kernelParam, shifts[n], dimX, dimY)) return 0;
+    Levels3 glv;
+    StripLevels lv;
+    const float wl[3] = {whiteLevel.x, whiteLevel.y, whiteLevel.z}, bl[3] = {blackLevel.x, blackLevel.y, blackLevel.z};
+    for (int c = 0; c < 3; c++) {
+        glv.white[c] = wl[c];
+        glv.black[c] = bl[c];
+        lv.black[c] = bl[c];
+        lv.invWhite[c] = 1.0f / wl[c];
+    }
+    const int hrW = 2 * dimX, hrH = 2 * dimY;
+    const HrWindow whole{0, 0, hrW, hrH, 0};
+    const WinLaunch wlc = win_launch(whole, hrW, 256);
+    const MarginRects mr = margin_rects(hrW, hrH, STRIP_MARGIN, whole);
+    const int tilesX = wlc.tilesX, tilesY = mfsr_cdiv(hrH, 4);
+    const int tilesPerXcd = g_strip_xcd_remap ? mfsr_cdiv(tilesX * tilesY, 8) : 0;
+    const dim3 block(64, 4), g1(tilesPerXcd ? 8 * tilesPerXcd : tilesX * tilesY);
+    hipStream_t st = mfsr_s(stream);
+    pix3* pI = (pix3*)imgOut;
+    pix3* pT = (pix3*)totalWeights;
+    const int cp = mfsr_cfa_packed();
+    BurstFrames fr;
+    for (int n = 0; n < 4 * TILE_BURST_GROUPS; n++) {
+        const int m = n < nFrames ? n : 0;
+        fr.f[n].raw = dataIn[m];
+        fr.f[n].mask = (const float4*)certaintyMask[m];
+        fr.f[n].shifts = shifts[m];
+    }
+    auto launch = [&](auto cfaTag) {
+        constexpr int CFA = decltype(cfaTag)::value;
+        if (fresh && zero_margin_bands(imgOut, totalWeights, hrH, strideOut, 0, hrH, wlc, st) != 0) return -1;
+        hipLaunchKernelGGL((k_accumulate2xTileBurst<CFA>), g1, block, 0, st, fr, nFrames / 4, pI, pT, kernelParam, glv, lv, dimX, dimY,
+                           strideOut, strideMask, cp, tilesX, tilesY, tilesPerXcd, fresh ? 1 : 0);
+        return 1;
+    };
+    auto margin = [&](auto nfTag) {
+        constexpr int NF = decltype(nfTag)::value;
+        TileFrames<NF> mf;
+        for (int n = 0; n < NF; n++) mf.f[n] = fr.f[n];
+        launch_margin_n<NF, 2>(st, mf, pI, pT, kernelParam, glv, dimX, dimY, strideOut, strideMask, cp, 0, hrH, wlc, mr);
+    };
+    int rc = 0;
+#define BURST_CASE(a, b, c, d)                                                      \
+    case pack_cfa(a, b, c, d):                                                      \
+        rc = launch(std::integral_constant<int, pack_cfa(a, b, c, d)>{});           \
+        break;
+    switch (packed2) {
+        BURST_CASE(MFSR_RED, MFSR_GREEN, MFSR_GREEN, MFSR_BLUE)
+        BURST_CASE(MFSR_BLUE, MFSR_GREEN, MFSR_GREEN, MFSR_RED)
+        BURST_CASE(MFSR_GREEN, MFSR_RED, MFSR_BLUE, MFSR_GREEN)
+        BURST_CASE(MFSR_GREEN, MFSR_BLUE, MFSR_RED, MFSR_GREEN)
+        default: break;
+    }
+#undef BURST_CASE
+    if (rc != 1) return rc;
+    if (MARGIN_BURST_LOOP) {
+        const long long cnt = 2LL * (STRIP_MARGIN - 1) * (hrW - 2) + (long long)(hrH - 2 * STRIP_MARGIN) * 2 * (STRIP_MARGIN - 1);
+        hipLaunchKernelGGL((k_accumulateMarginBurst<2>), dim3(mfsr_cdiv(cnt, 64)), dim3(64, 4), 0, st, fr, nFrames / 4, pI, pT, kernelParam,
+                           glv, dimX, dimY, strideOut, strideMask, cp);
+        return 1;
+    }
+    if (nFrames == 8) margin(std::integral_constant<int, 8>{});
+    if (nFrames == 12) margin(std::integral_constant<int, 12>{});
+    if (nFrames == 16) margin(std::integral_constant<int, 16>{});
+    return 1;
+}
+
 int mfsr_try_launch_accumulate4x_tile(int nFrames, const uint16_t* const* dataIn, mfsr_float3* imgOut,
                                       mfsr_float3* totalWeights, const mfsr_float4* const* certaintyMask,
                                       mfsr_tex2d kernelParam, const mfsr_tex2d* shifts, mfsr_float3 whiteLevel,
diff --git a/multi_frame_super_resolution_amd/csrc/pipeline.cpp b/multi_frame_super_resolution_amd/csrc/pipeline.cpp
--- a/multi_frame_super_resolution_amd/csrc/pipeline.cpp
+++ b/multi_frame_super_resolution_amd/csrc/pipeline.cpp
@@ -14,6 +14,8 @@
 constexpr int kMaxLevels = 4;
 constexpr int kMaxTimedLaunches = 4096;
 constexpr int kRing = 2 * MFSR_MAX_FUSE_GROUP;
+constexpr int kRingMax = MFSR_MAX_BURST_FUSE;
+inline int ring_size(const mfsr_config* c) { return c->frames <= kRing ? kRing : (c->frames < kRingMax ? c->frames : kRingMax); }
 constexpr int kMaxUploadRing = 32;
 
 inline size_t align_up(size_t v, size_t a) { return (v + a - 1) / a * a; }
@@ -50,8 +52,8 @@
     Img tensor, tensorTmp, tensorSm;
     Img fallback;
     Img tmpA, tmpB;
-    Img flowBuf[2 * kRing];
-    Img maskBuf[kRing];
+    Img flowBuf[2 * kRingMax];
+    Img maskBuf[kRingMax];
     Img maskRaw[MFSR_MAX_FUSE_GROUP];
     Img pre[kMaxLevels];
     Img warped, Ix, Iy, It, rawf;
@@ -227,6 +229,11 @@
     if (c->rawPacking != MFSR_PACK_NONE)
         for (int i = 0; i < c->uploadRing + 2; i++)
             L->stage[i] = (uint8_t*)b.take((size_t)mfsr_packed_row_bytes(c->rawPacking, L->W) * L->H);
+    for (int i = kRing; i < ring_size(c); i++) {
+        L->flowBuf[2 * i] = b.image(L->tw, L->th, 8);
+        L->flowBuf[2 * i + 1] = b.image(L->tw, L->th, 8);
+        L->maskBuf[i] = b.image(L->hw, L->hh, 16);
+    }
     L->total = align_up(b.off, 256);
     return layout;
 }
@@ -270,6 +277,10 @@
     Pending held;
     bool heldHas;
     int group;
+    bool holdFuse;
+    int nHold;
+    Pending hold[MFSR_MAX_BURST_FUSE / MFSR_MAX_FUSE_GROUP];
+    int burstLaunches, burstGroups;
     int nFramesTimed;
     struct Fresh {
         bool has;
@@ -277,12 +288,13 @@
     } fresh;
     int frameCounter;
     hipStream_t fuseStream;
-    hipEvent_t evAligned[kRing];
-    hipEvent_t evFused[kRing];
+    int ring;
+    hipEvent_t evAligned[kRingMax];
+    hipEvent_t evFused[kRingMax];
     hipEvent_t evRefStart, evRefDone;
     bool refOnFuse;
-    bool fusedOutstanding[kRing];
-    const Img* slotFlow[kRing];
+    bool fusedOutstanding[kRingMax];
+    const Img* slotFlow[kRingMax];
     hipStream_t copyStream;
     hipStream_t downStream;
     hipEvent_t evFinished, evDown;
@@ -325,6 +337,7 @@
     bool timing;
     int nEvents;
     hipEvent_t evStart[kMaxTimedLaunches], evStop[kMaxTimedLaunches];
+    unsigned char evLaunches[kMaxTimedLaunches];
     int32_t paths[MFSR_PATH_COUNT];
 };
 
@@ -450,6 +463,10 @@
     b->ref = b->L.ref;
     b->pend.n = 0;
     b->group = mfsr_burst_group_size(&b->cfg);
+    b->ring = ring_size(&b->cfg);
+    b->holdFuse = false;
+    b->nHold = 0;
+    b->burstLaunches = b->burstGroups = 0;
     b->fresh.has = false;
     b->nFramesTimed = 0;
     b->timing = false;
@@ -460,7 +477,7 @@
     b->fuseStream = nullptr;
     b->evRefStart = b->evRefDone = nullptr;
     b->refOnFuse = false;
-    for (int i = 0; i < kRing; i++) {
+    for (int i = 0; i < kRingMax; i++) {
         b->evAligned[i] = b->evFused[i] = nullptr;
         b->fusedOutstanding[i] = false;
         b->slotFlow[i] = nullptr;
@@ -476,7 +493,7 @@
         if (e == hipSuccess) e = hipStreamCreateWithPriority(&b->fuseStream, hipStreamNonBlocking, prio);
         if (e == hipSuccess) e = hipEventCreateWithFlags(&b->evRefStart, hipEventDisableTiming);
         if (e == hipSuccess) e = hipEventCreateWithFlags(&b->evRefDone, hipEventDisableTiming);
-        for (int i = 0; i < kRing && e == hipSuccess; i++) {
+        for (int i = 0; i < b->ring && e == hipSuccess; i++) {
             e = hipEventCreateWithFlags(&b->evAligned[i], hipEventDisableTiming);
             if (e == hipSuccess) e = hipEventCreateWithFlags(&b->evFused[i], hipEventDisableTiming);
         }
@@ -544,7 +561,7 @@
         if (b->evStop[i]) (void)hipEventDestroy(b->evStop[i]);
     }
     if (b->fuseStream) (void)hipStreamSynchronize(b->fuseStream);
-    for (int i = 0; i < kRing; i++) {
+    for (int i = 0; i < kRingMax; i++) {
         if (b->evAligned[i]) (void)hipEventDestroy(b->evAligned[i]);
         if (b->evFused[i]) (void)hipEventDestroy(b->evFused[i]);
     }
@@ -581,14 +598,16 @@
 {
     MFSR_REQUIRE(b && totalMs && launches && frames);
     double total = 0;
+    int nLaunches = 0;
     for (int i = 0; i < b->nEvents; i++) {
         MFSR_HIP_TRY(hipEventSynchronize(b->evStop[i]));
         float ms = 0;
         MFSR_HIP_TRY(hipEventElapsedTime(&ms, b->evStart[i], b->evStop[i]));
         total += ms;
+        nLaunches += b->evLaunches[i];
     }
     *totalMs = total;
-    *launches = b->nEvents;
+    *launches = nLaunches;
     *frames = b->nFramesTimed;
     b->nEvents = 0;
     b->nFramesTimed = 0;
@@ -825,7 +844,7 @@
     MFSR_REQUIRE(b != nullptr);
     const int rc = mfsr_window_check(&b->cfg, x0, y0, w, h);
     if (rc != MFSR_OK) return rc;
-    if (b->pend.n > 0 || b->heldHas) {
+    if (b->pend.n > 0 || b->heldHas || b->nHold > 0) {
         fprintf(stderr, "mfsr: mfsr_burst_set_window with frames pending (flush or finish the burst first)\n");
         return MFSR_E_INVALID;
     }
@@ -931,6 +950,121 @@
 
 static int accumulate_pending(mfsr_burst* b, mfsr_stream_t callerStream);
 
+static int g_burst_fuse = -1;
+static bool burst_fuse_enabled()
+{
+    if (g_burst_fuse < 0) {
+        const char* e = getenv("MFSR_BURST_FUSE");
+        g_burst_fuse = (e && e[0] == '0') ? 0 : 1;
+    }
+    return g_burst_fuse == 1;
+}
+extern "C" int mfsr_set_burst_fuse(int enable)
+{
+    g_burst_fuse = enable ? 1 : 0;
+    return MFSR_OK;
+}
+extern "C" int mfsr_burst_hold_fuse(mfsr_burst* b, int enable)
+{
+    MFSR_REQUIRE(b != nullptr);
+    b->holdFuse = enable != 0;
+    return MFSR_OK;
+}
+extern "C" int mfsr_burst_fuse_stats(const mfsr_burst* b, int* burstLaunches, int* groupsFused)
+{
+    MFSR_REQUIRE(b && burstLaunches && groupsFused);
+    *burstLaunches = b->burstLaunches;
+    *groupsFused = b->burstGroups;
+    return MFSR_OK;
+}
+
+static bool can_hold_group(const mfsr_burst* b, bool hostBurst)
+{
+    const mfsr_config& c = b->cfg;
+    if (!b->holdFuse || !burst_fuse_enabled() || hostBurst || b->heldHas || b->fuseStream || b->win.on) return false;
+    if (!c.fused || c.mono || c.scale != 2 || b->group != MFSR_MAX_FUSE_GROUP || b->pend.n != MFSR_MAX_FUSE_GROUP) return false;
+    if (b->L.tw * 2 != b->L.W || b->L.th * 2 != b->L.H) return false;
+    if (b->nHold >= MFSR_MAX_BURST_FUSE / MFSR_MAX_FUSE_GROUP) return false;
+    if (b->nHold > 0 && (b->hold[0].imgOut != b->pend.imgOut || b->hold[0].totalWeights != b->pend.totalWeights)) return false;
+    for (int i = 0; i < b->pend.n; i++)
+        if (upload_slot_of(b, b->pend.raw[i]) >= 0) return false;
+    return true;
+}
+
+static int accumulate_pending(mfsr_burst* b, mfsr_stream_t callerStream);
+
+static int fuse_hold(mfsr_burst* b, mfsr_stream_t stream)
+{
+    const int G = b->nHold;
+    if (G == 0) return MFSR_OK;
+    b->nHold = 0;
+    const mfsr_config& c = b->cfg;
+    const Layout& L = b->L;
+    int rc = MFSR_E_UNSUPPORTED;
+    if (G >= 2) {
+        const uint16_t* raws[MFSR_MAX_BURST_FUSE];
+        mfsr_tex2d masks[MFSR_MAX_BURST_FUSE], flows[MFSR_MAX_BURST_FUSE];
+        for (int g = 0; g < G; g++)
+            for (int i = 0; i < MFSR_MAX_FUSE_GROUP; i++) {
+                const int k = g * MFSR_MAX_FUSE_GROUP + i;
+                raws[k] = b->hold[g].raw[i];
+                masks[k] = as_tex(*b->hold[g].mask[i]);
+                flows[k] = as_tex(*b->hold[g].flow[i]);
+            }
+        mfsr_float3* imgOut = b->hold[0].imgOut;
+        mfsr_float3* totalWeights = b->hold[0].totalWeights;
+        mfsr_tex2d acc[2];
+        for (int p = 0; p < 2; p++) {
+            acc[p].ptr = p ? (void*)totalWeights : (void*)imgOut;
+            acc[p].pitch = 12 * L.hrW;
+            acc[p].width = L.hrW;
+            acc[p].height = L.hrH;
+        }
+        TRY(mfsr_set_cfa_pattern(c.cfa));
+        const int freshNow = b->fresh.has && b->fresh.imgOut == imgOut && b->fresh.totalWeights == totalWeights;
+        const bool timed = b->timing && b->nEvents < kMaxTimedLaunches;
+        if (timed) {
+            const int i = b->nEvents;
+            if (!b->evStart[i]) MFSR_HIP_TRY(hipEventCreate(&b->evStart[i]));
+            if (!b->evStop[i]) MFSR_HIP_TRY(hipEventCreate(&b->evStop[i]));
+            MFSR_HIP_TRY(hipEventRecord(b->evStart[i], mfsr_s(stream)));
+        }
+        const mfsr_float3 white = {c.white[0], c.white[1], c.white[2]};
+        const mfsr_float3 black = {c.black[0], c.black[1], c.black[2]};
+        rc = mfsr_accumulateSuperResBurst(G * MFSR_MAX_FUSE_GROUP, raws, acc[0], acc[1], masks, as_tex(L.kparam4), flows, white, black,
+                                          c.scale, freshNow, stream);
+        if (rc == MFSR_OK) {
+            if (b->fresh.has && !freshNow) {
+                const size_t bytes = acc_bytes(b);
+                MFSR_HIP_TRY(hipMemsetAsync(b->fresh.imgOut, 0, bytes, mfsr_s(stream)));
+                MFSR_HIP_TRY(hipMemsetAsync(b->fresh.totalWeights, 0, bytes, mfsr_s(stream)));
+            }
+            b->fresh.has = false;
+            b->burstLaunches++;
+            b->burstGroups += G;
+            if (timed) {
+                MFSR_HIP_TRY(hipEventRecord(b->evStop[b->nEvents], mfsr_s(stream)));
+                b->evLaunches[b->nEvents] = G;
+                b->nEvents++;
+                b->nFramesTimed += G * MFSR_MAX_FUSE_GROUP;
+            }
+            return MFSR_OK;
+        }
+        if (rc != MFSR_E_UNSUPPORTED) return rc;
+    }
+    const mfsr_burst::Pending later = b->pend;
+    for (int g = 0; g < G; g++) {
+        b->pend = b->hold[g];
+        const int rc1 = accumulate_pending(b, stream);
+        if (rc1 != MFSR_OK) {
+            b->pend = later;
+            return rc1;
+        }
+    }
+    b->pend = later;
+    return MFSR_OK;
+}
+
 static int fuse_held(mfsr_burst* b, mfsr_stream_t callerStream)
 {
     if (!b->heldHas) return MFSR_OK;
@@ -945,6 +1079,7 @@
 
 static int accumulate_pending(mfsr_burst* b, mfsr_stream_t callerStream)
 {
+    TRY(fuse_hold(b, callerStream));
     TRY(fuse_held(b, callerStream));
     TRY(align_deferred(b, callerStream));
     TRY(wait_uploads(b, callerStream));
@@ -986,6 +1121,7 @@
     }
     if (timed) {
         MFSR_HIP_TRY(hipEventRecord(b->evStop[b->nEvents], mfsr_s(stream)));
+        b->evLaunches[b->nEvents] = 1;
         b->nEvents++;
         b->nFramesTimed += n;
     }
@@ -1014,7 +1150,7 @@
 {
     if (!b->fuseStream) return MFSR_OK;
     TRY(wait_ref_products(b, stream));
-    for (int i = 0; i < kRing; i++)
+    for (int i = 0; i < b->ring; i++)
         if (b->fusedOutstanding[i]) {
             MFSR_HIP_TRY(hipStreamWaitEvent(mfsr_s(stream), b->evFused[i], 0));
             b->fusedOutstanding[i] = false;
@@ -1024,7 +1160,7 @@
 
 static int flush_pending(mfsr_burst* b, mfsr_stream_t stream, bool materializeFresh)
 {
-    if (materializeFresh && b->fresh.has && b->pend.n == 0 && !b->heldHas) {
+    if (materializeFresh && b->fresh.has && b->pend.n == 0 && !b->heldHas && b->nHold == 0) {
         const size_t bytes = acc_bytes(b);
         MFSR_HIP_TRY(hipMemsetAsync(b->fresh.imgOut, 0, bytes, mfsr_s(stream)));
         MFSR_HIP_TRY(hipMemsetAsync(b->fresh.totalWeights, 0, bytes, mfsr_s(stream)));
@@ -1406,9 +1542,12 @@
     TRY(mfsr_set_cfa_pattern(c.cfa));
     b->holdLastGroup = hostBurst;
     if (b->pend.n && (b->pend.imgOut != imgOut || b->pend.totalWeights != totalWeights)) TRY(flush_pending(b, stream));
+    if (b->nHold && (b->hold[0].imgOut != imgOut || b->hold[0].totalWeights != totalWeights ||
+                     b->nHold * MFSR_MAX_FUSE_GROUP + b->pend.n >= b->ring))
+        TRY(fuse_hold(b, stream));
     if (b->pend.n >= b->group) TRY(accumulate_pending(b, stream));
     MFSR_REQUIRE(b->pend.n < MFSR_MAX_FUSE_GROUP);
-    const int slot = b->frameCounter++ % kRing;
+    const int slot = b->frameCounter++ % b->ring;
     const Img *flow = nullptr, *mask = nullptr;
     const bool defer = can_defer_alignment(b, prepared || suppliedShifts);
     b->paths[defer ? MFSR_PATH_FRAMES_DEFERRED : MFSR_PATH_FRAMES_IMMEDIATE]++;
@@ -1447,6 +1586,12 @@
             return MFSR_OK;
         }
     }
+    if (can_hold_group(b, hostBurst)) {
+        TRY(align_deferred(b, stream));
+        b->hold[b->nHold++] = b->pend;
+        b->pend.n = 0;
+        return MFSR_OK;
+    }
     return accumulate_pending(b, stream);
 }
 
@@ -1483,7 +1628,8 @@
     MFSR_REQUIRE((long long)flowPitch >= 8LL * L.tw && (flowPitch & 7) == 0 && ((uintptr_t)flowOut & 7) == 0);
     MFSR_REQUIRE((long long)maskPitch >= 16LL * L.hw && (maskPitch & 15) == 0 && ((uintptr_t)maskOut & 15) == 0);
     TRY(mfsr_set_cfa_pattern(b->cfg.cfa));
-    const int slot = b->frameCounter++ % kRing;
+    TRY(fuse_hold(b, stream));
+    const int slot = b->frameCounter++ % b->ring;
     const Img *flow = nullptr, *mask = nullptr;
     TRY(align_frame(b, raw, isReference, slot, nullptr, nullptr, &flow, &mask, stream));
     b->flowCur = flow;
@@ -1508,13 +1654,14 @@
     for (int k = 0; k < nFrames; k++)
         MFSR_REQUIRE(raws[k] && flowOut[k] && maskOut[k] && ((uintptr_t)flowOut[k] & 7) == 0 && ((uintptr_t)maskOut[k] & 15) == 0);
     TRY(mfsr_set_cfa_pattern(b->cfg.cfa));
+    TRY(fuse_hold(b, stream));
     const bool batch = can_defer_alignment(b, false);
     const int per = batch ? b->group : 1;
     for (int k0 = 0; k0 < nFrames; k0 += per) {
         const int n = nFrames - k0 < per ? nFrames - k0 : per;
         for (int j = 0; j < n; j++) {
             const int isRef = isReference ? isReference[k0 + j] : 0;
-            const int slot = b->frameCounter++ % kRing;
+            const int slot = b->frameCounter++ % b->ring;
             b->pend.slot[j] = slot;
             b->pend.raw[j] = raws[k0 + j];
             b->pend.isRef[j] = isRef;
@@ -1577,6 +1724,7 @@
                                         c.scale, 12 * L.hrW, maskPitch, accumulatorsUndefined, rowBegin, rowEnd, stream));
     if (timed) {
         MFSR_HIP_TRY(hipEventRecord(b->evStop[b->nEvents], mfsr_s(stream)));
+        b->evLaunches[b->nEvents] = 1;
         b->nEvents++;
         b->nFramesTimed += nFrames;
     }
@@ -1624,6 +1772,7 @@
     TRY(flush_pending(b, stream));
     memset(b->paths, 0, sizeof(b->paths));
     b->sharpenedFinishes = 0;
+    b->burstLaunches = b->burstGroups = 0;
     b->fresh.has = true;
     b->fresh.imgOut = imgOut;
     b->fresh.totalWeights = totalWeights;
@@ -1703,7 +1852,7 @@
 extern "C" int mfsr_burst_set_sharpen(mfsr_burst* b, const mfsr_sharpen* sharpen)
 {
     MFSR_REQUIRE(b != nullptr);
-    MFSR_REQUIRE(b->pend.n == 0 && !b->heldHas && b->nUnp == 0);
+    MFSR_REQUIRE(b->pend.n == 0 && !b->heldHas && b->nHold == 0 && b->nUnp == 0);
     if (!sharpen) {
         b->sharpenOn = false;
         return MFSR_OK;
@@ -1726,7 +1875,7 @@
 extern "C" int mfsr_burst_set_render(mfsr_burst* b, const mfsr_render* render)
 {
     MFSR_REQUIRE(b != nullptr);
-    MFSR_REQUIRE(b->pend.n == 0 && !b->heldHas && b->nUnp == 0);
+    MFSR_REQUIRE(b->pend.n == 0 && !b->heldHas && b->nHold == 0 && b->nUnp == 0);
     if (!render) {
         b->renderOn = false;
         return MFSR_OK;
@@ -1980,6 +2129,7 @@
     MFSR_REQUIRE(b->haveRef);
     bool capturing = false;
     TRY(host_epoch(b, stream, &capturing));
+    TRY(fuse_hold(b, stream));
     const mfsr_config& c = b->cfg;
     const Layout& L = b->L;
     if (b->downRecorded) MFSR_HIP_TRY(hipStreamWaitEvent(mfsr_s(stream), b->evDown, 0));
@@ -2119,7 +2269,7 @@
 extern "C" int mfsr_burst_set_host_row_bytes(mfsr_burst* b, int rowBytes)
 {
     MFSR_REQUIRE(b != nullptr && b->cfg.uploadRing > 0);
-    MFSR_REQUIRE(b->pend.n == 0 && !b->heldHas && b->nUnp == 0);
+    MFSR_REQUIRE(b->pend.n == 0 && !b->heldHas && b->nHold == 0 && b->nUnp == 0);
     const bool isPacked = b->cfg.rawPacking != MFSR_PACK_NONE;
     const int dense = isPacked ? mfsr_packed_row_bytes(b->cfg.rawPacking, b->L.W) : 2 * b->L.W;
     MFSR_REQUIRE(rowBytes == 0 || rowBytes >= dense);
@@ -2433,7 +2583,7 @@
     TemporalScratch s;
     MFSR_REQUIRE(temporal_scratch(&c, nFrames, &s));
     MFSR_REQUIRE(((uintptr_t)scratchDev & 255) == 0 && scratchBytes >= s.total);
-    if (b->pend.n > 0 || b->heldHas || b->nUnp != 0) {
+    if (b->pend.n > 0 || b->heldHas || b->nHold > 0 || b->nUnp != 0) {
         fprintf(stderr, "mfsr: mfsr_burst_calibrate_noise_temporal with frames pending (flush or finish the burst first)\n");
         return MFSR_E_INVALID;
     }
@@ -2508,8 +2658,8 @@
 
 extern "C" int mfsr_burst_debug_frame_views(mfsr_burst* b, int framesBack, mfsr_tex2d* flow, mfsr_tex2d* mask)
 {
-    MFSR_REQUIRE(b != nullptr && framesBack >= 0 && framesBack < kRing && framesBack < b->frameCounter);
-    const int slot = (int)((b->frameCounter - 1 - framesBack) % kRing);
+    MFSR_REQUIRE(b != nullptr && framesBack >= 0 && framesBack < b->ring && framesBack < b->frameCounter);
+    const int slot = (int)((b->frameCounter - 1 - framesBack) % b->ring);
     MFSR_REQUIRE(b->slotFlow[slot] != nullptr);
     if (flow) *flow = as_tex(*b->slotFlow[slot]);
     if (mask) *mask = as_tex(b->L.maskBuf[slot]);
diff --git a/multi_frame_super_resolution_amd/pipeline.py b/multi_frame_super_resolution_amd/pipeline.py
--- a/multi_frame_super_resolution_amd/pipeline.py
+++ b/multi_frame_super_resolution_amd/pipeline.py
@@ -657,6 +657,8 @@
             self.L.burst_create(ctypes.byref(handle), ctypes.byref(cfg), self._ws_ptr, nbytes)
             self._h = handle
             self.window.apply(self.L.burst_set_window, self._h)
+        self._hold = None
+        self._held_frames = []
 
     def close(self):
         if getattr(self, "_h", None):
@@ -710,6 +712,18 @@
 
     def flush(self):
         self.L.burst_flush(self._h, self._stream())
+        self._held_frames.clear()
+
+    HOLD_FUSE = True
+
+    def hold_fuse(self, enable: bool = True):
+        self.L.burst_hold_fuse(self._h, 1 if enable else 0)
+        self._hold = bool(enable)
+
+    def fuse_stats(self):
+        n, g = ctypes.c_int(-1), ctypes.c_int(-1)
+        self.L.burst_fuse_stats(self._h, ctypes.byref(n), ctypes.byref(g))
+        return n.value, g.value
 
     @property
     def img_out(self) -> torch.Tensor:
@@ -727,26 +741,34 @@
         self._total_weights.zero_()
 
     def begin_burst(self):
+        if self._hold is None and self.HOLD_FUSE:
+            self.hold_fuse(True)
         self.L.burst_begin(self._h, self._img_out.data_ptr(), self._total_weights.data_ptr(), self._stream())
+        self._held_frames.clear()
 
     def set_reference(self, raw: torch.Tensor):
         self._check_raw(raw)
         self.L.burst_set_reference(self._h, raw.data_ptr(), self._stream())
+        self._held_frames.clear()
 
     def add_frame(self, raw: torch.Tensor, is_reference: bool = False):
         self._check_raw(raw)
         self.L.burst_add_frame(self._h, raw.data_ptr(), 1 if is_reference else 0, self._img_out.data_ptr(),
                                self._total_weights.data_ptr(), self._stream())
+        if self._hold:
+            self._held_frames.append(raw)
 
     def finish(self, want_float: bool = True, want_u16: bool = True):
         self.L.burst_finish(self._h, self._img_out.data_ptr(), self._total_weights.data_ptr(),
                             self.out_img.data_ptr() if want_float else None,
                             self.out16.data_ptr() if want_u16 else None, self._stream())
+        self._held_frames.clear()
         return self.window(self.out_img if want_float else None), self.window.output(self.out16 if want_u16 else None, self._fmt)
 
     def finish_rows(self, row0: int, rows: int) -> torch.Tensor:
         self.L.burst_finish_rows(self._h, self._img_out.data_ptr(), self._total_weights.data_ptr(), None,
                                  self.out16.data_ptr(), row0, rows, self._stream())
+        self._held_frames.clear()
         return self.out16
 
     def _checked(self, frames: Sequence[torch.Tensor], clone: bool):
```

New measurement: 24920 (median of 6 runs). 6.4% higher.
